# michelbarbeau/gr-uwspr

Hardware: AMD Instinct MI355X
Metric: 2-min WSPR frames decoded/sec (coarse+sync) (higher is better)
Workload: dtype f32

## Files before the change

gr-uwspr_amd/csrc/k4_jig.hip:

```cpp
#include "k4_common.h"

#pragma clang fp contract(off)

namespace uwspr {

constexpr int K4J_WAVES = 2;
#ifndef K4J_OCC
#define K4J_OCC 2
#endif
constexpr int K4J_PT_STRIDE = 18;

__global__ __launch_bounds__(64 * K4J_WAVES, K4J_OCC) void k4_jig(
    const float2 *__restrict__ frames, int fstride, int np, int nframes, const dev_grp *__restrict__ grps,
    int G, float *__restrict__ p_out, const float2 *__restrict__ ptab, int gps) {
  constexpr int NL = 6, PPW = 16;
  constexpr int R = 24;
  constexpr int AH = 21;
  constexpr int Q = (2 * (7 + AH) + 1) / 16;
  constexpr int M = Q + 1;
  constexpr int NSLOT = 16 + Q;
  constexpr int RS = 32 * M + 4;
  static_assert(4 * (NL - 1) < AH && M == 4, "ring reach");
  __shared__ __align__(16) float lds_all[K4J_WAVES][PPW * RS];
  __shared__ __align__(16) float2 ptl_all[K4J_WAVES][8 * K4J_PT_STRIDE];

  const int lane = threadIdx.x & 63;
  const int wv = __builtin_amdgcn_readfirstlane(threadIdx.x >> 6);
  float *lds = lds_all[wv];
  float2 *ptl = ptl_all[wv];

  const long long total = (long long)G * UWSPR_NSYM;
  const unsigned lblock = xcd_swizzle(blockIdx.x, gridDim.x);
  const long long g0 = ((long long)lblock * K4J_WAVES + wv) * PPW;
  if (g0 >= total) return;

  const int gA = (int)(g0 / UWSPR_NSYM);
  const int iA0 = (int)(g0 - (long long)gA * UWSPR_NSYM);
  const int sb = min(PPW, UWSPR_NSYM - iA0);
  const dev_grp A = grps[gA];
  const dev_grp Bg = grps[min(gA + 1, G - 1)];
  const bool okA = A.frame >= 0 && A.frame < nframes;
  const bool okB = (gA + 1 < G) && Bg.frame >= 0 && Bg.frame < nframes;
  const int frA = okA ? A.frame : 0, frB = okB ? Bg.frame : 0;
  const int nvA = okA ? (A.nvalid & 0xff) : 0, nvB = okB ? (Bg.nvalid & 0xff) : 0;
  const int selA = okA ? (A.nvalid >> 16) & 0xff : 0, selB = okB ? (Bg.nvalid >> 16) & 0xff : 0;
  const bool liveB = sb < PPW && okB;
  const bool use_tab = ptab != nullptr && (okA || liveB) && (!okA || selA != 0) && (!liveB || selB != 0);

  const int pr = lane >> 2;
  const int tone = lane & 3;
  const bool mineA = pr < sb;
  const int own_i = mineA ? iA0 + pr : pr - sb;
  if (!okA && !liveB) {
    if (g0 + pr < total) {
      const dev_grp &gy = mineA ? A : Bg;
      for (int l = 0; l < (gy.nvalid & 0xff) && l < NL; l++)
        p_out[((long long)(gy.hyp_base + (int)((gy.hmap >> (4 * l)) & 15u)) * UWSPR_NSYM + own_i) * 4 + tone] = 0.0f;
    }
    return;
  }
  const float2 *tabA = ptab, *tabB = ptab;
  if (use_tab) {
    tabA = ptab + ((size_t)(gA / gps) * kPtabPerSlot + (max(selA, 1) - 1)) * kPtabFloat2;
    tabB = ptab + ((size_t)((gA + 1) / gps) * kPtabPerSlot + (max(selB, 1) - 1)) * kPtabFloat2;
    if (!selA) tabA = tabB;
    if (!selB) tabB = tabA;
  }
  const bool knownA = !okA || (A.nvalid & 0x100) != 0, knownB = !okB || (Bg.nvalid & 0x100) != 0;
  const bool skip_mid = knownA && (knownB || sb >= PPW);
  const bool skip_last = !skip_mid && (!okA || nvA <= 5) && (!liveB || nvB <= 5);
  auto body = [&](auto skip_tag, auto tab_tag) __attribute__((always_inline)) {
  constexpr int SKIPL = decltype(skip_tag)::value;
  constexpr bool TAB = decltype(tab_tag)::value;
  const int l0A = okA ? A.lag[0] : 1 - 256 * iA0;
  const int l0B = okB ? Bg.lag[0] : 1;

  const int own_nb = (mineA ? l0A : l0B) + 256 * own_i;
  const bool interior = __all((own_nb > 0) && (own_nb + 255 + 16 * Q < np)  );

  const int kk = lane & 15;
  const int segq = lane >> 4;
  const float2 *src[4];
#pragma unroll
  for (int j = 0; j < 4; j++) {
    const int pj = 4 * j + segq;
    const bool sA = pj < sb;
    src[j] = frames + (long long)(sA ? frA : frB) * fstride + ((sA ? l0A + 256 * (iA0 + pj) : l0B + 256 * (pj - sb)) + kk);
  }
  float2 stage[4];
  auto load_slot = [&](int sl) {
    if (interior) {
#pragma unroll
      for (int j = 0; j < 4; j++) stage[j] = src[j][16 * sl];
    } else {
#pragma unroll
      for (int j = 0; j < 4; j++) {
        const int pj = 4 * j + segq;
        const bool sA = pj < sb;
        const int n = (sA ? l0A + 256 * (iA0 + pj) : l0B + 256 * (pj - sb)) + kk + 16 * sl;
        const bool inr = (n > 0) && (n < np);
        const float2 v = frames[(long long)(sA ? frA : frB) * fstride + min(max(n, 0), np - 1)];
        stage[j] = inr ? v : make_float2(0.0f, 0.0f);
      }
    }
  };
  const int st_row = segq * RS + 2 * kk;
  auto store_slot = [&](int pos) {
#pragma unroll
    for (int j = 0; j < 4; j++) *reinterpret_cast<float2 *>(&lds[st_row + 4 * j * RS + 32 * pos]) = stage[j];
  };
  float2 tstage[2];
  auto load_tab = [&](int c) {
#pragma unroll
    for (int j = 0; j < 2; j++) {
      const int e = lane + 64 * j, tn = (e >> 4) & 3, st = e & 15;
      tstage[j] = ((e >> 6) ? tabB : tabA)[tn * 256 + 16 * c + st];
    }
  };
  auto store_tab = [&]() {
#pragma unroll
    for (int j = 0; j < 2; j++) {
      const int e = lane + 64 * j;
      ptl[(e >> 4) * K4J_PT_STRIDE + (e & 15)] = tstage[j];
    }
  };

  {
    float2 pro[Q + 1][4];
#pragma unroll
    for (int sl = 0; sl <= Q; sl++) {
      load_slot(sl);
#pragma unroll
      for (int j = 0; j < 4; j++) pro[sl][j] = stage[j];
    }
    if (TAB) load_tab(0);
#pragma unroll
    for (int sl = 0; sl <= Q; sl++) {
#pragma unroll
      for (int j = 0; j < 4; j++) stage[j] = pro[sl][j];
      store_slot(sl);
    }
    if (TAB) store_tab();
  }
  float rc = 1.0f, rs = 0.0f, rcd = 1.0f, rsd = 0.0f;
  if (!TAB) {
    const dev_grp &gy = mineA ? A : Bg;
    const float fp = (gy.m_type == UWSPR_LINEAR)
                         ? (float)((double)gy.f0 + ((double)gy.drift / 2.0) * ((double)(float)own_i - 81.0) / 81.0)
                         : gy.f0 + gy.slmc;
    const float delta = ((float)tone - 1.5f) * 1.46484375f;
    double sn, cs;
    sincos(kTwoPiDt * (double)(fp + delta), &sn, &cs);
    rcd = (float)cs;
    rsd = (float)sn;
  }

  int sa[M];
#pragma unroll
  for (int q = 0; q < M; q++) sa[q] = pr * RS + 32 * q;
  const int trow = ((mineA ? 0 : 4) + tone) * K4J_PT_STRIDE;

  float inp[NL], quad[NL];
#pragma unroll
  for (int l = 0; l < NL; l++) { inp[l] = 0.0f; quad[l] = 0.0f; }

  float4 ring[R];
  wave_lds_fence();
#pragma unroll
  for (int e = 0; e < AH; e++) ring[e] = *reinterpret_cast<const float4 *>(&lds[sa[(2 * e) >> 4] + 2 * ((2 * e) & 15)]);
#pragma unroll
  for (int e = AH; e < R; e++) ring[e] = make_float4(0.0f, 0.0f, 0.0f, 0.0f);

  int wpos = 0;
  auto chunk = [&](auto phase_tag, int ch) __attribute__((always_inline)) {
    constexpr int PH = decltype(phase_tag)::value;
    load_slot(min(ch + Q + 1, NSLOT - 1));
    if (TAB) load_tab(min(ch + 1, 15));
    wave_lds_fence();
    float4 phn = make_float4(0.0f, 0.0f, 0.0f, 0.0f);
    if (TAB) phn = *reinterpret_cast<const float4 *>(&ptl[trow]);
#pragma unroll
    for (int i = 0; i < 8; i++) {
      const int j0 = 8 * PH + i;
      const int o = 2 * i + 2 * AH;
      ring[(j0 + AH) % R] = *reinterpret_cast<const float4 *>(&lds[sa[o >> 4] + 2 * (o & 15)]);
      float4 ph = phn;
      if (TAB) {
        if (i < 7) phn = *reinterpret_cast<const float4 *>(&ptl[trow + 2 * i + 2]);
      } else {
        ph.x = rc; ph.y = rs;
        k4_rot<false>(rc, rs, rcd, rsd);
        ph.z = rc; ph.w = rs;
        k4_rot<false>(rc, rs, rcd, rsd);
      }
      __builtin_amdgcn_sched_barrier(0);
#pragma unroll
      for (int l = 0; l < NL; l++) {
        if (l == SKIPL) continue;
        const float4 v = ring[(j0 + 4 * l) % R];
        k4_mac<false>(inp[l], quad[l], v.x, v.y, ph.x, ph.y);
        k4_mac<false>(inp[l], quad[l], v.z, v.w, ph.z, ph.w);
      }
      asm volatile("" : "+v"(inp[0]), "+v"(inp[1]), "+v"(inp[2]), "+v"(inp[3]), "+v"(inp[4]), "+v"(inp[5]),
                        "+v"(quad[0]), "+v"(quad[1]), "+v"(quad[2]), "+v"(quad[3]), "+v"(quad[4]), "+v"(quad[5])
                   :: "memory");
      __builtin_amdgcn_sched_barrier(0);
    }
    wave_lds_fence();
    store_slot(wpos);
    if (TAB) store_tab();
    wpos = (wpos + 1 == M) ? 0 : wpos + 1;
    const int first = sa[0];
#pragma unroll
    for (int q = 0; q + 1 < M; q++) sa[q] = sa[q + 1];
    sa[M - 1] = first;
  };
  for (int t = 0; t < 5; t++) {
    chunk(std::integral_constant<int, 0>{}, 3 * t);
    chunk(std::integral_constant<int, 1>{}, 3 * t + 1);
    chunk(std::integral_constant<int, 2>{}, 3 * t + 2);
  }
  chunk(std::integral_constant<int, 0>{}, 15);

  if (g0 + pr < total) {
    const int nv = mineA ? nvA : nvB;
    const int hb = mineA ? A.hyp_base : Bg.hyp_base;
    const uint32_t hm = mineA ? A.hmap : Bg.hmap;
#pragma unroll
    for (int l = 0; l < NL; l++) {
      if (l < nv && l != SKIPL) {
        const float pj = ieee_sqrtf(inp[l] * inp[l] + quad[l] * quad[l]);
        p_out[((long long)(hb + (int)((hm >> (4 * l)) & 15u)) * UWSPR_NSYM + own_i) * 4 + tone] = pj;
      }
    }
    const dev_grp &gy = mineA ? A : Bg;
    if (!(mineA ? okA : okB) && (gy.nvalid & 0xff) > 0)
      for (int l = 0; l < (gy.nvalid & 0xff) && l < NL; l++)
        p_out[((long long)(gy.hyp_base + (int)((gy.hmap >> (4 * l)) & 15u)) * UWSPR_NSYM + own_i) * 4 + tone] = 0.0f;
  }
  };
  if (use_tab) {
    if (skip_mid) body(std::integral_constant<int, 2>{}, std::true_type{});
    else if (skip_last) body(std::integral_constant<int, 5>{}, std::true_type{});
    else body(std::integral_constant<int, -1>{}, std::true_type{});
  } else {
    if (skip_mid) body(std::integral_constant<int, 2>{}, std::false_type{});
    else if (skip_last) body(std::integral_constant<int, 5>{}, std::false_type{});
    else body(std::integral_constant<int, -1>{}, std::false_type{});
  }
}

void launch_tonecorr_jig(uwspr_ctx *c, const float *frames, int B, const dev_grp *grps, int G, int64_t nhyps, float4 *p,
                         int gps) {
  if (G <= 0) return;
  prof_scope ps(c, UWSPR_K_TONECORR, nhyps, true);
  const long long total = (long long)G * UWSPR_NSYM;
  const long long waves = (total + 15) / 16;
  const unsigned blocks = (unsigned)((waves + K4J_WAVES - 1) / K4J_WAVES);
  if (gps < 1) gps = 1;
  launch_timed(c, ps, k4_jig, dim3(blocks), dim3(64 * K4J_WAVES), 0, (const float2 *)frames, c->fstride, c->np, B, grps, G,
               (float *)p, c->use_ptab ? (const float2 *)c->d_ptab : nullptr, gps);
}

}
```

gr-uwspr_amd/csrc/k4_tonecorr.hip:

```cpp
#include <string.h>

#include <algorithm>
#include <type_traits>

#include "k4_common.h"

#pragma clang fp contract(off)

namespace uwspr {

constexpr int K4_WAVES = 4;
constexpr int K4_ROWDW = 36;

template <int T, bool FAST = false>
__global__ __launch_bounds__(64 * K4_WAVES) void k4_tonecorr(
    const float2 *__restrict__ frames, int fstride, int np, int nframes, const dev_hyp *__restrict__ hyps,
    int H, float *__restrict__ p_out, const dev_grp *__restrict__ taken, int hyps_per_grp, int skip_pairs) {
  constexpr int PPW = 16 * T;
  constexpr int LPP = 4 / T;
  constexpr int NLD = PPW / 4;
  __shared__ __align__(16) float lds_all[K4_WAVES][PPW * K4_ROWDW];

  const int lane = threadIdx.x & 63;
  const int wv = __builtin_amdgcn_readfirstlane(threadIdx.x >> 6);
  float *lds = lds_all[wv];

  const long long total = (long long)H * UWSPR_NSYM;
  const long long g0 = ((long long)xcd_swizzle(blockIdx.x, gridDim.x) * K4_WAVES + wv) * PPW;
  if (g0 >= total) return;

  const int hA = (int)(g0 / UWSPR_NSYM);
  const int iA0 = (int)(g0 - (long long)hA * UWSPR_NSYM);
  const int sb = min(PPW, UWSPR_NSYM - iA0);
  dev_hyp A = hyps[hA];
  dev_hyp Bh = hyps[min(hA + 1, H - 1)];
  const int hB = min(hA + 1, H - 1);
  const bool takenA = (taken && ((taken[hA / hyps_per_grp].nvalid >> 16) & 0xff) != 0) ||
                      (skip_pairs && k4_drift_pair(hyps[hA & ~1], hyps[hA | 1], nframes));
  const bool takenB = (taken && ((taken[hB / hyps_per_grp].nvalid >> 16) & 0xff) != 0) ||
                      (skip_pairs && k4_drift_pair(hyps[hB & ~1], hyps[hB | 1], nframes));
  const bool okA = A.frame >= 0 && A.frame < nframes && !takenA;
  const bool okB = (hA + 1 < H) && Bh.frame >= 0 && Bh.frame < nframes && !takenB;
  if (!okA) { A.frame = 0; A.lag = 1 - 256 * iA0; }
  if (!okB) { Bh.frame = 0; Bh.lag = 1; }

  const int pr = lane / LPP;
  const int tone0 = (lane % LPP) * T;
  const bool mineA = pr < sb;
  const int own_i = mineA ? iA0 + pr : pr - sb;
  const bool own_ok = mineA ? okA : (okB && (g0 + pr) < total);
  if (!okA && !(okB && sb < PPW)) {
    if (g0 + pr < total && !(mineA ? takenA : takenB)) {
      float *out = p_out + (g0 + pr) * 4 + tone0;
#pragma unroll
      for (int j = 0; j < T; j++) out[j] = 0.0f;
    }
    return;
  }
  const int own_nb = (mineA ? A.lag : Bh.lag) + 256 * own_i;
  const bool interior = __all((own_nb > 0) && (own_nb + 255 < np));

  float cd[T], sd[T];
  {
    const dev_hyp &hy = mineA ? A : Bh;
    float fp;
    if (hy.m_type == UWSPR_LINEAR) {
      fp = (float)((double)hy.f0 +
                   ((double)hy.drift / 2.0) * ((double)(float)own_i - 81.0) / 81.0);
    } else {
      fp = hy.f0 + hy.slmc;
    }
#pragma unroll
    for (int j = 0; j < T; j++) {
      const float delta = ((float)(tone0 + j) - 1.5f) * 1.46484375f;
      const double ang = kTwoPiDt * (double)(fp + delta);
      double sn, cs;
      sincos(ang, &sn, &cs);
      cd[j] = (float)cs;
      sd[j] = (float)sn;
    }
  }

  const int kk = lane & 15;
  const int segq = lane >> 4;
  const float2 *src[NLD];
#pragma unroll
  for (int t = 0; t < NLD; t++) {
    const int seg = 4 * t + segq;
    const bool sA = seg < sb;
    const int fr = sA ? A.frame : Bh.frame;
    const int nb = sA ? A.lag + 256 * (iA0 + seg) : Bh.lag + 256 * (seg - sb);
    src[t] = frames + ((long long)fr * fstride + nb + kk);
  }

  float2 stage[NLD];
  auto load_chunk = [&](int c) {
    if (interior) {
#pragma unroll
      for (int t = 0; t < NLD; t++) stage[t] = src[t][16 * c];
    } else {
#pragma unroll
      for (int t = 0; t < NLD; t++) {
        const int seg = 4 * t + segq;
        const bool sA = seg < sb;
        const long long fb = (long long)(sA ? A.frame : Bh.frame) * fstride;
        const int n = (sA ? A.lag + 256 * (iA0 + seg) : Bh.lag + 256 * (seg - sb)) + 16 * c + kk;
        const bool inr = (n > 0) && (n < np);
        float2 v = frames[fb + min(max(n, 0), np - 1)];
        stage[t] = inr ? v : make_float2(0.0f, 0.0f);
      }
    }
  };

  float c[T], s[T], inp[T], quad[T];
#pragma unroll
  for (int j = 0; j < T; j++) { c[j] = 1.0f; s[j] = 0.0f; inp[j] = 0.0f; quad[j] = 0.0f; }

  load_chunk(0);
  for (int ch = 0; ch < 16; ch++) {
    wave_lds_fence();
#pragma unroll
    for (int t = 0; t < NLD; t++)
      *reinterpret_cast<float2 *>(&lds[(4 * t + segq) * K4_ROWDW + 2 * kk]) = stage[t];
    wave_lds_fence();
    if (ch < 15) load_chunk(ch + 1);
    float4 vnext = *reinterpret_cast<const float4 *>(&lds[pr * K4_ROWDW]);
#pragma unroll
    for (int k = 0; k < 16; k += 2) {
      const float4 v = vnext;
      if (k < 14) vnext = *reinterpret_cast<const float4 *>(&lds[pr * K4_ROWDW + 2 * (k + 2)]);
#pragma unroll
      for (int half = 0; half < 2; half++) {
        const float xx = half ? v.z : v.x, xy = half ? v.w : v.y;
#pragma unroll
        for (int j = 0; j < T; j++) {
          k4_mac<FAST>(inp[j], quad[j], xx, xy, c[j], s[j]);
          k4_rot<FAST>(c[j], s[j], cd[j], sd[j]);
        }
      }
    }
  }

  if (g0 + pr < total && !(mineA ? takenA : takenB)) {
    float *out = p_out + (g0 + pr) * 4 + tone0;
#pragma unroll
    for (int j = 0; j < T; j++) {
      const float pj = ieee_sqrtf(inp[j] * inp[j] + quad[j] * quad[j]);
      out[j] = own_ok ? pj : 0.0f;
    }
  }
}

void launch_tonecorr(uwspr_ctx *c, const float *frames, int B, const dev_hyp *hyps, int H,
                     float4 *p, const dev_grp *taken, int hyps_per_grp, bool skip_pairs) {
  if (H <= 0) return;
  prof_scope ps(c, UWSPR_K_TONECORR, H, true);
  const long long total = (long long)H * UWSPR_NSYM;
  int T = c->opt[UWSPR_OPT_K4_T];
  if (T != 1 && T != 2 && T != 4) T = total >= 1024 * 1024 ? 2 : 1;
  const long long waves = (total + 16 * T - 1) / (16 * T);
  const unsigned blocks = (unsigned)((waves + K4_WAVES - 1) / K4_WAVES);
  const float2 *fr = (const float2 *)frames;
  float *po = (float *)p;
  dim3 blk(64 * K4_WAVES);
  if (hyps_per_grp < 1) hyps_per_grp = 1;
  const int sp = skip_pairs && (H % 2 == 0) ? 1 : 0;
  if (T == 1 && c->fast_now) launch_timed(c, ps, (k4_tonecorr<1, true>), dim3(blocks), blk, 0, fr, c->fstride, c->np, B, hyps, H, po, taken, hyps_per_grp, sp);
  else if (T == 1) launch_timed(c, ps, k4_tonecorr<1>, dim3(blocks), blk, 0, fr, c->fstride, c->np, B, hyps, H, po, taken, hyps_per_grp, sp);
  else if (T == 2) launch_timed(c, ps, k4_tonecorr<2>, dim3(blocks), blk, 0, fr, c->fstride, c->np, B, hyps, H, po, taken, hyps_per_grp, sp);
  else launch_timed(c, ps, k4_tonecorr<4>, dim3(blocks), blk, 0, fr, c->fstride, c->np, B, hyps, H, po, taken, hyps_per_grp, sp);
}

}

namespace uwspr {

constexpr int K4G_WAVES = 2;

constexpr int K4_PT_STRIDE = 18;

template <int NL, int STEP, bool FAST = false>
__global__ __launch_bounds__(64 * K4G_WAVES) void k4_ring(
    const float2 *__restrict__ frames, int fstride, int np, int nframes, const dev_grp *__restrict__ grps,
    int G, float *__restrict__ p_out, const float2 *__restrict__ ptab, int gps) {
  constexpr int PPW = 16;
  constexpr int W = (NL - 1) * STEP;
  constexpr int Q = (15 + W) / 16;
  constexpr int M = Q + 1;
  constexpr int NSLOT = 16 + Q;
  constexpr int RS = 32 * M + 4;
  __shared__ __align__(16) float lds_all[K4G_WAVES][PPW * RS];
  __shared__ __align__(16) float2 ptl_all[K4G_WAVES][8 * K4_PT_STRIDE];

  const int lane = threadIdx.x & 63;
  const int wv = __builtin_amdgcn_readfirstlane(threadIdx.x >> 6);
  float *lds = lds_all[wv];
  float2 *ptl = ptl_all[wv];

  const long long total = (long long)G * UWSPR_NSYM;
  const unsigned lblock = xcd_swizzle(blockIdx.x, gridDim.x);
  const long long g0 = ((long long)lblock * K4G_WAVES + wv) * PPW;
  if (g0 >= total) return;

  const int gA = (int)(g0 / UWSPR_NSYM);
  const int iA0 = (int)(g0 - (long long)gA * UWSPR_NSYM);
  const int sb = min(PPW, UWSPR_NSYM - iA0);
  const dev_grp A = grps[gA];
  const dev_grp Bg = grps[min(gA + 1, G - 1)];
  const bool okA = A.frame >= 0 && A.frame < nframes;
  const bool okB = (gA + 1 < G) && Bg.frame >= 0 && Bg.frame < nframes;
  const int frA = okA ? A.frame : 0, frB = okB ? Bg.frame : 0;
  const int nvA = okA ? (A.nvalid & 0xff) : 0, nvB = okB ? (Bg.nvalid & 0xff) : 0;
  const int selA = okA ? (A.nvalid >> 16) & 0xff : 0, selB = okB ? (Bg.nvalid >> 16) & 0xff : 0;
  const bool liveB = sb < PPW && okB;
  const bool use_tab = ptab != nullptr && (okA || liveB) && (!okA || selA != 0) && (!liveB || selB != 0);
  const float2 *tabA = ptab, *tabB = ptab;
  if (use_tab) {
    if (selA) tabA = ptab + ((size_t)(gA / gps) * kPtabPerSlot + (selA - 1)) * kPtabFloat2;
    if (selB) tabB = ptab + ((size_t)((gA + 1) / gps) * kPtabPerSlot + (selB - 1)) * kPtabFloat2;
    if (!selA) tabA = tabB;
    if (!selB) tabB = tabA;
  }
  const bool knownA = !okA || (A.nvalid & 0x100) != 0, knownB = !okB || (Bg.nvalid & 0x100) != 0;
  const bool skip_mid = (NL == 5 || NL == 6) && knownA && (knownB || sb >= PPW);
#ifndef UWSPR_SKIP_LAST
#define UWSPR_SKIP_LAST 1
#endif
  const bool skip_last = UWSPR_SKIP_LAST && NL == 6 && !skip_mid && (okA || liveB) && (!okA || nvA <= 5) && (!liveB || nvB <= 5);
  const int l0A = okA ? A.lag[0] : 1 - 256 * iA0;
  const int l0B = okB ? Bg.lag[0] : 1;

  const int pr = lane >> 2;
  const int tone = lane & 3;
  const bool mineA = pr < sb;
  const int own_i = mineA ? iA0 + pr : pr - sb;
  if (!okA && !liveB) {
    if (g0 + pr < total) {
      const dev_grp &gy = mineA ? A : Bg;
      for (int l = 0; l < (gy.nvalid & 0xff) && l < NL; l++)
        p_out[((long long)(gy.hyp_base + (int)((gy.hmap >> (4 * l)) & 15u)) * UWSPR_NSYM + own_i) * 4 + tone] = 0.0f;
    }
    return;
  }
  const int own_nb = (mineA ? l0A : l0B) + 256 * own_i;
  const bool interior = __all((own_nb > 0) && (own_nb + 255 + 16 * Q < np)  );

  float cd = 1.0f, sd = 0.0f;
  if (!use_tab) {
    const dev_grp &gy = mineA ? A : Bg;
    float fp;
    if (gy.m_type == UWSPR_LINEAR) {
      fp = (float)((double)gy.f0 +
                   ((double)gy.drift / 2.0) * ((double)(float)own_i - 81.0) / 81.0);
    } else {
      fp = gy.f0 + gy.slmc;
    }
    const float delta = ((float)tone - 1.5f) * 1.46484375f;
    double sn, cs;
    sincos(kTwoPiDt * (double)(fp + delta), &sn, &cs);
    cd = (float)cs;
    sd = (float)sn;
  }

  const int kk = lane & 15;
  const int segq = lane >> 4;
  const float2 *src[4];
  long long fbase[4];
  int nfirst[4];
#pragma unroll
  for (int j = 0; j < 4; j++) {
    const int pj = 4 * j + segq;
    const bool sA = pj < sb;
    fbase[j] = (long long)(sA ? frA : frB) * fstride;
    nfirst[j] = (sA ? l0A + 256 * (iA0 + pj) : l0B + 256 * (pj - sb)) + kk;
    src[j] = frames + fbase[j] + nfirst[j];
  }
  float2 stage[4];
  auto load_slot = [&](int sl) {
    if (interior) {
#pragma unroll
      for (int j = 0; j < 4; j++) stage[j] = src[j][16 * sl];
    } else {
#pragma unroll
      for (int j = 0; j < 4; j++) {
        const int n = nfirst[j] + 16 * sl;
        const bool inr = (n > 0) && (n < np);
        const float2 v = frames[fbase[j] + min(max(n, 0), np - 1)];
        stage[j] = inr ? v : make_float2(0.0f, 0.0f);
      }
    }
  };
  auto store_slot = [&](int pos) {
#pragma unroll
    for (int j = 0; j < 4; j++)
      *reinterpret_cast<float2 *>(&lds[(4 * j + segq) * RS + 2 * kk + 32 * pos]) = stage[j];
  };

  {
    float2 pro[Q + 1][4];
#pragma unroll
    for (int sl = 0; sl <= Q; sl++) {
      load_slot(sl);
#pragma unroll
      for (int j = 0; j < 4; j++) pro[sl][j] = stage[j];
    }
#pragma unroll
    for (int sl = 0; sl <= Q; sl++) {
#pragma unroll
      for (int j = 0; j < 4; j++) stage[j] = pro[sl][j];
      store_slot(sl);
    }
  }

  int sa[M];
#pragma unroll
  for (int q = 0; q < M; q++) sa[q] = pr * RS + 32 * q;

  float c = 1.0f, s = 0.0f;
  float inp[NL], quad[NL];
#pragma unroll
  for (int l = 0; l < NL; l++) { inp[l] = 0.0f; quad[l] = 0.0f; }

  float2 tstage[2];
  auto load_tab = [&](int c) {
#pragma unroll
    for (int j = 0; j < 2; j++) {
      const int e = lane + 64 * j, tn = (e >> 4) & 3, st = e & 15;
      tstage[j] = ((e >> 6) ? tabB : tabA)[tn * 256 + 16 * c + st];
    }
  };
  auto store_tab = [&]() {
#pragma unroll
    for (int j = 0; j < 2; j++) {
      const int e = lane + 64 * j;
      ptl[(e >> 4) * K4_PT_STRIDE + (e & 15)] = tstage[j];
    }
  };
  const int trow = ((mineA ? 0 : 4) + tone) * K4_PT_STRIDE;
  if (use_tab) { load_tab(0); store_tab(); }

  int wpos = 0;
  auto walk = [&](auto skip_tag, auto tab_tag) {
    constexpr int SKIPL = decltype(skip_tag)::value;
    constexpr bool TAB = decltype(tab_tag)::value;
    for (int ch = 0; ch < 16; ch++) {
      load_slot(min(ch + Q + 1, NSLOT - 1));
      if (TAB) load_tab(min(ch + 1, 15));
      wave_lds_fence();
      static_assert(STEP % 2 == 0, "sample pairs must not straddle lags");
      float4 vc[NL], vn[NL];
#pragma unroll
      for (int l = 0; l < NL; l++) {
        if (l == SKIPL) { vc[l] = make_float4(0.0f, 0.0f, 0.0f, 0.0f); vn[l] = vc[l]; continue; }
        vc[l] = *reinterpret_cast<const float4 *>(&lds[sa[(STEP * l) >> 4] + 2 * ((STEP * l) & 15)]);
        vn[l] = vc[l];
      }
#pragma unroll
      for (int k = 0; k < 16; k += 2) {
        if (k < 14) {
#pragma unroll
          for (int l = 0; l < NL; l++) {
            if (l == SKIPL) continue;
            const int o = k + 2 + STEP * l;
            vn[l] = *reinterpret_cast<const float4 *>(&lds[sa[o >> 4] + 2 * (o & 15)]);
          }
        }
        float4 ph = make_float4(0.0f, 0.0f, 0.0f, 0.0f);
        if (TAB) ph = *reinterpret_cast<const float4 *>(&ptl[trow + k]);
#pragma unroll
        for (int half = 0; half < 2; half++) {
          const float pc = TAB ? (half ? ph.z : ph.x) : c, psn = TAB ? (half ? ph.w : ph.y) : s;
#pragma unroll
          for (int l = 0; l < NL; l++) {
            if (l == SKIPL) continue;
            const float xx = half ? vc[l].z : vc[l].x, xy = half ? vc[l].w : vc[l].y;
            k4_mac<FAST>(inp[l], quad[l], xx, xy, pc, psn);
          }
          if (!TAB) k4_rot<FAST>(c, s, cd, sd);
        }
#pragma unroll
        for (int l = 0; l < NL; l++) vc[l] = vn[l];
      }
      wave_lds_fence();
      store_slot(wpos);
      if (TAB) store_tab();
      wpos = (wpos + 1 == M) ? 0 : wpos + 1;
      const int first = sa[0];
#pragma unroll
      for (int q = 0; q + 1 < M; q++) sa[q] = sa[q + 1];
      sa[M - 1] = first;
    }
  };
  using sk_none = std::integral_constant<int, -1>;
  using sk_mid = std::integral_constant<int, 2>;
  using sk_last = std::integral_constant<int, NL == 6 ? NL - 1 : -1>;
  if (use_tab) {
    if (skip_mid) walk(sk_mid{}, std::true_type{});
    else if (skip_last) walk(sk_last{}, std::true_type{});
    else walk(sk_none{}, std::true_type{});
  } else {
    if (skip_mid) walk(sk_mid{}, std::false_type{});
    else if (skip_last) walk(sk_last{}, std::false_type{});
    else walk(sk_none{}, std::false_type{});
  }

  if (g0 + pr < total) {
    const int nv = mineA ? nvA : nvB;
    const int hb = mineA ? A.hyp_base : Bg.hyp_base;
    const uint32_t hm = mineA ? A.hmap : Bg.hmap;
#pragma unroll
    for (int l = 0; l < NL; l++) {
      if (l < nv && !(skip_mid && l == 2)) {
        const float pj = ieee_sqrtf(inp[l] * inp[l] + quad[l] * quad[l]);
        p_out[((long long)(hb + (int)((hm >> (4 * l)) & 15u)) * UWSPR_NSYM + own_i) * 4 + tone] = pj;
      }
    }
    const dev_grp &gy = mineA ? A : Bg;
    if (!(mineA ? okA : okB) && (gy.nvalid & 0xff) > 0)
      for (int l = 0; l < (gy.nvalid & 0xff) && l < NL; l++)
        p_out[((long long)(gy.hyp_base + (int)((gy.hmap >> (4 * l)) & 15u)) * UWSPR_NSYM + own_i) * 4 + tone] = 0.0f;
  }
}

void launch_tonecorr_ring(uwspr_ctx *c, const float *frames, int B, const dev_grp *grps, int G,
                          int NL, int step, int64_t nhyps, float4 *p, int gps) {
  if (G <= 0) return;
  const bool r5 = NL == 5 && step == 16, r6 = NL == 6 && step == 8;
  if (!r5 && !r6) return;
  prof_scope ps(c, UWSPR_K_TONECORR, nhyps, true);
  const long long total = (long long)G * UWSPR_NSYM;
  const long long waves = (total + 15) / 16;
  const unsigned blocks = (unsigned)((waves + K4G_WAVES - 1) / K4G_WAVES);
  const float2 *fr = (const float2 *)frames;
  float *po = (float *)p;
  dim3 blk(64 * K4G_WAVES);
  const float2 *pt = c->use_ptab ? c->d_ptab : nullptr;
  if (gps < 1) gps = 1;
  if (r5 && c->fast_now) launch_timed(c, ps, (k4_ring<5, 16, true>), dim3(blocks), blk, 0, fr, c->fstride, c->np, B, grps, G, po, pt, gps);
  else if (r5) launch_timed(c, ps, (k4_ring<5, 16>), dim3(blocks), blk, 0, fr, c->fstride, c->np, B, grps, G, po, pt, gps);
  else launch_timed(c, ps, (k4_ring<6, 8>), dim3(blocks), blk, 0, fr, c->fstride, c->np, B, grps, G, po, pt, gps);
}


}

namespace uwspr {

#ifndef K4F_CHUNK
#define K4F_CHUNK 32
#endif

constexpr int K4L_ROWS_PER_SLOT = UWSPR_NSYM + 1;

template <int QMASK, bool FAST>
__device__ __forceinline__ void k4_lag0_chunk(const float *__restrict__ smprow, const float4 *__restrict__ tabrow,
                                              int a0, float (&inp)[4], float (&quad)[4]) {
#pragma unroll 1
  for (int k0 = 0; k0 < 32; k0 += 8) {
#pragma unroll
    for (int kk = 0; kk < 8; kk += 2) {
      const int k = k0 + kk;
      const float4 x = *reinterpret_cast<const float4 *>(&smprow[2 * k]);
#pragma unroll
      for (int q = 0; q < 4; q++) {
        if (!((QMASK >> q) & 1)) continue;
        const float4 ph = tabrow[(a0 - 64 * q + k) >> 1];
        k4_mac<FAST>(inp[q], quad[q], x.x, x.y, ph.x, ph.y);
        k4_mac<FAST>(inp[q], quad[q], x.z, x.w, ph.z, ph.w);
      }
    }
  }
}

template <bool FAST = false>
__global__ __launch_bounds__(256, 4) void k4_lag0(
    const float2 *__restrict__ frames, int fstride, int np, int nframes, const dev_grp *__restrict__ grps,
    int nslots, float *__restrict__ p_out, const float2 *__restrict__ ptab) {
  constexpr int ROWS = 64, CH = 32, ROWDW = 2 * CH + 4, SEGS = 256 / CH, NR = ROWS / SEGS, NCHUNK = 14;
  __shared__ __align__(16) float smp[ROWS * ROWDW];
  __shared__ __align__(16) float4 tab[2][4][128];

  const int tid = threadIdx.x;
  const int lane = tid & 63;
  const int tone = __builtin_amdgcn_readfirstlane(tid >> 6);
  const long long total = (long long)nslots * K4L_ROWS_PER_SLOT;
  const long long g0 = (long long)xcd_swizzle(blockIdx.x, gridDim.x) * ROWS;
  if (g0 >= total) return;

  const int slotA = (int)(g0 / K4L_ROWS_PER_SLOT);
  const int rA0 = (int)(g0 - (long long)slotA * K4L_ROWS_PER_SLOT);
  const int sb = min(ROWS, K4L_ROWS_PER_SLOT - rA0);
  const bool hasB = sb < ROWS && slotA + 1 < nslots;
  const int slotB = hasB ? slotA + 1 : slotA;
  const dev_grp A = grps[slotA], Bg = grps[slotB];
  const int selA = (A.nvalid >> 16) & 0xff, selB = (Bg.nvalid >> 16) & 0xff;
  const bool doA = A.frame >= 0 && A.frame < nframes && selA != 0;
  const bool doB = hasB && Bg.frame >= 0 && Bg.frame < nframes && selB != 0;
  if (!doA && !doB) return;

#pragma unroll
  for (int sl = 0; sl < 2; sl++) {
    if (!(sl ? doB : doA)) continue;
    const float4 *src = reinterpret_cast<const float4 *>(
        ptab + ((size_t)(sl ? slotB : slotA) * kPtabPerSlot + ((sl ? selB : selA) - 1)) * kPtabFloat2);
    float4 *dst = &tab[sl][0][0];
    dst[tid] = src[tid];
    dst[tid + 256] = src[tid + 256];
  }

  const int row = lane;
  const bool mineA = row < sb;
  const int own_r = mineA ? rA0 + row : row - sb;
  const bool own_do = mineA ? doA : doB;
  const bool valid = (g0 + row < total) && (mineA || hasB) && own_do;

  const int kk = tid % CH, seg = tid / CH;
  const float2 *fbA = frames + (long long)(doA ? A.frame : 0) * fstride;
  const float2 *fbB = frames + (long long)(doB ? Bg.frame : 0) * fstride;
  const int nA0 = A.lag[0] + 256 * rA0, nB0 = Bg.lag[0];
  const bool interior = doA && (nA0 > 0) && (nA0 + 256 * (sb - 1) + 32 * NCHUNK < np) &&
                        (sb >= ROWS || (doB && (nB0 > 0) && (nB0 + 256 * (ROWS - sb - 1) + 32 * NCHUNK < np)));
  float2 stage[NR];
  int nrow[NR];
  bool rowB[NR];
#pragma unroll
  for (int r = 0; r < NR; r++) {
    const int rw = SEGS * r + seg;
    rowB[r] = rw >= sb;
    nrow[r] = (rowB[r] ? nB0 + 256 * (rw - sb) : nA0 + 256 * rw) + kk;
  }
  auto load_chunk = [&](int c) {
    if (interior) {
#pragma unroll
      for (int r = 0; r < NR; r++) stage[r] = (rowB[r] ? fbB : fbA)[nrow[r] + CH * c];
    } else {
#pragma unroll
      for (int r = 0; r < NR; r++) {
        const int n = nrow[r] + CH * c;
        const bool inr = (n > 0) && (n < np);
        const float2 v = (rowB[r] ? fbB : fbA)[min(max(n, 0), np - 1)];
        stage[r] = inr ? v : make_float2(0.0f, 0.0f);
      }
    }
  };
  auto store_chunk = [&]() {
#pragma unroll
    for (int r = 0; r < NR; r++)
      *reinterpret_cast<float2 *>(&smp[(SEGS * r + seg) * ROWDW + 2 * kk]) = stage[r];
  };

  float inp[4], quad[4];
#pragma unroll
  for (int q = 0; q < 4; q++) { inp[q] = 0.0f; quad[q] = 0.0f; }
  const float *smprow = &smp[row * ROWDW];
  const float4 *tabrow = &tab[mineA ? 0 : 1][tone][0];

  load_chunk(0);
  auto phase = [&](auto mask_tag, int c0) {
    constexpr int QMASK = decltype(mask_tag)::value;
#pragma unroll 1
    for (int c = c0; c < c0 + 2; c++) {
      __syncthreads();
      store_chunk();
      __syncthreads();
      load_chunk(min(c + 1, NCHUNK - 1));
      k4_lag0_chunk<QMASK, FAST>(smprow, tabrow, 32 * c, inp, quad);
    }
  };
  phase(std::integral_constant<int, 0x1>{}, 0);
  phase(std::integral_constant<int, 0x3>{}, 2);
  phase(std::integral_constant<int, 0x7>{}, 4);
  phase(std::integral_constant<int, 0xf>{}, 6);
  phase(std::integral_constant<int, 0xe>{}, 8);
  phase(std::integral_constant<int, 0xc>{}, 10);
  phase(std::integral_constant<int, 0x8>{}, 12);

  if (valid) {
    const int hb = mineA ? A.hyp_base : Bg.hyp_base;
#pragma unroll
    for (int q = 0; q < 4; q++) {
      const float pj = ieee_sqrtf(inp[q] * inp[q] + quad[q] * quad[q]);
      if (own_r < UWSPR_NSYM) p_out[((long long)(hb + q) * UWSPR_NSYM + own_r) * 4 + tone] = pj;
      if (q == 0 && own_r >= 1) p_out[((long long)(hb + 4) * UWSPR_NSYM + own_r - 1) * 4 + tone] = pj;
    }
  }
}

template <int WSETS>
__global__ __launch_bounds__(256 * WSETS, WSETS == 1 ? 3 : 6) void k4_lag0x(
    const float2 *__restrict__ frames, int fstride, int np, int nframes, const dev_grp *__restrict__ grps,
    int nslots, float *__restrict__ p_out, const float2 *__restrict__ ptab) {
  constexpr int NT = 256 * WSETS;
  constexpr int ROWS = 64, CH = 32, ROWDW = 2 * CH + 4, SEGS = NT / CH, NR = ROWS / SEGS, NCHUNK = 14;
  __shared__ __align__(16) float smp[2][ROWS * ROWDW];
  __shared__ __align__(16) float4 tab[2][4][128];

  const int tid = threadIdx.x;
  const int lane = tid & 63;
  const int wv = __builtin_amdgcn_readfirstlane(tid >> 6);
  const int tone = wv & 3;
  const int wset = wv >> 2;
  const long long total = (long long)nslots * K4L_ROWS_PER_SLOT;
  const long long g0 = (long long)xcd_swizzle(blockIdx.x, gridDim.x) * ROWS;
  if (g0 >= total) return;

  const int slotA = (int)(g0 / K4L_ROWS_PER_SLOT);
  const int rA0 = (int)(g0 - (long long)slotA * K4L_ROWS_PER_SLOT);
  const int sb = min(ROWS, K4L_ROWS_PER_SLOT - rA0);
  const bool hasB = sb < ROWS && slotA + 1 < nslots;
  const int slotB = hasB ? slotA + 1 : slotA;
  const dev_grp A = grps[slotA], Bg = grps[slotB];
  const int selA = (A.nvalid >> 16) & 0xff, selB = (Bg.nvalid >> 16) & 0xff;
  const bool doA = A.frame >= 0 && A.frame < nframes && selA != 0;
  const bool doB = hasB && Bg.frame >= 0 && Bg.frame < nframes && selB != 0;
  if (!doA && !doB) return;

#pragma unroll
  for (int sl = 0; sl < 2; sl++) {
    if (!(sl ? doB : doA)) continue;
    const float4 *src = reinterpret_cast<const float4 *>(
        ptab + ((size_t)(sl ? slotB : slotA) * kPtabPerSlot + ((sl ? selB : selA) - 1)) * kPtabFloat2);
    float4 *dst = &tab[sl][0][0];
    for (int e = tid; e < 512; e += NT) dst[e] = src[e];
  }

  const int row = lane;
  const bool mineA = row < sb;
  const int own_r = mineA ? rA0 + row : row - sb;
  const bool own_do = mineA ? doA : doB;
  const bool valid = (g0 + row < total) && (mineA || hasB) && own_do;

  const int kk = tid % CH, seg = tid / CH;
  const float2 *fbA = frames + (long long)(doA ? A.frame : 0) * fstride;
  const float2 *fbB = frames + (long long)(doB ? Bg.frame : 0) * fstride;
  const int nA0 = A.lag[0] + 256 * rA0, nB0 = Bg.lag[0];
  const bool interior = doA && (nA0 > 0) && (nA0 + 256 * (sb - 1) + 32 * NCHUNK < np) &&
                        (sb >= ROWS || (doB && (nB0 > 0) && (nB0 + 256 * (ROWS - sb - 1) + 32 * NCHUNK < np)));
  float2 stage[NR];
  int nrow[NR];
  bool rowB[NR];
#pragma unroll
  for (int r = 0; r < NR; r++) {
    const int rw = SEGS * r + seg;
    rowB[r] = rw >= sb;
    nrow[r] = (rowB[r] ? nB0 + 256 * (rw - sb) : nA0 + 256 * rw) + kk;
  }
  auto load_chunk = [&](int c) {
    if (interior) {
#pragma unroll
      for (int r = 0; r < NR; r++) stage[r] = (rowB[r] ? fbB : fbA)[nrow[r] + CH * c];
    } else {
#pragma unroll
      for (int r = 0; r < NR; r++) {
        const int n = nrow[r] + CH * c;
        const bool inr = (n > 0) && (n < np);
        const float2 v = (rowB[r] ? fbB : fbA)[min(max(n, 0), np - 1)];
        stage[r] = inr ? v : make_float2(0.0f, 0.0f);
      }
    }
  };
  auto store_chunk = [&](int buf) {
#pragma unroll
    for (int r = 0; r < NR; r++)
      *reinterpret_cast<float2 *>(&smp[buf][(SEGS * r + seg) * ROWDW + 2 * kk]) = stage[r];
  };

  float inp[4], quad[4];
#pragma unroll
  for (int q = 0; q < 4; q++) { inp[q] = 0.0f; quad[q] = 0.0f; }
  const float4 *tabrow = &tab[mineA ? 0 : 1][tone][0];

  load_chunk(0);
  store_chunk(0);
  load_chunk(1);
  __syncthreads();
  auto phase = [&](auto mask_tag, int c0) {
    constexpr int QM = decltype(mask_tag)::value;
#pragma unroll 1
    for (int c = c0; c < c0 + 2; c++) {
      if (WSETS == 1) {
        k4_lag0_chunk<QM, false>(&smp[c & 1][row * ROWDW], tabrow, 32 * c, inp, quad);
      } else if (wset == 0) {
        if (QM & 0x5) k4_lag0_chunk<QM & 0x5, false>(&smp[c & 1][row * ROWDW], tabrow, 32 * c, inp, quad);
      } else {
        if (QM & 0xa) k4_lag0_chunk<QM & 0xa, false>(&smp[c & 1][row * ROWDW], tabrow, 32 * c, inp, quad);
      }
      store_chunk((c + 1) & 1);
      load_chunk(min(c + 2, NCHUNK - 1));
      __syncthreads();
    }
  };
  phase(std::integral_constant<int, 0x1>{}, 0);
  phase(std::integral_constant<int, 0x3>{}, 2);
  phase(std::integral_constant<int, 0x7>{}, 4);
  phase(std::integral_constant<int, 0xf>{}, 6);
  phase(std::integral_constant<int, 0xe>{}, 8);
  phase(std::integral_constant<int, 0xc>{}, 10);
  phase(std::integral_constant<int, 0x8>{}, 12);

  if (valid) {
    const int hb = mineA ? A.hyp_base : Bg.hyp_base;
#pragma unroll
    for (int q = 0; q < 4; q++) {
      if (WSETS == 2 && (q & 1) != wset) continue;
      const float pj = ieee_sqrtf(inp[q] * inp[q] + quad[q] * quad[q]);
      if (own_r < UWSPR_NSYM) p_out[((long long)(hb + q) * UWSPR_NSYM + own_r) * 4 + tone] = pj;
      if (q == 0 && own_r >= 1) p_out[((long long)(hb + 4) * UWSPR_NSYM + own_r - 1) * 4 + tone] = pj;
    }
  }
}

void launch_tonecorr_lag0(uwspr_ctx *c, const float *frames, int B, const dev_grp *grps, int nslots,
                          int64_t nhyps, float4 *p) {
  if (nslots <= 0) return;
  prof_scope ps(c, UWSPR_K_TONECORR, nhyps, true);
  const unsigned wgs = (unsigned)(((long long)nslots * K4L_ROWS_PER_SLOT + 63) / 64);
  const int form = c->fast_now ? 0 : (c->opt[UWSPR_OPT_K4_FORMS] >> 1) & 3;
  if (c->fast_now)
    launch_timed(c, ps, k4_lag0<true>, dim3(wgs), dim3(256), 0, (const float2 *)frames, c->fstride, c->np, B, grps,
                 nslots, (float *)p, (const float2 *)c->d_ptab);
  else if (form & 2)
    launch_timed(c, ps, k4_lag0x<2>, dim3(wgs), dim3(512), 0, (const float2 *)frames, c->fstride, c->np, B, grps,
                 nslots, (float *)p, (const float2 *)c->d_ptab);
  else if (form & 1)
    launch_timed(c, ps, k4_lag0x<1>, dim3(wgs), dim3(256), 0, (const float2 *)frames, c->fstride, c->np, B, grps,
                 nslots, (float *)p, (const float2 *)c->d_ptab);
  else
    launch_timed(c, ps, k4_lag0<false>, dim3(wgs), dim3(256), 0, (const float2 *)frames, c->fstride, c->np, B, grps,
                 nslots, (float *)p, (const float2 *)c->d_ptab);
}

#ifdef K4F_STAMPS
constexpr int K4F_STAMP_WAVES = 4096;
__device__ unsigned long long g_k4f_stamps[K4F_STAMP_WAVES * 10];
#define K4F_T(v) const unsigned long long v = __builtin_amdgcn_s_memtime()
#define K4F_ACC(a, t1, t0) a += (t1) - (t0)
#else
#define K4F_T(v) do { } while (0)
#define K4F_ACC(a, t1, t0) do { } while (0)
#endif

template <int NF, int CH, bool FAST = false>
__global__ __launch_bounds__(256) void k4_fpack(
    const float2 *__restrict__ frames, int fstride, int np, int nframes, const dev_hyp *__restrict__ hyps,
    int nslots, float *__restrict__ p_out) {
  constexpr int ROWS = 64;
  constexpr int ROWDW = 2 * CH + 4;
  constexpr int NCH = 256 / CH;
  constexpr int SEGS = 256 / CH;
  constexpr int NR = ROWS / SEGS;
  __shared__ __align__(16) float smp[ROWS * ROWDW];
  __shared__ __align__(16) float4 tab[2][4][CH / 2][NF];

  const int tid = threadIdx.x;
  const int lane = tid & 63;
  const int tone = __builtin_amdgcn_readfirstlane(tid >> 6);
  #ifdef K4F_STAMPS
  const unsigned long long st_c0 = __builtin_amdgcn_s_memtime(), st_r0 = __builtin_amdgcn_s_memrealtime();
  unsigned long long st_bar1 = 0, st_gen = 0, st_bar2 = 0, st_ar = 0;
#endif
  const long long total = (long long)nslots * UWSPR_NSYM;
  const long long g0 = (long long)xcd_swizzle(blockIdx.x, gridDim.x) * ROWS;
  if (g0 >= total) return;
  const unsigned prio_class = k4_prio_class();

  const int slotA = (int)(g0 / UWSPR_NSYM);
  const int iA0 = (int)(g0 - (long long)slotA * UWSPR_NSYM);
  const int sb = min(ROWS, UWSPR_NSYM - iA0);
  const bool hasB = sb < ROWS && slotA + 1 < nslots;
  const int slotB = hasB ? slotA + 1 : slotA;
  const dev_hyp hA = hyps[(size_t)slotA * NF], hB = hyps[(size_t)slotB * NF];
  float fA[NF], fB[NF];
#pragma unroll
  for (int q = 0; q < NF; q++) { fA[q] = hyps[(size_t)slotA * NF + q].f0; fB[q] = hyps[(size_t)slotB * NF + q].f0; }
  const bool liveA = hA.frame >= 0 && hA.frame < nframes;
  const bool liveB = hasB && hB.frame >= 0 && hB.frame < nframes;
  const bool tabA = (hA.m_type != UWSPR_LINEAR) || (hA.drift == 0.0f);
  const bool tabB = (hB.m_type != UWSPR_LINEAR) || (hB.drift == 0.0f);
  const bool knownA = hyps[(size_t)slotA * NF + NF / 2].frame <= -2, knownB = hyps[(size_t)slotB * NF + NF / 2].frame <= -2;
  const bool tabled = (!liveA || tabA) && (!liveB || tabB);
  const bool skip_mid = (liveA || liveB) && (!liveA || knownA) && (!liveB || knownB);

  const int row = lane;
  const bool mineA = row < sb;
  const int own_i = mineA ? iA0 + row : row - sb;
  const int own_slot = mineA ? slotA : slotB;
  const bool own_live = mineA ? liveA : liveB;
  const bool valid = (g0 + row < total) && (mineA || hasB);
  if (!liveA && !liveB) {
    if (valid) {
#pragma unroll
      for (int q = 0; q < NF; q++) p_out[(((long long)own_slot * NF + q) * UWSPR_NSYM + own_i) * 4 + tone] = 0.0f;
    }
    return;
  }
  const dev_hyp &ho = mineA ? hA : hB;
  const float delta = ((float)tone - 1.5f) * 1.46484375f;

  const int kk = tid % CH, seg = tid / CH;
  const float2 *fbA = frames + (long long)(liveA ? hA.frame : 0) * fstride;
  const float2 *fbB = frames + (long long)(liveB ? hB.frame : 0) * fstride;
  const int nA0 = hA.lag + 256 * iA0, nB0 = hB.lag;
  const bool interior = liveA && (nA0 > 0) && (nA0 + 256 * sb < np) &&
                        (sb >= ROWS || (liveB && (nB0 > 0) && (nB0 + 256 * (ROWS - sb) < np)));
  float2 stage[NR];
  int nrow[NR];
  bool rowB[NR];
#pragma unroll
  for (int r = 0; r < NR; r++) {
    const int rw = SEGS * r + seg;
    rowB[r] = rw >= sb;
    nrow[r] = (rowB[r] ? nB0 + 256 * (rw - sb) : nA0 + 256 * rw) + kk;
  }
  auto load_chunk = [&](int c) {
    if (interior) {
#pragma unroll
      for (int r = 0; r < NR; r++) stage[r] = (rowB[r] ? fbB : fbA)[nrow[r] + CH * c];
    } else {
#pragma unroll
      for (int r = 0; r < NR; r++) {
        const int n = nrow[r] + CH * c;
        const bool inr = (n > 0) && (n < np);
        const float2 v = (rowB[r] ? fbB : fbA)[min(max(n, 0), np - 1)];
        stage[r] = inr ? v : make_float2(0.0f, 0.0f);
      }
    }
  };
  auto store_chunk = [&]() {
#pragma unroll
    for (int r = 0; r < NR; r++)
      *reinterpret_cast<float2 *>(&smp[(SEGS * r + seg) * ROWDW + 2 * kk]) = stage[r];
  };

  float inp[NF], quad[NF];
#pragma unroll
  for (int q = 0; q < NF; q++) { inp[q] = 0.0f; quad[q] = 0.0f; }

  if (tabled) {
    float cq = 1.0f, sq = 0.0f, cdq = 1.0f, sdq = 0.0f;
    const int gs = lane >= 4 * NF ? 1 : 0, gl = lane - gs * 4 * NF;
    const int gq = gl % NF, gt = min(gl / NF, 3);
    const bool gen = (tone == 0) && (lane < 8 * NF) && (gs ? liveB : liveA);
    if (gen) {
      float fq = gs ? fB[0] : fA[0];
#pragma unroll
      for (int q = 1; q < NF; q++) fq = (gq == q) ? (gs ? fB[q] : fA[q]) : fq;
      const dev_hyp &hg = gs ? hB : hA;
      const float fp = (hg.m_type == UWSPR_LINEAR)
                           ? (float)((double)fq + ((double)hg.drift / 2.0) * ((double)(float)0 - 81.0) / 81.0)
                           : fq + hg.slmc;
      const float gdelta = ((float)gt - 1.5f) * 1.46484375f;
      double sn, cs;
      sincos(kTwoPiDt * (double)(fp + gdelta), &sn, &cs);
      cdq = (float)cs;
      sdq = (float)sn;
    }
    const float4 *mytab = &tab[mineA ? 0 : 1][tone][0][0];
    load_chunk(0);
    auto walk = [&](auto skip_tag) {
      constexpr bool SKIP = decltype(skip_tag)::value;
      for (int ch = 0; ch < NCH; ch++) {
        K4F_T(t0);
        __syncthreads();
        K4F_T(t1);
        store_chunk();
        if (gen) {
#pragma unroll
          for (int k = 0; k < CH; k++) {
            reinterpret_cast<float2 *>(&tab[gs][gt][k >> 1][gq])[k & 1] = make_float2(cq, sq);
            k4_rot<FAST>(cq, sq, cdq, sdq);
          }
        }
        K4F_T(t2);
        __syncthreads();
        K4F_T(t3);
        k4_rotate_priority((unsigned)ch, prio_class);
        load_chunk(min(ch + 1, NCH - 1));
#pragma unroll
        for (int k = 0; k < CH; k += 2) {
          const float4 x = *reinterpret_cast<const float4 *>(&smp[row * ROWDW + 2 * k]);
#pragma unroll
          for (int q = 0; q < NF; q++) {
            if (SKIP && q == NF / 2) continue;
            const float4 ph = mytab[(k >> 1) * NF + q];
            k4_mac<FAST>(inp[q], quad[q], x.x, x.y, ph.x, ph.y);
            k4_mac<FAST>(inp[q], quad[q], x.z, x.w, ph.z, ph.w);
          }
        }
        K4F_T(t4);
        K4F_ACC(st_bar1, t1, t0); K4F_ACC(st_gen, t2, t1); K4F_ACC(st_bar2, t3, t2); K4F_ACC(st_ar, t4, t3);
      }
    };
    if (skip_mid) walk(std::true_type{}); else walk(std::false_type{});
  } else {
    float c[NF], s[NF], cd[NF], sd[NF];
#pragma unroll
    for (int q = 0; q < NF; q++) {
      const float f0 = mineA ? fA[q] : fB[q];
      const float fp = (ho.m_type == UWSPR_LINEAR)
                           ? (float)((double)f0 + ((double)ho.drift / 2.0) * ((double)(float)own_i - 81.0) / 81.0)
                           : f0 + ho.slmc;
      double sn, cs;
      sincos(kTwoPiDt * (double)(fp + delta), &sn, &cs);
      cd[q] = (float)cs; sd[q] = (float)sn; c[q] = 1.0f; s[q] = 0.0f;
    }
    load_chunk(0);
    for (int ch = 0; ch < NCH; ch++) {
      __syncthreads();
      store_chunk();
      __syncthreads();
      load_chunk(min(ch + 1, NCH - 1));
#pragma unroll
      for (int k = 0; k < CH; k += 2) {
        const float4 x4 = *reinterpret_cast<const float4 *>(&smp[row * ROWDW + 2 * k]);
#pragma unroll
        for (int half = 0; half < 2; half++) {
          const float xx = half ? x4.z : x4.x, xy = half ? x4.w : x4.y;
#pragma unroll
          for (int q = 0; q < NF; q++) {
            k4_mac<FAST>(inp[q], quad[q], xx, xy, c[q], s[q]);
            k4_rot<FAST>(c[q], s[q], cd[q], sd[q]);
          }
        }
      }
    }
  }

#ifdef K4F_STAMPS
  {
    const unsigned gw = xcd_swizzle(blockIdx.x, gridDim.x) * 4 + tone;
    if (lane == 0 && gw < (unsigned)K4F_STAMP_WAVES) {
      unsigned long long *o = &g_k4f_stamps[(size_t)gw * 10];
      o[0] = st_c0; o[1] = __builtin_amdgcn_s_memtime(); o[2] = st_r0; o[3] = __builtin_amdgcn_s_memrealtime();
      o[4] = st_bar1; o[5] = st_gen; o[6] = st_bar2; o[7] = st_ar;
      o[8] = (unsigned long long)__builtin_amdgcn_s_getreg((31 << 11) | 4) | ((unsigned long long)__builtin_amdgcn_s_getreg((31 << 11) | 20) << 32);
      o[9] = tabled ? 1 : 0;
    }
  }
#endif
  if (valid) {
#pragma unroll
    for (int q = 0; q < NF; q++) {
      float *o = &p_out[(((long long)own_slot * NF + q) * UWSPR_NSYM + own_i) * 4 + tone];
      if (!own_live) *o = 0.0f;
      else if (!(skip_mid && q == NF / 2)) *o = ieee_sqrtf(inp[q] * inp[q] + quad[q] * quad[q]);
    }
  }
}

void launch_tonecorr_fstage(uwspr_ctx *c, const float *frames, int B, const dev_hyp *hyps, int nslots,
                            int64_t nhyps, float4 *p) {
  if (nslots <= 0) return;
  prof_scope ps(c, UWSPR_K_TONECORR, nhyps, true);
  const unsigned wgs = (unsigned)(((long long)nslots * UWSPR_NSYM + 63) / 64);
  if (c->fast_now)
    launch_timed(c, ps, (k4_fpack<5, K4F_CHUNK, true>), dim3(wgs), dim3(256), 0,
                 (const float2 *)frames, c->fstride, c->np, B, hyps, nslots, (float *)p);
  else
    launch_timed(c, ps, (k4_fpack<5, K4F_CHUNK>), dim3(wgs), dim3(256), 0,
                 (const float2 *)frames, c->fstride, c->np, B, hyps, nslots, (float *)p);
}

}

#ifdef K4F_STAMPS
extern "C" int uwspr_debug_k4f_stamps(unsigned long long *out, int nwaves) {
  if (nwaves > uwspr::K4F_STAMP_WAVES) nwaves = uwspr::K4F_STAMP_WAVES;
  hipDeviceSynchronize();
  return (int)hipMemcpyFromSymbol(out, HIP_SYMBOL(uwspr::g_k4f_stamps), (size_t)nwaves * 80);
}
#endif
```

gr-uwspr_amd/csrc/k5_fold_schedule.hip:

```cpp
#include "uwspr_internal.h"

#pragma clang fp contract(off)

namespace uwspr {

__device__ __constant__ uint32_t kPr3[6] = UWSPR_PR3_WORDS;
__device__ __forceinline__ bool pr3_rt(int i) { return (kPr3[i >> 5] >> (i & 31)) & 1u; }

__device__ __forceinline__ void k5_wave_fence() {
  __builtin_amdgcn_fence(__ATOMIC_RELEASE, "wavefront");
  __builtin_amdgcn_wave_barrier();
  __builtin_amdgcn_fence(__ATOMIC_ACQUIRE, "wavefront");
}
constexpr int K5L_CH = 9;
__global__ __launch_bounds__(64) void k5_fold(const dev_hyp *__restrict__ hyps,
                                              const float4 *__restrict__ p, int H,
                                              float symfac, float *__restrict__ sync,
                                              uint8_t *__restrict__ symbols,
                                              const float4 *__restrict__ pwin, int per_slot) {
  UWSPR_SET_PRIO(UWSPR_SMALL_PRIO);
  __shared__ __align__(16) float4 tile[64 * K5L_CH];
  __shared__ __align__(16) uint8_t bytes[64 * UWSPR_NSYM];
  __shared__ int rowoff[64];
  __shared__ int rowslot[64];
  const int lane = threadIdx.x;
  const int h0 = blockIdx.x * 64;
  const int nh = min(64, H - h0);
  const int h = h0 + min(lane, nh - 1);
  const int fr = hyps[h].frame;
  const bool known = pwin != nullptr && fr <= -2;
  const bool live = lane < nh && (fr >= 0 || known);
  const bool soft = symbols != nullptr;
  const float4 *base = p + (size_t)h0 * UWSPR_NSYM;
  rowoff[lane] = known ? -1 : min(lane, nh - 1) * UWSPR_NSYM;
  rowslot[lane] = known ? h / per_slot : 0;

  auto stage = [&](int c) {
    k5_wave_fence();
#pragma unroll
    for (int j = 0; j < K5L_CH; j++) {
      const int idx = lane + 64 * j;
      const int hy = idx / K5L_CH, sy = idx - hy * K5L_CH;
      const int ro = rowoff[hy];
      tile[idx] = ro >= 0 ? base[(size_t)ro + c * K5L_CH + sy]
                          : pwin[(size_t)rowslot[hy] * UWSPR_NSYM + c * K5L_CH + sy];
    }
    k5_wave_fence();
  };

  float ss = 0.0f, totp = 0.0f, fsum = 0.0f, f2sum = 0.0f;
  for (int c = 0; c < UWSPR_NSYM / K5L_CH; c++) {
    stage(c);
#pragma unroll
    for (int j = 0; j < K5L_CH; j++) {
      const float4 P = tile[lane * K5L_CH + j];
      const bool bit = pr3_rt(c * K5L_CH + j);
      totp = totp + P.x; totp = totp + P.y; totp = totp + P.z; totp = totp + P.w;
      const float cmet = (P.y + P.w) - (P.x + P.z);
      ss = bit ? ss + cmet : ss - cmet;
      if (soft) {
        const float fs = bit ? P.w - P.y : P.z - P.x;
        fsum = (float)((double)fsum + (double)fs / 162.0);
        f2sum = (float)((double)f2sum + (double)(fs * fs) / 162.0);
      }
    }
  }
  if (lane < nh) sync[h] = live ? ieee_divf(ss, totp) : -1e30f;
  if (!soft) return;

  const float fac = ieee_sqrtf(f2sum - fsum * fsum);
  for (int c = 0; c < UWSPR_NSYM / K5L_CH; c++) {
    stage(c);
#pragma unroll
    for (int j = 0; j < K5L_CH; j++) {
      const float4 P = tile[lane * K5L_CH + j];
      const int i = c * K5L_CH + j;
      const bool bit = pr3_rt(i);
      float v = bit ? P.w - P.y : P.z - P.x;
      v = ieee_divf(symfac * v, fac);
      if (v > 127.0f) v = 127.0f;
      if (v < -128.0f) v = -128.0f;
      v = v + 128.0f;
      bytes[lane * UWSPR_NSYM + i] = (!live || v != v) ? (uint8_t)0 : (uint8_t)(int)v;
    }
  }
  k5_wave_fence();
  uint8_t *out = symbols + (size_t)h0 * UWSPR_NSYM;
  const int nbytes = nh * UWSPR_NSYM;
  for (int o = 4 * lane; o < nbytes; o += 256) {
    if (o + 4 <= nbytes && ((reinterpret_cast<uintptr_t>(out) + o) & 3) == 0) {
      *reinterpret_cast<uint32_t *>(out + o) = *reinterpret_cast<const uint32_t *>(&bytes[o]);
    } else {
      for (int q = 0; q < 4 && o + q < nbytes; q++) out[o + q] = bytes[o + q];
    }
  }
}

constexpr int K5W_WAVES = 4;

struct k5_wave_lds {
  float4 str[2][UWSPR_NSYM];
};
struct k5_wave_lds_soft {
  double q[2][UWSPR_NSYM];
};

template <bool SOFT>
__device__ __forceinline__ float fold_wave(const dev_hyp *__restrict__ hyps,
                                           const float4 *__restrict__ p, int h, float symfac,
                                           uint8_t *__restrict__ symbols, k5_wave_lds &L,
                                           k5_wave_lds_soft *Q, const float4 *__restrict__ prow = nullptr) {
  const int lane = threadIdx.x & 63;
  if (hyps[h].frame < 0 && !prow) {
    if (SOFT)
      for (int i = lane; i < UWSPR_NSYM; i += 64) symbols[(size_t)h * UWSPR_NSYM + i] = 0;
    return -1e30f;
  }
  const float4 *src = prow ? prow : p + (size_t)h * UWSPR_NSYM;
  float fs[3];
#pragma unroll
  for (int r = 0; r < 3; r++) {
    const int i = lane + 64 * r;
    fs[r] = 0.0f;
    if (i < UWSPR_NSYM) {
      const float4 P = src[i];
      const bool bit = pr3_rt(i);
      L.str[0][i] = P;
      const float cmet = (P.y + P.w) - (P.x + P.z);
      L.str[1][i] = make_float4(0.0f, 0.0f, 0.0f, bit ? cmet : -cmet);
      fs[r] = bit ? P.w - P.y : P.z - P.x;
      if (SOFT) {
        Q->q[0][i] = (double)fs[r] / 162.0;
        Q->q[1][i] = (double)(fs[r] * fs[r]) / 162.0;
      }
    }
  }
  k5_wave_fence();
  float acc = 0.0f;
  if (lane < 2) {
    const float4 *st = L.str[lane];
#pragma unroll 9
    for (int i = 0; i < UWSPR_NSYM; i++) {
      const float4 P = st[i];
      acc = acc + P.x; acc = acc + P.y; acc = acc + P.z; acc = acc + P.w;
    }
  } else if (SOFT && lane < 4) {
    const double *q = Q->q[lane - 2];
#pragma unroll 9
    for (int i = 0; i < UWSPR_NSYM; i++) acc = (float)((double)acc + q[i]);
  }
  const float totp = __shfl(acc, 0), ss = __shfl(acc, 1);
  const float sync = ieee_divf(ss, totp);
  if (SOFT) {
    const float fsum = __shfl(acc, 2), f2sum = __shfl(acc, 3);
    const float fac = ieee_sqrtf(f2sum - fsum * fsum);
#pragma unroll
    for (int r = 0; r < 3; r++) {
      const int i = lane + 64 * r;
      if (i < UWSPR_NSYM) {
        float v = ieee_divf(symfac * fs[r], fac);
        if (v > 127.0f) v = 127.0f;
        if (v < -128.0f) v = -128.0f;
        v = v + 128.0f;
        symbols[(size_t)h * UWSPR_NSYM + i] = (v != v) ? (uint8_t)0 : (uint8_t)(int)v;
      }
    }
  }
  k5_wave_fence();
  return sync;
}

template <bool SOFT>
__global__ __launch_bounds__(64 * K5W_WAVES) void k5_fold_wave(
    const dev_hyp *__restrict__ hyps, const float4 *__restrict__ p, int H, float symfac,
    float *__restrict__ sync, uint8_t *__restrict__ symbols, const float4 *__restrict__ pwin, int per_slot) {
  UWSPR_SET_PRIO(UWSPR_SMALL_PRIO);
  __shared__ k5_wave_lds L[K5W_WAVES];
  __shared__ k5_wave_lds_soft Q[SOFT ? K5W_WAVES : 1];
  const int wv = __builtin_amdgcn_readfirstlane(threadIdx.x >> 6);
  const int h = blockIdx.x * K5W_WAVES + wv;
  if (h >= H) return;
  const float4 *prow = (pwin && hyps[h].frame <= -2) ? pwin + (size_t)(h / per_slot) * UWSPR_NSYM : nullptr;
  const float s = fold_wave<SOFT>(hyps, p, h, symfac, symbols, L[wv], SOFT ? &Q[wv] : nullptr, prow);
  if ((threadIdx.x & 63) == 0) sync[h] = s;
}

void launch_fold(uwspr_ctx *c, const dev_hyp *hyps, const float4 *p, int H, float *sync,
                 uint8_t *symbols, const float4 *pwin, int per_slot) {
  if (H <= 0) return;
  prof_scope ps(c, UWSPR_K_FOLD, H);
  const int forced = c->opt[UWSPR_OPT_K5_LANES];
  const bool lanes_form = forced >= 0 ? forced != 0 : H >= 32768;
  if (per_slot < 1) per_slot = 1;
  if (!lanes_form) {
    dim3 g((H + K5W_WAVES - 1) / K5W_WAVES), b(64 * K5W_WAVES);
    if (symbols) hipLaunchKernelGGL(k5_fold_wave<true>, g, b, 0, c->stream, hyps, p, H, 50.0f, sync, symbols, pwin, per_slot);
    else hipLaunchKernelGGL(k5_fold_wave<false>, g, b, 0, c->stream, hyps, p, H, 50.0f, sync, symbols, pwin, per_slot);
  } else {
    hipLaunchKernelGGL(k5_fold, dim3((H + 63) / 64), dim3(64), 0, c->stream, hyps, p, H, 50.0f,
                       sync, symbols, pwin, per_slot);
  }
}

__device__ float slm_drift_t0(double V1, double V2, int p1, int p2, float cf) {
  const double q1 = V1 * 0.0 + (double)p1, q2 = V2 * 0.0 + (double)p2;
  const float sign = (float)(((q1 * V1 + q2 * V2) > 0) * 2 - 1);
  const double num = fabs(V1 * q1 + V2 * q2);
  const double den = sqrt(q1 * q1 + q2 * q2);
  if (den == 0) return 0.0f;
  return (float)((double)(-sign) * num / den * (double)cf / (double)1500.0f);
}

__global__ void k_prep_hyps(const uwspr_hyp *__restrict__ in, dev_hyp *__restrict__ out, int H,
                            float cf) {
  const int h = blockIdx.x * 256 + threadIdx.x;
  if (h >= H) return;
  const uwspr_hyp a = in[h];
  dev_hyp d;
  d.frame = a.frame; d.lag = a.lag; d.f0 = a.f0; d.drift = a.drift; d.m_type = a.m_type;
  d.slmc = (a.m_type == UWSPR_NONLINEAR) ? slm_drift_t0(a.V1, a.V2, a.p1, a.p2, cf) : 0.0f;
  out[h] = d;
}

void launch_prep_hyps(uwspr_ctx *c, const uwspr_hyp *abi, dev_hyp *out, int H) {
  if (H <= 0) return;
  prof_scope ps(c, UWSPR_K_SCHED, H);
  hipLaunchKernelGGL(k_prep_hyps, dim3((H + 255) / 256), dim3(256), 0, c->stream, abi, out, H,
                     (float)c->p.cf);
}


__device__ inline void emit(dev_hyp *h, const cand_state &st, bool on, int lag, float f0,
                            float drift, bool known = false) {
  h->frame = on ? (known ? -2 - st.frame : st.frame) : -1;
  h->lag = lag; h->f0 = f0; h->drift = drift; h->slmc = st.slmc; h->m_type = st.m_type;
}

__device__ inline void emit_group(dev_grp *g, const cand_state &st, bool on, float f0, float drift,
                                  int hyp_base, const int *lags, int n, uint32_t hmap = 0x76543210u) {
  g->frame = on ? st.frame : -1;
  g->m_type = st.m_type; g->f0 = f0; g->drift = drift; g->slmc = st.slmc;
  g->nvalid = n; g->hyp_base = hyp_base; g->hmap = hmap;
  for (int l = 0; l < 8; l++) g->lag[l] = l < n ? lags[l] : lags[0];
}

__device__ inline void emit_centre(uwspr_candidate *ce, int32_t *cframe, const cand_state &st, bool on) {
  ce->freq = st.f1; ce->snr = 0.0f; ce->drift = 0.0f; ce->sync = 0.0f; ce->shift = st.shift1;
  ce->m_nonlinear.V1 = 0.0; ce->m_nonlinear.V2 = 0.0; ce->m_nonlinear.p1 = 0; ce->m_nonlinear.p2 = 0;
  if (st.m_type == UWSPR_LINEAR) { ce->m_type = UWSPR_LINEAR; ce->m_linear.drift = st.drift1; }
  else { ce->m_type = 2; ce->m_linear.drift = st.slmc; }
  *cframe = on ? st.frame : -1;
}

struct best3 { float sync; int shift; float f; int q; };
__device__ inline best3 best_of(const float *sy, const dev_hyp *hy, int n) {
  best3 b{-1e30f, 0, 0.0f, -1};
  for (int q = 0; q < n; q++)
    if (sy[q] > b.sync) { b.sync = sy[q]; b.shift = hy[q].lag; b.f = hy[q].f0; b.q = q; }
  return b;
}

constexpr double kTwoPiDt5 = 2.0 * 3.14159265358979323846 * (double)(float)(1.0 / 375.0);

__device__ __forceinline__ void ptab_build(float2 *__restrict__ tabs, int nq, int qfirst, float fc, float fstep,
                                           int m_type, float drift, float slmc) {
  const int lane = threadIdx.x & 63;
  if (lane >= 4 * nq) return;
  const int qi = lane >> 2, tone = lane & 3, q = qfirst + qi;
  const float f0 = fc + (float)(q - 2) * fstep;
  const float fp = (m_type == UWSPR_LINEAR)
                       ? (float)((double)f0 + ((double)drift / 2.0) * ((double)(float)0 - 81.0) / 81.0)
                       : f0 + slmc;
  const float delta = ((float)tone - 1.5f) * 1.46484375f;
  double sn, cs;
  sincos(kTwoPiDt5 * (double)(fp + delta), &sn, &cs);
  const float cd = (float)cs, sd = (float)sn;
  float c = 1.0f, sv = 0.0f;
  float4 *t = reinterpret_cast<float4 *>(tabs + (size_t)qi * kPtabFloat2 + tone * 256);
  for (int k = 0; k < 128; k += 4) {
    float4 v[4];
#pragma unroll
    for (int j = 0; j < 4; j++) {
      v[j].x = c; v[j].y = sv;
      float nc = c * cd - sv * sd;
      float ns = c * sd + sv * cd;
      c = nc; sv = ns;
      v[j].z = c; v[j].w = sv;
      nc = c * cd - sv * sd;
      ns = c * sd + sv * cd;
      c = nc; sv = ns;
    }
#pragma unroll
    for (int j = 0; j < 4; j++) t[k + j] = v[j];
  }
}

__device__ __forceinline__ int ptab_index(const cand_state &st, int set, float f0, float drift, bool on) {
  if (!on) return -1;
  if (st.m_type == UWSPR_LINEAR && drift != 0.0f) return -1;
  if (!(set == 0 ? st.tabA_ok : st.tabB_ok)) return -1;
  const float fc = set == 0 ? st.tabA_f : st.tabB_f, step = set == 0 ? 0.25f : 0.05f;
  for (int q = 0; q < 5; q++)
    if (__float_as_int(fc + (float)(q - 2) * step) == __float_as_int(f0)) return (set == 0 ? 0 : kPtabSetB) + q;
  return -1;
}
__device__ __forceinline__ int ptab_set(const cand_state &st, int set, float centre, float drift, bool on) {
  if (!on) return -1;
  if (st.m_type == UWSPR_LINEAR && drift != 0.0f) return -1;
  if (!(set == 0 ? st.tabA_ok : st.tabB_ok)) return -1;
  if (__float_as_int(centre) != __float_as_int(set == 0 ? st.tabA_f : st.tabB_f)) return -1;
  return set == 0 ? 0 : kPtabSetB;
}
__device__ __forceinline__ int ptab_select(const cand_state &st, int set, float f0, float drift, bool on) {
  return ptab_index(st, set, f0, drift, on) + 1;
}

__global__ void k_sched_init(const uwspr_candidate *__restrict__ cands,
                             const int32_t *__restrict__ npk, int cand_stride, int B,
                             int per_frame, float cf, cand_state *__restrict__ state,
                             dev_hyp *__restrict__ hyps, dev_grp *__restrict__ grps, float2 *__restrict__ ptab) {
  UWSPR_SET_PRIO(UWSPR_SMALL_PRIO);
  const int slot = blockIdx.x;
  if (slot >= B * per_frame) return;
  const int b = slot / per_frame, j = slot - b * per_frame;
  cand_state st;
  const bool on = j < npk[b] && j < cand_stride;
  if (on) {
    const uwspr_candidate cnd = cands[(size_t)b * cand_stride + j];
    st.frame = b;
    st.m_type = cnd.m_type;
    st.slmc = (cnd.m_type == UWSPR_NONLINEAR)
                  ? slm_drift_t0(cnd.m_nonlinear.V1, cnd.m_nonlinear.V2, cnd.m_nonlinear.p1,
                                 cnd.m_nonlinear.p2, cf)
                  : 0.0f;
    st.f1 = cnd.freq;
    st.drift1 = (cnd.m_type == UWSPR_LINEAR) ? cnd.m_linear.drift : 0.0f;
    st.shift1 = cnd.shift;
    st.sync1 = cnd.sync;
  } else {
    st.frame = -1; st.m_type = 0; st.slmc = 0.0f; st.f1 = 0.0f; st.drift1 = 0.0f;
    st.shift1 = 0; st.sync1 = 0.0f;
  }
  st.worth = 0; st.driftp = 0.0f; st.driftm = 0.0f; st.csync = 0.0f; st.cknown = 0;
  const float f0 = st.f1 + (float)0 * 0.0f;
  st.tabA_f = f0; st.tabB_f = 0.0f; st.tabB_ok = 0;
  st.tabA_ok = (ptab != nullptr && on && (st.m_type != UWSPR_LINEAR || st.drift1 == 0.0f)) ? 1 : 0;
  if (st.tabA_ok) ptab_build(ptab + ((size_t)slot * kPtabPerSlot + 2) * kPtabFloat2, 1, 2, f0, 0.25f, st.m_type, st.drift1, st.slmc);
  if (threadIdx.x != 0) return;
  state[slot] = st;
  dev_hyp *h = hyps + (size_t)slot * 5;
  int lags[5];
  for (int q = 0; q < 5; q++) {
    lags[q] = st.shift1 - 128 + 64 * q;
    emit(&h[q], st, on, lags[q], f0, st.drift1);
  }
  emit_group(&grps[slot], st, on, f0, st.drift1, slot * 5, lags, 5);
  grps[slot].nvalid |= ptab_select(st, 0, f0, st.drift1, on) << 16;
}

template <int STAGE>
__device__ __forceinline__ void sched_step_body(int slot, cand_state *__restrict__ state,
                                                const dev_hyp *__restrict__ hin,
                                                const float *sync_of_slot,
                                                dev_hyp *__restrict__ hout,
                                                dev_grp *__restrict__ grps,
                                                uwspr_candidate *__restrict__ cent,
                                                int32_t *__restrict__ cframe, bool reuse, int team = 0,
                                                int njig = UWSPR_NJIG, int *wsrc = nullptr, bool tabs = false,
                                                bool fast = false) {
  int ws = -1;
  cand_state st = state[slot];
  const bool live = st.frame >= 0;
  constexpr int NIN = STAGE == 1 ? 5 : STAGE == 2 ? 5 : STAGE == 3 ? 2 : STAGE == 4 ? 5 : 5;
  constexpr int NOUT = STAGE == 1 ? 5 : STAGE == 2 ? 2 : STAGE == 3 ? 5 : STAGE == 4 ? 5 : 17;
  const dev_hyp *hi = hin + (size_t)slot * NIN;
  const float *sy = sync_of_slot;
  dev_hyp *ho = hout + (size_t)slot * (STAGE == 5 ? njig : NOUT);

  if (STAGE == 1) {
    if (live) { best3 b = best_of(sy, hi, 5); st.sync1 = b.sync; st.shift1 = b.shift; st.f1 = b.f; ws = b.q; }
    st.cknown = (reuse && live && st.sync1 > -1e30f) ? 1 : 0;
    st.csync = st.sync1;
    for (int q = 0; q < 5; q++)
      emit(&ho[q], st, live, st.shift1, st.f1 + (float)(q - 2) * 0.25f, st.drift1, q == 2 && st.cknown);
    emit_centre(&cent[slot], &cframe[slot], st, live);
  } else if (STAGE == 2) {
    if (live) {
      best3 b = best_of(sy, hi, 5); st.sync1 = b.sync; st.shift1 = b.shift; st.f1 = b.f;
      ws = (b.q == 2 && hi[2].frame <= -2) ? -1 : b.q;
    }
    st.cknown = (reuse && live && st.sync1 > -1e30f) ? 1 : 0;
    st.csync = st.sync1;
    const bool lin = live && st.m_type == UWSPR_LINEAR;
    st.driftp = (float)((double)st.drift1 + 0.5);
    st.driftm = (float)((double)st.drift1 - 0.5);
    const float f0 = st.f1 + (float)0 * 0.0f;
    emit(&ho[0], st, lin, st.shift1, f0, st.driftp);
    emit(&ho[1], st, lin, st.shift1, f0, st.driftm);
    emit_centre(&cent[slot], &cframe[slot], st, lin);
  } else if (STAGE == 3) {
    if (live && st.m_type == UWSPR_LINEAR) {
      float syncp = -1e30f, syncm = -1e30f;
      if (sy[0] > syncp) syncp = sy[0]; else { st.f1 = 0.0f; st.shift1 = 0; st.cknown = 0; }
      if (sy[1] > syncm) syncm = sy[1]; else { st.f1 = 0.0f; st.shift1 = 0; st.cknown = 0; }
      if (syncp > st.sync1) { st.drift1 = st.driftp; st.sync1 = syncp; ws = 0; }
      else if (syncm > st.sync1) { st.drift1 = st.driftm; st.sync1 = syncm; ws = 1; }
    }
    st.worth = (live && st.sync1 > 0.10f) ? 1 : 0;
    st.csync = st.sync1;
    const float f0 = st.f1 + (float)0 * 0.0f;
    int lags[5];
    for (int q = 0; q < 5; q++) {
      lags[q] = st.shift1 - 32 + 16 * q;
      emit(&ho[q], st, st.worth != 0, lags[q], f0, st.drift1, q == 2 && st.cknown);
    }
    emit_group(&grps[slot], st, st.worth != 0, f0, st.drift1, slot * 5, lags, 5);
    if (st.cknown) grps[slot].nvalid |= 0x100;
    st.tabB_f = f0;
    st.tabB_ok = (tabs && st.worth && (st.m_type != UWSPR_LINEAR || st.drift1 == 0.0f)) ? 1 : 0;
    grps[slot].nvalid |= ptab_select(st, 1, f0, st.drift1, st.worth != 0) << 16;
  } else if (STAGE == 4) {
    if (st.worth) {
      best3 b = best_of(sy, hi, 5); st.sync1 = b.sync; st.shift1 = b.shift; st.f1 = b.f;
      ws = (b.q == 2 && hi[2].frame <= -2) ? -1 : b.q;
    }
    st.cknown = (reuse && st.worth && st.sync1 > -1e30f) ? 1 : 0;
    st.csync = st.sync1;
    for (int q = 0; q < 5; q++)
      emit(&ho[q], st, st.worth != 0, st.shift1, st.f1 + (float)(q - 2) * 0.05f, st.drift1,
           q == 2 && st.cknown);
    emit_centre(&cent[slot], &cframe[slot], st, st.worth != 0);
  } else {
    if (st.worth) {
      best3 b = best_of(sy, hi, 5); st.sync1 = b.sync; st.shift1 = b.shift; st.f1 = b.f;
      ws = (b.q == 2 && hi[2].frame <= -2) ? -1 : b.q;
    }
    const bool known0 = reuse && !fast && st.worth && st.sync1 > -1e30f;
    st.cknown = known0 ? 1 : 0;
    if (team < njig) {
      const int idt = team;
      int ii = (idt + 1) / 2;
      if (idt % 2 == 1) ii = -ii;
      ii = 8 * ii;
      emit(&ho[idt], st, st.worth != 0, st.shift1 + ii, st.f1, st.drift1, idt == 0 && known0);
    }
    for (int g = 0; g < 3; g++) {
      if (team != UWSPR_NJIG + g) continue;
      const int n = g < 2 ? 6 : 5;
      int gl[6], idt0 = 99;
      int id[6];
      for (int l = 0; l < n; l++) {
        const int m = 6 * g + l, d = m - 8;
        id[l] = d == 0 ? 0 : (d < 0 ? -2 * d - 1 : 2 * d);
        gl[l] = st.shift1 + 8 * d;
        idt0 = id[l] < idt0 ? id[l] : idt0;
      }
      uint32_t hmap = 0;
      for (int l = 0; l < n; l++) hmap |= (uint32_t)(id[l] - idt0) << (4 * l);
      emit_group(&grps[slot * 3 + g], st, st.worth != 0 && njig >= UWSPR_NJIG, st.f1, st.drift1,
                 slot * UWSPR_NJIG + idt0, gl, n, hmap);
      if (g == 1 && known0) grps[slot * 3 + g].nvalid |= 0x100;
      grps[slot * 3 + g].nvalid |= ptab_select(st, 1, st.f1, st.drift1, st.worth != 0 && njig >= UWSPR_NJIG) << 16;
    }
  }
  if (team == 0) { state[slot] = st; if (wsrc) *wsrc = ws; }
}

__device__ __forceinline__ float wave_sum(float v) {
#pragma unroll
  for (int o = 32; o >= 1; o >>= 1) v += __shfl_xor(v, o);
  return v;
}
__device__ __forceinline__ float fold_wave_fast(const dev_hyp *__restrict__ hyps, const float4 *__restrict__ p, int h) {
  const int lane = threadIdx.x & 63;
  if (hyps[h].frame < 0) return -1e30f;
  float tp = 0.0f, sm = 0.0f;
#pragma unroll
  for (int r = 0; r < 3; r++) {
    const int i = lane + 64 * r;
    if (i < UWSPR_NSYM) {
      const float4 P = p[(size_t)h * UWSPR_NSYM + i];
      tp += (P.x + P.y) + (P.z + P.w);
      const float cmet = (P.y + P.w) - (P.x + P.z);
      sm += pr3_rt(i) ? cmet : -cmet;
    }
  }
  return ieee_divf(wave_sum(sm), wave_sum(tp));
}

template <int STAGE, bool FAST = false>
__global__ void k5_fold_step(cand_state *__restrict__ state, const dev_hyp *__restrict__ hin,
                             const float4 *__restrict__ p, float *__restrict__ sync,
                             dev_hyp *__restrict__ hout, dev_grp *__restrict__ grps,
                             uwspr_candidate *__restrict__ cent, int32_t *__restrict__ cframe, int nslots,
                             int reuse, int njig, float4 *__restrict__ pwin, float2 *__restrict__ ptab) {
  UWSPR_SET_PRIO(UWSPR_SMALL_PRIO);
  constexpr int NIN = STAGE == 3 ? 2 : 5;
  __shared__ k5_wave_lds L[FAST ? 1 : NIN];
  __shared__ float sy[NIN];
  __shared__ int s_wsrc;
  const int slot = blockIdx.x;
  const int wv = __builtin_amdgcn_readfirstlane(threadIdx.x >> 6);
  {
    const int q = wv;
    const int h = slot * NIN + q;
    float s;
    if (hin[h].frame <= -2) s = state[slot].csync;
    else if (FAST) s = fold_wave_fast(hin, p, h);
    else s = fold_wave<false>(hin, p, h, 50.0f, nullptr, L[FAST ? 0 : q], nullptr);
    if ((threadIdx.x & 63) == 0) { sy[q] = s; sync[h] = s; }
  }
  __syncthreads();
  if (STAGE == 5) {
    if (threadIdx.x < UWSPR_NJIG + 3)
      sched_step_body<STAGE>(slot, state, hin, sy, hout, grps, cent, cframe, reuse != 0, (int)threadIdx.x, njig, &s_wsrc, ptab != nullptr, FAST);
  } else if (threadIdx.x == 0) {
    sched_step_body<STAGE>(slot, state, hin, sy, hout, grps, cent, cframe, reuse != 0, 0, njig, &s_wsrc, ptab != nullptr, FAST);
  }
  __syncthreads();
  if (STAGE == 3 && ptab && threadIdx.x < 64) {
    const cand_state st = state[slot];
    if (st.tabB_ok)
      ptab_build(ptab + ((size_t)slot * kPtabPerSlot + kPtabSetB) * kPtabFloat2, 5, 0, st.tabB_f, 0.05f, st.m_type, st.drift1, st.slmc);
  }
  const int ws = s_wsrc;
  if (pwin && ws >= 0)
    for (int e = threadIdx.x; e < UWSPR_NSYM; e += blockDim.x)
      pwin[(size_t)slot * UWSPR_NSYM + e] = p[((size_t)slot * NIN + ws) * UWSPR_NSYM + e];
}

__global__ void k_sched_finish(const cand_state *__restrict__ state,
                               const dev_hyp *__restrict__ h5, const float *__restrict__ sync5,
                               const uint8_t *__restrict__ sym5, uwspr_demod_out *__restrict__ out,
                               int nslots, int njig, const uwspr_candidate *__restrict__ cands,
                               const int32_t *__restrict__ npk, int maxfreqs, int per_frame, int K,
                               uint8_t *__restrict__ slab) {
  UWSPR_SET_PRIO(UWSPR_SMALL_PRIO);
  const int slot = blockIdx.x;
  if (slot >= nslots) return;
  const int tid = threadIdx.x;
  constexpr int K5F_HALFWORDS = (UWSPR_NJIG * UWSPR_NSYM + 2) / 2, K5F_ROUNDS = (K5F_HALFWORDS + 255) / 256;
  uint16_t symv[K5F_ROUNDS];
  {
    const uint16_t *src = reinterpret_cast<const uint16_t *>(sym5 + (size_t)slot * njig * UWSPR_NSYM);
    const int have = njig * UWSPR_NSYM;
#pragma unroll
    for (int j = 0; j < K5F_ROUNDS; j++) {
      const int e = tid + 256 * j;
      symv[j] = (e < K5F_HALFWORDS && 2 * e < have) ? src[e] : (uint16_t)0;
    }
  }
  const cand_state st = state[slot];
  uwspr_demod_out *o = out + slot;
  if (tid == 0) {
    o->f1 = st.f1; o->drift1 = st.drift1; o->sync1 = st.sync1; o->shift1 = st.shift1;
    o->worth_a_try = st.worth;
  }
  const bool on = st.frame >= 0 && st.worth;
  static_assert((UWSPR_NJIG * UWSPR_NSYM) % 2 == 0 && UWSPR_NSYM % 2 == 0, "two-byte accesses below");
  static_assert(offsetof(uwspr_demod_out, symbols) % 4 == 0 && sizeof(uwspr_demod_out) % 4 == 0 &&
                offsetof(uwspr_demod_out, _pad) == offsetof(uwspr_demod_out, symbols) + UWSPR_NJIG * UWSPR_NSYM &&
                sizeof(((uwspr_demod_out *)0)->_pad) == 2, "symbols + pad are written as 32-bit words below");
  __shared__ __align__(4) uint8_t sy_s[UWSPR_NJIG * UWSPR_NSYM + 2];
  const int nby = on ? njig * UWSPR_NSYM : 0;
  {
    uint16_t *dst = reinterpret_cast<uint16_t *>(sy_s);
#pragma unroll
    for (int j = 0; j < K5F_ROUNDS; j++) {
      const int e = tid + 256 * j;
      if (e < K5F_HALFWORDS) dst[e] = 2 * e < nby ? symv[j] : (uint16_t)0;
    }
  }
  __syncthreads();
  if (tid < UWSPR_NJIG) {
    const bool have = on && tid < njig;
    const size_t q = (size_t)slot * njig + tid;
    float rms = 0.0f;
    if (have) {
      float sq = 0.0f;
#pragma unroll 6
      for (int i = 0; i < UWSPR_NSYM; i++) {
        const float y = (float)((double)(float)sy_s[tid * UWSPR_NSYM + i] - 128.0);
        sq += y * y;
      }
      rms = (float)sqrt((double)sq / 162.0);
    }
    o->jig_sync[tid] = have ? sync5[q] : 0.0f;
    o->jig_rms[tid] = rms;
    o->jig_shift[tid] = have ? h5[q].lag : 0;
  }
  {
    uint32_t *dst = reinterpret_cast<uint32_t *>(&o->symbols[0][0]);
    const uint32_t *src = reinterpret_cast<const uint32_t *>(sy_s);
    for (int e = tid; e < (UWSPR_NJIG * UWSPR_NSYM + 2) / 4; e += blockDim.x) dst[e] = src[e];
  }
  if (slab != nullptr && slot % per_frame == 0) {
    const int b = slot / per_frame;
    const int slab_bytes = 16 + K * 48 + 16, words = slab_bytes / 4;
    uint32_t *so = reinterpret_cast<uint32_t *>(slab + (size_t)b * slab_bytes);
    const uint32_t *cw = reinterpret_cast<const uint32_t *>(cands + (size_t)b * maxfreqs);
    const int n = npk[b];
    for (int w = tid; w < words; w += blockDim.x) {
      uint32_t v = 0;
      if (w == 0) v = (uint32_t)n;
      else if (w >= 4 && w < 4 + K * 12) { const int k = (w - 4) / 12; v = (k < n && k < maxfreqs) ? cw[w - 4] : 0u; }
      else if (w >= 4 + K * 12) {
        const int t = w - 4 - K * 12;
        v = t == 0 ? __float_as_uint(st.f1) : t == 1 ? __float_as_uint(st.drift1) : t == 2 ? __float_as_uint(st.sync1) : (uint32_t)st.shift1;
      }
      so[w] = v;
    }
  }
}

__global__ void k_pack_slabs(const uwspr_candidate *__restrict__ cands,
                             const int32_t *__restrict__ npk, int maxfreqs,
                             const uwspr_demod_out *__restrict__ dout, int per_frame, int K,
                             uint8_t *__restrict__ slab, int B) {
  UWSPR_SET_PRIO(UWSPR_SMALL_PRIO);
  const int b = blockIdx.x;
  if (b >= B) return;
  const int slab_bytes = 16 + K * 48 + 16;
  uint32_t *out = reinterpret_cast<uint32_t *>(slab + (size_t)b * slab_bytes);
  const int words = slab_bytes / 4;
  const uint32_t *cw = reinterpret_cast<const uint32_t *>(cands + (size_t)b * maxfreqs);
  const uint32_t *dw = reinterpret_cast<const uint32_t *>(dout + (size_t)b * per_frame);
  const int n = npk[b];
  for (int w = threadIdx.x; w < words; w += blockDim.x) {
    uint32_t v = 0;
    if (w == 0) v = (uint32_t)n;
    else if (w >= 4 && w < 4 + K * 12) { const int k = (w - 4) / 12; v = (k < n && k < maxfreqs) ? cw[w - 4] : 0u; }
    else if (w >= 4 + K * 12) v = dw[w - 4 - K * 12];
    out[w] = v;
  }
}

void launch_pack_slabs(uwspr_ctx *c, const uwspr_candidate *cands, const int32_t *npk,
                       const uwspr_demod_out *dout, int per_frame, int K, uint8_t *slab, int B) {
  prof_scope ps(c, UWSPR_K_SCHED, B);
  hipLaunchKernelGGL(k_pack_slabs, dim3(B), dim3(128), 0, c->stream, cands, npk, c->fc.maxfreqs,
                     dout, per_frame, K, slab, B);
}

void launch_sched_init(uwspr_ctx *c, const uwspr_candidate *cands, const int32_t *npk,
                       int cand_stride, int B, int per_frame) {
  const int nslots = B * per_frame;
  prof_scope ps(c, UWSPR_K_SCHED, nslots);
  hipLaunchKernelGGL(k_sched_init, dim3(nslots), dim3(64), 0, c->stream, cands,
                     npk, cand_stride, B, per_frame, (float)c->p.cf, c->d_state, c->d_hyps, c->d_grps,
                     c->use_ptab ? c->d_ptab : nullptr);
}

void launch_fold_step(uwspr_ctx *c, int stage, int nslots, int njig) {
  prof_scope ps(c, UWSPR_K_FOLD, (int64_t)nslots * (stage == 3 ? 2 : 5));
  dev_hyp *half0 = c->d_hyps, *half1 = c->d_hyps + (size_t)nslots * UWSPR_NJIG;
  dev_hyp *hin = (stage & 1) ? half0 : half1;
  dev_hyp *hout = (stage & 1) ? half1 : half0;
  dim3 g(nslots);
  const int reuse = c->reuse_centre ? 1 : 0;
  auto go = [&](auto kern, int threads) {
    hipLaunchKernelGGL(kern, g, dim3(threads), 0, c->stream, c->d_state, hin, c->d_p, c->d_sync, hout, c->d_grps,
                       c->d_cent, c->d_cent_frame, nslots, reuse, njig, (float4 *)c->d_pwin,
                       c->use_ptab ? c->d_ptab : nullptr);
  };
  if (c->fast_now) {
    switch (stage) {
      case 1: go(k5_fold_step<1, true>, 320); break;
      case 2: go(k5_fold_step<2, true>, 320); break;
      case 3: go(k5_fold_step<3, true>, 128); break;
      case 4: go(k5_fold_step<4, true>, 320); break;
      default: go(k5_fold_step<5, true>, 320); break;
    }
  } else {
    switch (stage) {
      case 1: go(k5_fold_step<1>, 320); break;
      case 2: go(k5_fold_step<2>, 320); break;
      case 3: go(k5_fold_step<3>, 128); break;
      case 4: go(k5_fold_step<4>, 320); break;
      default: go(k5_fold_step<5>, 320); break;
    }
  }
}

__global__ void k_keep_try0(const dev_hyp *__restrict__ h5, const float4 *__restrict__ p, float4 *__restrict__ pwin,
                            int njig, int nslots) {
  UWSPR_SET_PRIO(UWSPR_SMALL_PRIO);
  const int slot = blockIdx.x;
  if (slot >= nslots || h5[(size_t)slot * njig].frame < 0) return;
  for (int e = threadIdx.x; e < UWSPR_NSYM; e += blockDim.x)
    pwin[(size_t)slot * UWSPR_NSYM + e] = p[(size_t)slot * njig * UWSPR_NSYM + e];
}

void launch_keep_try0(uwspr_ctx *c, int nslots, int njig) {
  dev_hyp *h5 = c->d_hyps + (size_t)nslots * UWSPR_NJIG;
  hipLaunchKernelGGL(k_keep_try0, dim3(nslots), dim3(192), 0, c->stream, h5, c->d_p, (float4 *)c->d_pwin, njig, nslots);
}

void launch_sched_finish(uwspr_ctx *c, int nslots, int njig) {
  prof_scope ps(c, UWSPR_K_SCHED, nslots);
  dev_hyp *h5 = c->d_hyps + (size_t)nslots * UWSPR_NJIG;
  uint8_t *slab = c->cands_from_fdr ? c->next_slab : nullptr;
  hipLaunchKernelGGL(k_sched_finish, dim3(nslots), dim3(256), 0, c->stream, c->d_state, h5,
                     c->d_sync, c->d_sym, c->cur_dout, nslots, njig, c->cur_cands, c->cur_npk, c->fc.maxfreqs,
                     c->sched_per_frame, c->next_slab_K, slab);
  if (slab) c->next_slab_done = true;
}

}
```

gr-uwspr_amd/csrc/uwspr_api.hip:

```cpp
#include <errno.h>
#include <math.h>
#include <stdarg.h>
#include <stdio.h>
#include <stdlib.h>
#include <string.h>

#include <algorithm>
#include <vector>

#include "uwspr_internal.h"

namespace uwspr {
int coarse_configure(const fdr_consts &f);
size_t coarse_lds_bytes(const fdr_consts &f);
int coarse_seq_words();
size_t coarse_plan(fdr_consts &f, int pitch_opt, int tile_opt);
uint32_t coarse_seq_entry(const fdr_consts &f, int k, int off);
}

using namespace uwspr;

static int fail(uwspr_ctx *c, int status, const char *fmt, ...) {
  if (c) {
    va_list ap;
    va_start(ap, fmt);
    vsnprintf(c->err, sizeof(c->err), fmt, ap);
    va_end(ap);
  }
  return status;
}

#define HIPCHK(c, call)                                                                  \
  do {                                                                                   \
    hipError_t e_ = (call);                                                              \
    if (e_ != hipSuccess)                                                                \
      return fail((c), UWSPR_ERR_HIP, "%s failed: %s (%s:%d)", #call, hipGetErrorString(e_), \
                  __FILE__, __LINE__);                                                   \
  } while (0)

template <typename T>
static int ensure(uwspr_ctx *c, T **buf, size_t *cap, size_t need_elems) {
  if (need_elems <= *cap && *buf) return UWSPR_OK;
  if (*buf) { HIPCHK(c, hipStreamSynchronize(c->stream)); HIPCHK(c, hipFree(*buf)); *buf = nullptr; *cap = 0; }
  size_t n = std::max<size_t>(need_elems, 1);
  hipError_t e = hipMalloc((void **)buf, n * sizeof(T));
  if (e != hipSuccess) return fail(c, UWSPR_ERR_NOMEM, "hipMalloc(%zu bytes): %s", n * sizeof(T), hipGetErrorString(e));
  *cap = n;
  return UWSPR_OK;
}

prof_scope::prof_scope(uwspr_ctx *cx, int kind, int64_t units, bool ext_) : c(cx), idx(-1), ext(ext_) {
  if (!(c->prof_mask & (1 << kind))) return;
  ev_pair p;
  auto get = [&]() {
    hipEvent_t e;
    if (!c->ev_pool.empty()) { e = c->ev_pool.back(); c->ev_pool.pop_back(); }
    else (void)hipEventCreate(&e);
    return e;
  };
  p.a = get(); p.b = get(); p.kind = kind; p.units = units;
  if (!ext) (void)hipEventRecord(p.a, c->stream);
  c->prof_events.push_back(p);
  idx = (int)c->prof_events.size() - 1;
}
prof_scope::~prof_scope() {
  if (idx >= 0 && !ext) (void)hipEventRecord(c->prof_events[idx].b, c->stream);
}

static float slm_frequency_drift(double V1, double V2, int p1, int p2, float cf, float t) {
  const float cs = 1500.0f;
  const double q1 = V1 * (double)t + (double)p1;
  const double q2 = V2 * (double)t + (double)p2;
  const float sign = (float)(((q1 * V1 + q2 * V2) > 0) * 2 - 1);
  const double num = fabs(V1 * q1 + V2 * q2);
  const double den = sqrt(q1 * q1 + q2 * q2);
  if (den == 0) return 0.0f;
  return (float)((double)(-sign) * num / den * (double)cf / (double)cs);
}

static const struct { const char *name; int dflt, lo, hi; } kOptions[UWSPR_NOPT] = {
    {"sched", 1, 0, 1},
    {"stage_kernels", 1, 0, 1},
    {"reuse", 1, 0, 1},
    {"phasor_tables", 1, 0, 1},
    {"fast_search", 0, 0, 1},
    {"k4_t", 0, 0, 4},
    {"k5_lanes", -1, -1, 1},
    {"k1_rows", 0, 0, 348},
    {"k3_tile", -1, -1, 2},
    {"k3_pitch", 0, 0, 4096},
    {"sched_stamps", 0, 0, 1},
    {"sched_grid", 0, 0, 65536},
    {"dist_force_comm", 0, 0, 1},
    {"frontend", 0, 0, 1},
    {"k4_forms", 1, 0, 255},
};

static void refresh_options(uwspr_ctx *c) {
  c->use_stage_kernels = c->opt[UWSPR_OPT_STAGE_KERNELS] != 0;
  c->reuse_centre = c->opt[UWSPR_OPT_REUSE] != 0;
  c->use_ptab = c->opt[UWSPR_OPT_PHASOR_TABLES] != 0;
  c->fast_search = c->opt[UWSPR_OPT_FAST_SEARCH] != 0;
  c->use_fused = c->opt[UWSPR_OPT_SCHED] != 0 && !c->fast_search;
  c->sched_grid = c->opt[UWSPR_OPT_SCHED_GRID];
}

static int option_index(const char *name) {
  if (!name) return -1;
  for (int i = 0; i < UWSPR_NOPT; i++)
    if (!strcmp(name, kOptions[i].name)) return i;
  return -1;
}

extern "C" int uwspr_set_option(uwspr_ctx *c, const char *name, int value) {
  if (!c) return UWSPR_ERR_ARG;
  const int i = option_index(name);
  if (i < 0) return fail(c, UWSPR_ERR_ARG, "unknown option '%s'", name ? name : "(null)");
  if (i == UWSPR_OPT_K1_ROWS || i == UWSPR_OPT_K3_TILE || i == UWSPR_OPT_K3_PITCH)
    return fail(c, UWSPR_ERR_ARG, "option '%s' shapes the context when it is created: UWSPR_OPTIONS=%s=%d", name, name, value);
  if (value < kOptions[i].lo || value > kOptions[i].hi)
    return fail(c, UWSPR_ERR_ARG, "option '%s' = %d: allowed %d .. %d", name, value, kOptions[i].lo, kOptions[i].hi);
  c->opt[i] = value; c->opt_set[i] = true;
  refresh_options(c);
  return UWSPR_OK;
}

extern "C" int uwspr_get_option(uwspr_ctx *c, const char *name, int *value) {
  if (!c || !value) return UWSPR_ERR_ARG;
  const int i = option_index(name);
  if (i < 0) return fail(c, UWSPR_ERR_ARG, "unknown option '%s'", name ? name : "(null)");
  *value = c->opt[i];
  return UWSPR_OK;
}

static int options_from_environment(uwspr_ctx *c) {
  for (int i = 0; i < UWSPR_NOPT; i++) { c->opt[i] = kOptions[i].dflt; c->opt_set[i] = false; }
  const char *e = getenv("UWSPR_OPTIONS");
  if (e) {
    char buf[512];
    const size_t len = strlen(e);
    if (len >= sizeof(buf)) return fail(c, UWSPR_ERR_ARG, "UWSPR_OPTIONS: %zu characters (at most %zu)", len, sizeof(buf) - 1);
    memcpy(buf, e, len + 1);
    char *tok = buf;
    while (*tok) {
      while (*tok == ',' || *tok == ' ') tok++;
      if (!*tok) break;
      char *end = tok;
      while (*end && *end != ',' && *end != ' ') end++;
      const bool last = *end == 0;
      *end = 0;
      char *eq = strchr(tok, '=');
      if (!eq) return fail(c, UWSPR_ERR_ARG, "UWSPR_OPTIONS: '%s' is not name=value", tok);
      *eq = 0;
      const int i = option_index(tok);
      if (i < 0) return fail(c, UWSPR_ERR_ARG, "UWSPR_OPTIONS: unknown option '%s'", tok);
      char *vend = nullptr;
      errno = 0;
      const long v = strtol(eq + 1, &vend, 10);
      if (vend == eq + 1 || *vend || errno || v < kOptions[i].lo || v > kOptions[i].hi)
        return fail(c, UWSPR_ERR_ARG, "UWSPR_OPTIONS: %s='%s' is not an integer in %d .. %d", tok, eq + 1, kOptions[i].lo, kOptions[i].hi);
      c->opt[i] = (int)v; c->opt_set[i] = true;
      if (last) break;
      tok = end + 1;
    }
  }
  refresh_options(c);
  return UWSPR_OK;
}

extern "C" int uwspr_ctx_create(const uwspr_params *p, int device, uwspr_ctx **out) {
  if (!p || !out) return UWSPR_ERR_ARG;
  *out = nullptr;
  uwspr_ctx *c = new (std::nothrow) uwspr_ctx();
  if (!c) return UWSPR_ERR_NOMEM;
  memset(c->err, 0, sizeof(c->err));
  c->p = *p;
  c->device = device;
  c->own_stream = c->stream = nullptr;
  c->d_window = c->d_twiddle = nullptr; c->d_off = nullptr; c->d_umap = nullptr; c->d_k3_tile = nullptr;
  c->d_fe_taps = nullptr; c->fe_mode = -1; c->fe_J = 0; c->fe_dcols = 0; c->cap_audio = 0; c->d_audio = nullptr;
  c->cap_frames_bytes = 0; c->d_frames = nullptr; c->cap_B = 0;
  c->d_ps = c->d_psavg = c->d_smraw = c->d_smspec = c->d_noise = nullptr;
  c->d_cands = nullptr; c->d_npk = nullptr; c->d_work = nullptr; c->last_B = 0; c->num_cus = 256;
  c->grid_cap = 0; c->cap_grid_bytes = 0; c->d_syncgrid = nullptr;
  c->cap_hyps = 0; c->d_hyps = nullptr; c->cap_grps = 0; c->d_grps = nullptr;
  c->cap_cent = 0; c->d_cent = nullptr; c->d_cent_frame = nullptr; c->cap_abi_hyps = 0; c->d_abi_hyps = nullptr;
  c->cap_p = 0; c->d_p = nullptr; c->cap_sync = 0; c->d_sync = nullptr;
  c->cap_sym = 0; c->d_sym = nullptr; c->cap_state = 0; c->d_state = nullptr;
  c->cap_dout = 0; c->d_dout = nullptr; c->prof_mask = 0;
  c->cur_cands = nullptr; c->cur_npk = nullptr; c->cur_dout = nullptr; c->last_per_frame = 0;
  c->cands_from_fdr = false; c->fast_now = false;
  c->cap_slab = 0; c->d_slab = nullptr;
  c->tx = nullptr;
  c->sub = nullptr;
  c->osd = nullptr;
  c->dist_comm = nullptr; c->dist_rank = 0; c->dist_world = 0;
  c->cap_tmpc = 0; c->d_tmpc = nullptr; c->cap_tmpn = 0; c->d_tmpn = nullptr;
  c->h_pin = nullptr; c->pin_busy[0] = c->pin_busy[1] = false;
  c->d_stream_frames = nullptr; c->cap_stream_frames = 0; c->ring_ev = nullptr;
  c->fstride = p->fl; c->np = p->fl < 45000 ? p->fl : 45000;
  c->cap_ptab = 0; c->d_ptab = nullptr;
  c->ntries = UWSPR_NJIG; c->cap_pwin = 0; c->d_pwin = nullptr; c->cap_need = 0; c->d_need = nullptr;
  c->last_slots = 0; c->last_sched_B = 0; c->last_sched_per_frame = 0; c->last_sched_lazy = false; c->last_sched_out = nullptr;
  c->cap_tabs = 0; c->d_tabs = nullptr; c->d_counter = nullptr; c->d_sched_stamps = nullptr; c->cap_sched_stamps = 0;
  *out = c;
  {
    const int orc = options_from_environment(c);
    if (orc) return orc;
  }

  fdr_consts &f = c->fc;
  memset(&f, 0, sizeof(f));
  const int size = 2 * p->spb;
  const int maxfreq = (int)((float)p->fs / 2.0);
  if (p->halfbandwidth > maxfreq)
    return fail(c, UWSPR_ERR_PARAM, "Half pass bandwidth (%d) must be lower than max freq range (%d)",
                p->halfbandwidth, maxfreq);
  if (p->spb != 256) return fail(c, UWSPR_ERR_UNSUPPORTED, "spb=%d: this build implements the 512-point transform (spb=256)", p->spb);
  if (p->fs <= 0 || p->fl <= 0 || p->maxdrift < 0 || p->maxfreqs < 1 || p->halfbandwidth < 1 || p->cf <= 0)
    return fail(c, UWSPR_ERR_ARG, "non-positive constructor argument");
  f.fl = p->fl; f.size = size; f.m = size / 2; f.maxfreqs = p->maxfreqs; f.maxdrift = p->maxdrift;
  f.df = (float)p->fs / (float)size;
  f.hpbm = (int)ceil((float)(int)(float)p->halfbandwidth / f.df);
  f.n = (int)(floor(((float)p->fl / (float)p->spb) * 2.0) - 3);
  f.finpb = 2 * f.hpbm;
  f.noiseidx = (int)floor(0.3 * (float)f.finpb);
  f.min_snr = (float)pow(10.0, -7.0 / 10.0);
  f.min_snr_floor = (float)(0.1 * (double)f.min_snr);
  f.threshold = (float)p->threshold;
  if (f.n < 2 * (UWSPR_NSYM - 1) + UWSPR_NK0 || (f.n - 1) * (p->spb / 2) + size > p->fl)
    return fail(c, UWSPR_ERR_UNSUPPORTED, "fl=%d too short for 162 symbols + 26 half-symbol offsets", p->fl);
  if (f.finpb > 512 || f.finpb < 3) return fail(c, UWSPR_ERR_RANGE, "pass band of %d bins", f.finpb);

  f.nlin = 2 * p->maxdrift + 1;
  f.cell_hyps = f.nlin + UWSPR_NSLM;
  f.ntot = UWSPR_NIFR * UWSPR_NK0 * f.cell_hyps;
  f.ifr_lo = f.m - f.hpbm + 1 - 2;
  const int ifr_hi = f.m + f.hpbm - 2 + 2;
  f.n_ifr = ifr_hi - f.ifr_lo + 1;
  std::vector<float> slm((size_t)UWSPR_NSLM * 111);
  for (int s = 0; s < UWSPR_NSLM; s++) {
    const double V1 = (double)((s / 5) % 5) - 2.0, V2 = (double)(s / 25) - 2.0;
    const int p2 = 50 + 200 * (s % 5);
    for (int t = 0; t < 111; t++)
      slm[(size_t)s * 111 + t] = slm_frequency_drift(V1, V2, 0, p2, (float)p->cf, (float)t);
  }
  std::vector<int8_t> off((size_t)f.n_ifr * f.cell_hyps * 164, 0);
  int omin = 1 << 30, omax = -(1 << 30);
  for (int r = 0; r < f.n_ifr; r++) {
    const int ifr = f.ifr_lo + r;
    for (int h = 0; h < f.cell_hyps; h++) {
      for (int k = 0; k < UWSPR_NSYM; k++) {
        int ifd;
        if (h < f.nlin) {
          const int drift = h - p->maxdrift;
          ifd = (int)((double)ifr + ((double)(float)k - 81.0) / 81.0 * (double)(float)drift /
                                        (2.0 * (double)f.df));
        } else {
          const int t = k * 111 / 162;
          ifd = (int)((float)ifr + slm[(size_t)(h - f.nlin) * 111 + t] / f.df);
        }
        const int o = ifd - ifr;
        if (o < -128 || o > 127) return fail(c, UWSPR_ERR_RANGE, "search reach %d bins", o);
        omin = std::min(omin, o); omax = std::max(omax, o);
        off[((size_t)r * f.cell_hyps + h) * 164 + k] = (int8_t)o;
      }
    }
  }
  f.off_min = omin; f.off_max = omax; f.nc = UWSPR_NIFR + (omax - omin);
  const int lo = std::min(f.m - f.hpbm - 3, f.ifr_lo + omin - 3);
  const int hi = std::max(f.m + f.hpbm - 1 + 3, ifr_hi + omax + 3);
  if (lo < 0 || hi > size - 1)
    return fail(c, UWSPR_ERR_RANGE,
                "halfbandwidth=%d: pass band + search reach needs columns %d..%d of 0..%d "
                "(the reference reads out of bounds here)", p->halfbandwidth, lo, hi, size - 1);
  f.band_lo = lo; f.band_w = hi - lo + 1;
  f.cand_slots = std::min(p->maxfreqs, std::max(1, (f.finpb - 1) / 2));

  int ndev = 0;
  if (hipGetDeviceCount(&ndev) != hipSuccess || ndev <= 0)
    return fail(c, UWSPR_ERR_NODEVICE, "no HIP device visible; this library has no CPU fallback");
  if (device < 0 || device >= ndev) return fail(c, UWSPR_ERR_ARG, "device %d of %d", device, ndev);
  HIPCHK(c, hipSetDevice(device));
  hipDeviceProp_t prop;
  HIPCHK(c, hipGetDeviceProperties(&prop, device));
  snprintf(c->device_name, sizeof(c->device_name), "%s", prop.gcnArchName);
  c->num_cus = prop.multiProcessorCount > 0 ? prop.multiProcessorCount : 256;
  if (strncmp(prop.gcnArchName, "gfx950", 6) != 0)
    return fail(c, UWSPR_ERR_NODEVICE, "device %d is %s; kernels are built for gfx950 only", device,
                prop.gcnArchName);
  HIPCHK(c, hipStreamCreateWithFlags(&c->own_stream, hipStreamNonBlocking));
  c->stream = c->own_stream;

  std::vector<float> w(size), tw(size);
  for (int i = 0; i < size; i++) w[i] = (float)sin((M_PI / (size - 1)) * i);
  for (int k = 0; k < size / 2; k++) {
    const double ang = 2.0 * M_PI * (double)k / 512.0;
    tw[2 * k] = (float)cos(ang);
    tw[2 * k + 1] = (float)(-sin(ang));
  }
  tw[0] = 1.0f; tw[1] = 0.0f; tw[256] = 0.0f; tw[257] = -1.0f;
  std::vector<std::vector<int>> uniq_of(f.n_ifr);
  std::vector<uint16_t> umap((size_t)f.n_ifr * f.cell_hyps);
  f.umax = 0;
  for (int r = 0; r < f.n_ifr; r++) {
    for (int h = 0; h < f.cell_hyps; h++) {
      const int8_t *sh = &off[((size_t)r * f.cell_hyps + h) * 164];
      int u = -1;
      for (size_t q = 0; q < uniq_of[r].size(); q++)
        if (memcmp(sh, &off[((size_t)r * f.cell_hyps + uniq_of[r][q]) * 164], UWSPR_NSYM) == 0) { u = (int)q; break; }
      if (u < 0) { u = (int)uniq_of[r].size(); uniq_of[r].push_back(h); }
      umap[(size_t)r * f.cell_hyps + h] = (uint16_t)u;
    }
    f.umax = std::max(f.umax, (int)uniq_of[r].size());
  }
  const size_t k3_scratch = coarse_plan(f, c->opt[UWSPR_OPT_K3_PITCH], c->opt[UWSPR_OPT_K3_TILE]);
  const int sw = coarse_seq_words();
  std::vector<uint32_t> offw((size_t)f.n_ifr * f.umax * sw, 0u);
  for (int r = 0; r < f.n_ifr; r++)
    for (int u = 0; u < f.umax; u++) {
      const int h = u < (int)uniq_of[r].size() ? uniq_of[r][u] : uniq_of[r][0];
      for (int k = 0; k < UWSPR_NSYM; k++) {
        const uint32_t e = coarse_seq_entry(f, k, off[((size_t)r * f.cell_hyps + h) * 164 + k]);
        if (e > 0xffffu) return fail(c, UWSPR_ERR_UNSUPPORTED, "coarse tile of %d centre columns", f.nc);
        offw[((size_t)r * f.umax + u) * sw + k / 2] |= e << (16 * (k & 1));
      }
    }
  if (coarse_lds_bytes(f) > 160 * 1024)
    return fail(c, UWSPR_ERR_UNSUPPORTED, "coarse search needs %zu B of LDS (> 160 KiB): reduce maxdrift/cf",
                coarse_lds_bytes(f));
  if (k3_scratch) HIPCHK(c, hipMalloc((void **)&c->d_k3_tile, k3_scratch * sizeof(float) * (size_t)c->num_cus));
  HIPCHK(c, hipMalloc((void **)&c->d_umap, umap.size() * sizeof(uint16_t)));
  HIPCHK(c, hipMemcpy(c->d_umap, umap.data(), umap.size() * sizeof(uint16_t), hipMemcpyHostToDevice));
  HIPCHK(c, hipMalloc((void **)&c->d_window, size * sizeof(float)));
  HIPCHK(c, hipMalloc((void **)&c->d_twiddle, size * sizeof(float)));
  HIPCHK(c, hipMalloc((void **)&c->d_off, offw.size() * sizeof(uint32_t)));
  HIPCHK(c, hipMemcpy(c->d_window, w.data(), size * sizeof(float), hipMemcpyHostToDevice));
  HIPCHK(c, hipMemcpy(c->d_twiddle, tw.data(), size * sizeof(float), hipMemcpyHostToDevice));
  HIPCHK(c, hipMemcpy(c->d_off, offw.data(), offw.size() * sizeof(uint32_t), hipMemcpyHostToDevice));
  if (coarse_configure(f) != 0) return fail(c, UWSPR_ERR_HIP, "cannot reserve %zu B of LDS for the coarse search", coarse_lds_bytes(f));
  return UWSPR_OK;
}

extern "C" void uwspr_ctx_destroy(uwspr_ctx *c) {
  if (!c) return;
  (void)uwspr_dist_finalize(c);
  if (c->own_stream) { (void)hipStreamSynchronize(c->own_stream); }
  tx_release(c);
  sub_release(c);
  osd_release(c);
  void *bufs[] = {c->d_window, c->d_twiddle, c->d_k3_tile, c->d_off, c->d_umap, c->d_fe_taps, c->d_audio, c->d_frames, c->d_ps, c->d_psavg, c->d_smraw,
                  c->d_smspec, c->d_noise, c->d_cands, c->d_npk, c->d_work, c->d_syncgrid, c->d_hyps, c->d_grps, c->d_cent,
                  c->d_abi_hyps, c->d_p, c->d_sync, c->d_sym, c->d_state, c->d_dout, c->d_slab, c->d_tabs, c->d_counter, c->d_sched_stamps, c->d_pwin, c->d_ptab, c->d_need, c->d_stream_frames, c->d_tmpc, c->d_tmpn};
  for (void *b : bufs) if (b) (void)hipFree(b);
  c->ring.close();
  if (c->ring_ev) (void)hipEventDestroy(c->ring_ev);
  if (c->h_pin) { (void)hipHostFree(c->h_pin); (void)hipEventDestroy(c->pin_ev[0]); (void)hipEventDestroy(c->pin_ev[1]); }
  for (auto &e : c->prof_events) { (void)hipEventDestroy(e.a); (void)hipEventDestroy(e.b); }
  for (auto &e : c->ev_pool) (void)hipEventDestroy(e);
  if (c->own_stream) (void)hipStreamDestroy(c->own_stream);
  delete c;
}

extern "C" const char *uwspr_last_error(const uwspr_ctx *c) { return c ? c->err : "null context"; }

extern "C" const char *uwspr_status_string(int s) {
  switch (s) {
    case UWSPR_OK: return "ok";
    case UWSPR_ERR_PARAM: return "half pass bandwidth above fs/2";
    case UWSPR_ERR_RANGE: return "pass band plus search reach outside the spectrum";
    case UWSPR_ERR_UNSUPPORTED: return "unsupported geometry";
    case UWSPR_ERR_HIP: return "HIP runtime error";
    case UWSPR_ERR_NOMEM: return "out of memory";
    case UWSPR_ERR_ARG: return "bad argument";
    case UWSPR_ERR_NODEVICE: return "no gfx950 device (no CPU fallback)";
    default: return "unknown status";
  }
}

extern "C" int uwspr_get_info(const uwspr_ctx *c, uwspr_info *o) {
  if (!c || !o) return UWSPR_ERR_ARG;
  const fdr_consts &f = c->fc;
  memset(o, 0, sizeof(*o));
  o->abi_version = UWSPR_ABI_VERSION;
  o->size = f.size; o->m = f.m; o->hpbm = f.hpbm; o->n = f.n; o->finpb = f.finpb;
  o->noiseidx = f.noiseidx; o->df = f.df; o->min_snr = f.min_snr;
  o->band_lo = f.band_lo; o->band_w = f.band_w; o->cell_hyps = f.cell_hyps;
  o->off_min = f.off_min; o->off_max = f.off_max; o->device = c->device;
  snprintf(o->device_name, sizeof(o->device_name), "%s", c->device_name);
  return UWSPR_OK;
}

static int ready(uwspr_ctx *c) {
  if (!c) return UWSPR_ERR_ARG;
  if (!c->own_stream) return fail(c, UWSPR_ERR_NODEVICE, "context has no device (creation failed: %s)", c->err);
  hipError_t e = hipSetDevice(c->device);
  if (e != hipSuccess) return fail(c, UWSPR_ERR_HIP, "hipSetDevice: %s", hipGetErrorString(e));
  return UWSPR_OK;
}

extern "C" int uwspr_set_stream(uwspr_ctx *c, void *s) {
  int rc = ready(c);
  if (rc) return rc;
  c->stream = s ? (hipStream_t)s : c->own_stream;
  return UWSPR_OK;
}

extern "C" int uwspr_synchronize(uwspr_ctx *c) {
  int rc = ready(c);
  if (rc) return rc;
  HIPCHK(c, hipStreamSynchronize(c->stream));
  return UWSPR_OK;
}

static int upload(uwspr_ctx *c, void *dst, const void *src, size_t bytes) {
  const size_t PIECE = 8u << 20;
  {
    hipPointerAttribute_t at;
    if (hipPointerGetAttributes(&at, src) == hipSuccess && at.type == hipMemoryTypeHost) {
      HIPCHK(c, hipMemcpyAsync(dst, src, bytes, hipMemcpyHostToDevice, c->stream));
      return UWSPR_OK;
    }
    (void)hipGetLastError();
  }
  if (bytes > 4 * PIECE) {
    HIPCHK(c, hipMemcpyAsync(dst, src, bytes, hipMemcpyHostToDevice, c->stream));
    return UWSPR_OK;
  }
  if (!c->h_pin) {
    if (hipHostMalloc((void **)&c->h_pin, 2 * PIECE, hipHostMallocDefault) != hipSuccess) {
      c->h_pin = nullptr;
      (void)hipGetLastError();
      HIPCHK(c, hipMemcpyAsync(dst, src, bytes, hipMemcpyHostToDevice, c->stream));
      return UWSPR_OK;
    }
    HIPCHK(c, hipEventCreateWithFlags(&c->pin_ev[0], hipEventDisableTiming));
    HIPCHK(c, hipEventCreateWithFlags(&c->pin_ev[1], hipEventDisableTiming));
    c->pin_busy[0] = c->pin_busy[1] = false;
  }
  size_t off = 0;
  int k = 0;
  while (off < bytes) {
    const size_t n = bytes - off < PIECE ? bytes - off : PIECE;
    char *half = (char *)c->h_pin + (size_t)(k & 1) * PIECE;
    if (c->pin_busy[k & 1]) HIPCHK(c, hipEventSynchronize(c->pin_ev[k & 1]));
    memcpy(half, (const char *)src + off, n);
    HIPCHK(c, hipMemcpyAsync((char *)dst + off, half, n, hipMemcpyHostToDevice, c->stream));
    HIPCHK(c, hipEventRecord(c->pin_ev[k & 1], c->stream));
    c->pin_busy[k & 1] = true;
    off += n;
    k++;
  }
  return UWSPR_OK;
}

static int frames_on_device(uwspr_ctx *c, const float *frames, int B, int where, const float **dev) {
  if (!frames || B <= 0) return fail(c, UWSPR_ERR_ARG, "frames=%p B=%d", (const void *)frames, B);
  if (where == UWSPR_DEVICE || where == UWSPR_DEVICE_FRAMES) { *dev = frames; return UWSPR_OK; }
  if (where != UWSPR_HOST) return fail(c, UWSPR_ERR_ARG, "where=%d", where);
  const size_t bytes = ((size_t)(B - 1) * c->fstride + c->fc.fl) * 2 * sizeof(float);
  size_t cap = c->cap_frames_bytes / sizeof(float);
  int rc = ensure(c, &c->d_frames, &cap, bytes / sizeof(float));
  c->cap_frames_bytes = cap * sizeof(float);
  if (rc) return rc;
  if ((rc = upload(c, c->d_frames, frames, bytes))) return rc;
  *dev = c->d_frames;
  return UWSPR_OK;
}

int uwspr::api_frames_on_device(uwspr_ctx *c, const float *frames, int B, int where, const float **dev) {
  return frames_on_device(c, frames, B, where, dev);
}

static int copy_out(uwspr_ctx *c, void *dst, const void *src, size_t bytes, int where) {
  if (!dst || bytes == 0) return UWSPR_OK;
  HIPCHK(c, hipMemcpyAsync(dst, src, bytes, where != UWSPR_DEVICE ? hipMemcpyDeviceToHost : hipMemcpyDeviceToDevice, c->stream));
  return UWSPR_OK;
}

extern "C" int uwspr_frontend_batch(uwspr_ctx *c, const float *audio, int B, int nin, int where,
                                    float *frames_out) {
  int rc = ready(c);
  if (rc) return rc;
  const int nout = c->fc.fl;
  if (!audio || !frames_out || B <= 0 || nin <= 0) return fail(c, UWSPR_ERR_ARG, "uwspr_frontend_batch: audio/out/B/nin");
  if (c->p.fs != 375) return fail(c, UWSPR_ERR_UNSUPPORTED, "front-end is 12000 -> 375 S/s (fs=%d)", c->p.fs);
  if (!c->d_fe_taps || c->fe_mode != c->opt[UWSPR_OPT_FRONTEND]) {
    std::vector<float> img;
    int J = 0, dcols = 0;
    if (frontend_tap_image(c->opt[UWSPR_OPT_FRONTEND], img, &J, &dcols)) return fail(c, UWSPR_ERR_ARG, "front-end mode %d", c->opt[UWSPR_OPT_FRONTEND]);
    if (frontend_prepare()) return fail(c, UWSPR_ERR_HIP, "front-end kernel: %zu bytes of LDS refused", (size_t)160 * 1024);
    HIPCHK(c, hipStreamSynchronize(c->stream));
    if (c->d_fe_taps) { HIPCHK(c, hipFree(c->d_fe_taps)); c->d_fe_taps = nullptr; }
    HIPCHK(c, hipMalloc((void **)&c->d_fe_taps, img.size() * sizeof(float)));
    HIPCHK(c, hipMemcpy(c->d_fe_taps, img.data(), img.size() * sizeof(float), hipMemcpyHostToDevice));
    c->fe_mode = c->opt[UWSPR_OPT_FRONTEND]; c->fe_J = J; c->fe_dcols = dcols;
  }
  const float *da = audio;
  float *dout = frames_out;
  if (where == UWSPR_HOST) {
    if ((rc = ensure(c, &c->d_audio, &c->cap_audio, (size_t)B * nin))) return rc;
    size_t cap = c->cap_frames_bytes / sizeof(float);
    rc = ensure(c, &c->d_frames, &cap, (size_t)B * nout * 2);
    c->cap_frames_bytes = cap * sizeof(float);
    if (rc) return rc;
    HIPCHK(c, hipMemcpyAsync(c->d_audio, audio, (size_t)B * nin * sizeof(float), hipMemcpyHostToDevice, c->stream));
    da = c->d_audio; dout = c->d_frames;
  } else if (where != UWSPR_DEVICE) {
    return fail(c, UWSPR_ERR_ARG, "where=%d", where);
  }
  launch_frontend(c, da, B, nin, (float2 *)dout, nout);
  HIPCHK(c, hipGetLastError());
  if (where == UWSPR_HOST) {
    HIPCHK(c, hipMemcpyAsync(frames_out, c->d_frames, (size_t)B * nout * 2 * sizeof(float), hipMemcpyDeviceToHost, c->stream));
    HIPCHK(c, hipStreamSynchronize(c->stream));
  }
  return UWSPR_OK;
}

extern "C" int uwspr_frontend_design(int mode, int stage, double *taps, int cap, int *delay) {
  std::vector<double> g;
  int d = 0;
  const int rc = frontend_design(mode, stage, g, &d);
  if (rc) return rc;
  if (delay) *delay = d;
  const int n = stage == 0 ? (int)g.size() / 2 : (int)g.size();
  if (taps) {
    const int k = (stage == 0 ? 2 : 1) * std::min(n, cap < 0 ? 0 : cap);
    for (int i = 0; i < k; i++) taps[i] = g[i];
  }
  return n;
}

static int ensure_fdr(uwspr_ctx *c, int B) {
  const fdr_consts &f = c->fc;
  if (B <= c->cap_B) return UWSPR_OK;
  size_t cap;
  int rc;
  c->cap_B = 0;
#define GROW(ptr, elems) cap = 0; if (ptr) { HIPCHK(c, hipStreamSynchronize(c->stream)); HIPCHK(c, hipFree(ptr)); ptr = nullptr; } \
  rc = ensure(c, &ptr, &cap, (size_t)(elems)); if (rc) return rc;
  GROW(c->d_ps, (size_t)B * f.n * f.band_w);
  GROW(c->d_psavg, (size_t)B * f.band_w);
  GROW(c->d_smraw, (size_t)B * f.finpb);
  GROW(c->d_smspec, (size_t)B * f.finpb);
  GROW(c->d_noise, (size_t)B);
  GROW(c->d_cands, (size_t)B * f.maxfreqs);
  GROW(c->d_npk, (size_t)B);
  GROW(c->d_work, (size_t)B * f.cand_slots + 1);
#undef GROW
  c->cap_B = B;
  return UWSPR_OK;
}

static int run_fdr(uwspr_ctx *c, const float *dframes, int B, uwspr_candidate *user_cands = nullptr,
                   int32_t *user_npk = nullptr) {
  int rc = ensure_fdr(c, B);
  if (rc) return rc;
  c->cur_cands = user_cands ? user_cands : c->d_cands;
  c->cur_npk = user_npk ? user_npk : c->d_npk;
  if (c->grid_cap > 0) {
    size_t cap = c->cap_grid_bytes / sizeof(float);
    rc = ensure(c, &c->d_syncgrid, &cap, (size_t)B * c->grid_cap * c->fc.ntot);
    c->cap_grid_bytes = cap * sizeof(float);
    if (rc) return rc;
  }
  launch_spectrogram(c, dframes, B);
  launch_spectrum(c, B);
  launch_coarse(c, B);
  HIPCHK(c, hipGetLastError());
  c->last_B = B;
  return UWSPR_OK;
}

extern "C" int uwspr_fdr_batch(uwspr_ctx *c, const float *frames, int B, int where,
                               uwspr_candidate *cands, int32_t *npk) {
  int rc = ready(c);
  if (rc) return rc;
  const float *d;
  if ((rc = frames_on_device(c, frames, B, where, &d))) return rc;
  const bool direct = where == UWSPR_DEVICE && cands && npk;
  if ((rc = run_fdr(c, d, B, direct ? cands : nullptr, direct ? npk : nullptr))) return rc;
  if (!direct) {
    if ((rc = copy_out(c, cands, c->d_cands, (size_t)B * c->fc.maxfreqs * sizeof(uwspr_candidate), where))) return rc;
    if ((rc = copy_out(c, npk, c->d_npk, (size_t)B * sizeof(int32_t), where))) return rc;
  }
  if (where != UWSPR_DEVICE) HIPCHK(c, hipStreamSynchronize(c->stream));
  return UWSPR_OK;
}

extern "C" int uwspr_fdr_read_spectrum(uwspr_ctx *c, int B, float *ps_band, float *psavg, float *smraw,
                                       float *smspec, float *noise) {
  int rc = ready(c);
  if (rc) return rc;
  if (B <= 0 || B > c->last_B) return fail(c, UWSPR_ERR_ARG, "B=%d but the last FDR batch held %d frames", B, c->last_B);
  const fdr_consts &f = c->fc;
  if ((rc = copy_out(c, ps_band, c->d_ps, (size_t)B * f.n * f.band_w * 4, UWSPR_HOST))) return rc;
  if ((rc = copy_out(c, psavg, c->d_psavg, (size_t)B * f.band_w * 4, UWSPR_HOST))) return rc;
  if ((rc = copy_out(c, smraw, c->d_smraw, (size_t)B * f.finpb * 4, UWSPR_HOST))) return rc;
  if ((rc = copy_out(c, smspec, c->d_smspec, (size_t)B * f.finpb * 4, UWSPR_HOST))) return rc;
  if ((rc = copy_out(c, noise, c->d_noise, (size_t)B * 4, UWSPR_HOST))) return rc;
  HIPCHK(c, hipStreamSynchronize(c->stream));
  return UWSPR_OK;
}

extern "C" int uwspr_fdr_keep_syncgrid(uwspr_ctx *c, int ncand_cap) {
  int rc = ready(c);
  if (rc) return rc;
  if (ncand_cap < 0) return fail(c, UWSPR_ERR_ARG, "ncand_cap=%d", ncand_cap);
  c->grid_cap = std::min(ncand_cap, c->fc.cand_slots);
  if (c->grid_cap == 0 && c->d_syncgrid) {
    HIPCHK(c, hipStreamSynchronize(c->stream));
    HIPCHK(c, hipFree(c->d_syncgrid));
    c->d_syncgrid = nullptr; c->cap_grid_bytes = 0;
  }
  return UWSPR_OK;
}

extern "C" int uwspr_fdr_read_syncgrid(uwspr_ctx *c, int B, float *grid) {
  int rc = ready(c);
  if (rc) return rc;
  if (!c->d_syncgrid || c->grid_cap <= 0) return fail(c, UWSPR_ERR_ARG, "sync grid not kept: call uwspr_fdr_keep_syncgrid first");
  if (B <= 0 || B > c->last_B) return fail(c, UWSPR_ERR_ARG, "B=%d but the last FDR batch held %d frames", B, c->last_B);
  if ((rc = copy_out(c, grid, c->d_syncgrid, (size_t)B * c->grid_cap * c->fc.ntot * 4, UWSPR_HOST))) return rc;
  HIPCHK(c, hipStreamSynchronize(c->stream));
  return UWSPR_OK;
}

static int ensure_sweep(uwspr_ctx *c, size_t H, bool soft) {
  int rc;
  if ((rc = ensure(c, &c->d_p, &c->cap_p, H * UWSPR_NSYM))) return rc;
  if ((rc = ensure(c, &c->d_sync, &c->cap_sync, H))) return rc;
  if (soft && (rc = ensure(c, &c->d_sym, &c->cap_sym, H * UWSPR_NSYM))) return rc;
  return UWSPR_OK;
}

extern "C" int uwspr_sync_sweep(uwspr_ctx *c, const float *frames, int B, const uwspr_hyp *hyps, int H,
                                int where, float *sync, uint8_t *symbols) {
  int rc = ready(c);
  if (rc) return rc;
  if (!hyps || H <= 0) return fail(c, UWSPR_ERR_ARG, "hyps=%p H=%d", (const void *)hyps, H);
  if (where == UWSPR_DEVICE_FRAMES) return fail(c, UWSPR_ERR_ARG, "uwspr_sync_sweep: where is UWSPR_HOST or UWSPR_DEVICE");
  const float *d;
  if ((rc = frames_on_device(c, frames, B, where, &d))) return rc;
  if ((rc = ensure(c, &c->d_hyps, &c->cap_hyps, (size_t)H))) return rc;
  const uwspr_hyp *dabi = hyps;
  if (where == UWSPR_HOST) {
    for (int h = 0; h < H; h++)
      if (hyps[h].frame >= B) return fail(c, UWSPR_ERR_ARG, "hyps[%d].frame=%d >= B=%d", h, hyps[h].frame, B);
    if ((rc = ensure(c, &c->d_abi_hyps, &c->cap_abi_hyps, (size_t)H))) return rc;
    HIPCHK(c, hipMemcpyAsync(c->d_abi_hyps, hyps, (size_t)H * sizeof(uwspr_hyp), hipMemcpyHostToDevice, c->stream));
    dabi = c->d_abi_hyps;
  }
  const bool soft = symbols != nullptr;
  if ((rc = ensure_sweep(c, (size_t)H, soft))) return rc;
  launch_prep_hyps(c, dabi, c->d_hyps, H);
  launch_tonecorr(c, d, B, c->d_hyps, H, c->d_p);
  launch_fold(c, c->d_hyps, c->d_p, H, c->d_sync, soft ? c->d_sym : nullptr);
  HIPCHK(c, hipGetLastError());
  if ((rc = copy_out(c, sync, c->d_sync, (size_t)H * 4, where))) return rc;
  if (soft && (rc = copy_out(c, symbols, c->d_sym, (size_t)H * UWSPR_NSYM, where))) return rc;
  if (where == UWSPR_HOST) HIPCHK(c, hipStreamSynchronize(c->stream));
  return UWSPR_OK;
}

extern "C" int uwspr_sync_grid(uwspr_ctx *c, const float *frames, int B, int where,
                               const uwspr_candidate *centres, int nf, const float *df, int ndrift,
                               const float *ddrift, int nlag, const int32_t *dlag, float *sync,
                               uint8_t *symbols) {
  int rc = ready(c);
  if (rc) return rc;
  if (!centres || !df || !ddrift || !dlag || nf < 1 || ndrift < 1 || nlag < 1 || nf > 32 || ndrift > 32 || nlag > 4096)
    return fail(c, UWSPR_ERR_ARG, "uwspr_sync_grid: nf=%d ndrift=%d nlag=%d (nf, ndrift <= 32)", nf, ndrift, nlag);
  if (where == UWSPR_DEVICE_FRAMES) return fail(c, UWSPR_ERR_ARG, "uwspr_sync_grid: where is UWSPR_HOST or UWSPR_DEVICE");
  const float *d;
  if ((rc = frames_on_device(c, frames, B, where, &d))) return rc;
  const long long H = (long long)B * nf * ndrift * nlag;
  if (H > (1LL << 27)) return fail(c, UWSPR_ERR_ARG, "uwspr_sync_grid: %lld hypotheses in one call", H);
  const bool soft = symbols != nullptr;
  if ((rc = ensure(c, &c->d_hyps, &c->cap_hyps, (size_t)H))) return rc;
  if ((rc = ensure_sweep(c, (size_t)H, soft))) return rc;
  size_t need_abi = ((size_t)B * sizeof(uwspr_candidate) + (size_t)nlag * sizeof(int32_t) + sizeof(uwspr_hyp) - 1) / sizeof(uwspr_hyp) + 1;
  if ((rc = ensure(c, &c->d_abi_hyps, &c->cap_abi_hyps, need_abi))) return rc;
  uwspr_candidate *dcent = reinterpret_cast<uwspr_candidate *>(c->d_abi_hyps);
  int32_t *ddl = reinterpret_cast<int32_t *>(dcent + B);
  HIPCHK(c, hipMemcpyAsync(dcent, centres, (size_t)B * sizeof(uwspr_candidate),
                           where == UWSPR_HOST ? hipMemcpyHostToDevice : hipMemcpyDeviceToDevice, c->stream));
  HIPCHK(c, hipMemcpyAsync(ddl, dlag, (size_t)nlag * sizeof(int32_t), hipMemcpyHostToDevice, c->stream));
  if (!launch_tonecorr_grid(c, d, B, dcent, nf, df, ndrift, ddrift, nlag, dlag, ddl, c->d_hyps, c->d_p)) {
    launch_tonecorr(c, d, B, c->d_hyps, (int)H, c->d_p);
  }
  launch_fold(c, c->d_hyps, c->d_p, (int)H, c->d_sync, soft ? c->d_sym : nullptr);
  HIPCHK(c, hipGetLastError());
  if ((rc = copy_out(c, sync, c->d_sync, (size_t)H * 4, where))) return rc;
  if (soft && (rc = copy_out(c, symbols, c->d_sym, (size_t)H * UWSPR_NSYM, where))) return rc;
  if (where == UWSPR_HOST) HIPCHK(c, hipStreamSynchronize(c->stream));
  return UWSPR_OK;
}

extern "C" int uwspr_sync_and_demodulate_batch(uwspr_ctx *c, const float *frames, int B, int where,
                                               const uwspr_sync_call *calls, int ncalls,
                                               uwspr_sync_result *results) {
  int rc = ready(c);
  if (rc) return rc;
  if (!calls || !results || ncalls <= 0) return fail(c, UWSPR_ERR_ARG, "calls/results/ncalls");
  std::vector<uwspr_hyp> hyps;
  std::vector<size_t> first(ncalls + 1, 0);
  bool soft = false;
  for (int q = 0; q < ncalls; q++) {
    const uwspr_sync_call &k = calls[q];
    if (k.mode < 0 || k.mode > 2) return fail(c, UWSPR_ERR_ARG, "calls[%d].mode=%d", q, k.mode);
    if (k.symfac != 50) return fail(c, UWSPR_ERR_UNSUPPORTED, "calls[%d].symfac=%d (the path uses 50)", q, k.symfac);
    if (k.frame < 0 || k.frame >= B) return fail(c, UWSPR_ERR_ARG, "calls[%d].frame=%d", q, k.frame);
    int ifmin = k.ifmin, ifmax = k.ifmax, lagmin = k.lagmin, lagmax = k.lagmax;
    float fstep = k.fstep;
    if (k.mode == 0) { ifmin = 0; ifmax = 0; fstep = 0.0f; }
    if (k.mode == 1) { lagmin = k.shift1; lagmax = k.shift1; }
    if (k.mode == 2) { lagmin = k.shift1; lagmax = k.shift1; ifmin = 0; ifmax = 0; soft = true; }
    if (k.lagstep <= 0) return fail(c, UWSPR_ERR_ARG, "calls[%d].lagstep=%d", q, k.lagstep);
    first[q] = hyps.size();
    for (int ifreq = ifmin; ifreq <= ifmax; ifreq++) {
      const float f0 = k.f1 + (float)ifreq * fstep;
      for (int lag = lagmin; lag <= lagmax; lag += k.lagstep) {
        uwspr_hyp h;
        memset(&h, 0, sizeof(h));
        h.frame = k.frame; h.m_type = k.candidate.m_type; h.f0 = f0; h.lag = lag;
        h.drift = k.drift1;
        if (k.candidate.m_type == UWSPR_NONLINEAR) {
          h.V1 = k.candidate.m_nonlinear.V1; h.V2 = k.candidate.m_nonlinear.V2;
          h.p1 = k.candidate.m_nonlinear.p1; h.p2 = k.candidate.m_nonlinear.p2;
        }
        hyps.push_back(h);
        if (hyps.size() > (size_t)1 << 26) return fail(c, UWSPR_ERR_ARG, "more than 2^26 hypotheses in one batch");
      }
    }
  }
  first[ncalls] = hyps.size();
  const int H = (int)hyps.size();
  std::vector<float> sync(std::max(H, 1));
  std::vector<uint8_t> sym(soft ? (size_t)std::max(H, 1) * UWSPR_NSYM : 0);
  if (H > 0) {
    const float *d;
    if ((rc = frames_on_device(c, frames, B, where, &d))) return rc;
    if ((rc = ensure(c, &c->d_hyps, &c->cap_hyps, (size_t)H))) return rc;
    if ((rc = ensure(c, &c->d_abi_hyps, &c->cap_abi_hyps, (size_t)H))) return rc;
    if ((rc = ensure_sweep(c, (size_t)H, soft))) return rc;
    HIPCHK(c, hipMemcpyAsync(c->d_abi_hyps, hyps.data(), (size_t)H * sizeof(uwspr_hyp), hipMemcpyHostToDevice, c->stream));
    launch_prep_hyps(c, c->d_abi_hyps, c->d_hyps, H);
    launch_tonecorr(c, d, B, c->d_hyps, H, c->d_p);
    launch_fold(c, c->d_hyps, c->d_p, H, c->d_sync, soft ? c->d_sym : nullptr);
    HIPCHK(c, hipGetLastError());
    HIPCHK(c, hipMemcpyAsync(sync.data(), c->d_sync, (size_t)H * 4, hipMemcpyDeviceToHost, c->stream));
    if (soft) HIPCHK(c, hipMemcpyAsync(sym.data(), c->d_sym, (size_t)H * UWSPR_NSYM, hipMemcpyDeviceToHost, c->stream));
    HIPCHK(c, hipStreamSynchronize(c->stream));
  }
  for (int q = 0; q < ncalls; q++) {
    const uwspr_sync_call &k = calls[q];
    uwspr_sync_result &r = results[q];
    memset(&r, 0, sizeof(r));
    float syncmax = -1e30f, fbest = 0.0f;
    int best_shift = 0;
    for (size_t h = first[q]; h < first[q + 1]; h++)
      if (sync[h] > syncmax) { syncmax = sync[h]; best_shift = hyps[h].lag; fbest = hyps[h].f0; }
    r.sync = syncmax;
    if (k.mode <= 1) { r.shift1 = best_shift; r.f1 = fbest; }
    else {
      r.shift1 = k.shift1; r.f1 = k.f1;
      if (first[q + 1] > first[q]) memcpy(r.symbols, &sym[(first[q + 1] - 1) * UWSPR_NSYM], UWSPR_NSYM);
    }
  }
  return UWSPR_OK;
}

static int run_schedule_impl(uwspr_ctx *c, const float *dframes, int B, const uwspr_candidate *dcands,
                             const int32_t *dnpk, int cand_stride, int per_frame, uwspr_demod_out *user_out);

static int run_schedule(uwspr_ctx *c, const float *dframes, int B, const uwspr_candidate *dcands,
                        const int32_t *dnpk, int cand_stride, int per_frame,
                        uwspr_demod_out *user_out = nullptr) {
  c->last_sched_B = 0; c->last_sched_per_frame = 0; c->last_sched_lazy = false; c->last_sched_out = nullptr;
  const int rc = run_schedule_impl(c, dframes, B, dcands, dnpk, cand_stride, per_frame, user_out);
  if (rc) return rc;
  c->last_slots = B * per_frame; c->last_sched_B = B; c->last_sched_per_frame = per_frame;
  c->last_sched_lazy = c->ntries < UWSPR_NJIG;
  c->last_sched_out = c->cur_dout;
  return UWSPR_OK;
}

static int run_schedule_impl(uwspr_ctx *c, const float *dframes, int B, const uwspr_candidate *dcands,
                             const int32_t *dnpk, int cand_stride, int per_frame, uwspr_demod_out *user_out) {
  static const int hpc[6] = {5, 5, 2, 5, 5, UWSPR_NJIG};
  const size_t nslots = (size_t)B * per_frame;
  c->sched_per_frame = per_frame;
  int rc;
  if ((rc = ensure(c, &c->d_state, &c->cap_state, nslots))) return rc;
  const int njig = c->ntries < UWSPR_NJIG ? c->ntries : UWSPR_NJIG;
  if (c->use_fused || njig < UWSPR_NJIG) {
    if (c->sched_grid <= 0) c->sched_grid = c->num_cus;
    if ((rc = ensure(c, &c->d_tabs, &c->cap_tabs, (size_t)c->sched_grid * kSchedTabFloats))) return rc;
    if (!c->d_counter) HIPCHK(c, hipMalloc((void **)&c->d_counter, 64));
  }
  if (c->use_fused) {
    if (c->opt[UWSPR_OPT_SCHED_STAMPS] &&
        (rc = ensure(c, &c->d_sched_stamps, &c->cap_sched_stamps, nslots * 64))) return rc;
    if ((rc = ensure(c, &c->d_dout, &c->cap_dout, nslots))) return rc;
    c->cur_dout = user_out ? user_out : c->d_dout;
    if (c->ntries < UWSPR_NJIG) {
      if ((rc = ensure(c, &c->d_pwin, &c->cap_pwin, nslots * UWSPR_NSYM * 4))) return rc;
    }
    launch_sched_fused(c, dframes, B, dcands, dnpk, cand_stride, per_frame, c->cur_dout,
                       c->ntries < UWSPR_NJIG ? c->ntries : UWSPR_NJIG);
    HIPCHK(c, hipGetLastError());
    return UWSPR_OK;
  }
  if ((rc = ensure(c, &c->d_hyps, &c->cap_hyps, 2 * nslots * UWSPR_NJIG))) return rc;
  if ((rc = ensure(c, &c->d_grps, &c->cap_grps, 3 * nslots))) return rc;
  if ((rc = ensure(c, &c->d_cent, &c->cap_cent, (nslots * 13 + 11) / 12 + 1))) return rc;
  c->d_cent_frame = reinterpret_cast<int32_t *>(c->d_cent + nslots);
  if ((rc = ensure_sweep(c, nslots * UWSPR_NJIG, true))) return rc;
  if ((rc = ensure(c, &c->d_dout, &c->cap_dout, nslots))) return rc;
  c->cur_dout = user_out ? user_out : c->d_dout;
  dev_hyp *half[2] = {c->d_hyps, c->d_hyps + nslots * UWSPR_NJIG};
  if ((rc = ensure(c, &c->d_pwin, &c->cap_pwin, nslots * UWSPR_NSYM * 4))) return rc;
  if ((rc = ensure(c, &c->d_ptab, &c->cap_ptab, nslots * kPtabPerSlot * kPtabFloat2))) return rc;
  launch_sched_init(c, dcands, dnpk, cand_stride, B, per_frame);
  const bool lazy = njig < UWSPR_NJIG;
  const int sk = c->opt[UWSPR_OPT_STAGE_KERNELS];
  for (int s = 0; s < 6; s++) {
    c->fast_now = c->fast_search && s < 5;
    const int H = (int)(nslots * (s == 5 ? njig : hpc[s]));
    const dev_hyp *h = half[s & 1];
    if (sk == 0 || (lazy && s == 5)) launch_tonecorr(c, dframes, B, h, H, c->d_p);
#if !defined(UWSPR_S2_PAIRS) || UWSPR_S2_PAIRS
    else if (s == 2) {
      launch_tonecorr_dpair(c, dframes, B, h, (int)nslots, c->d_p);
      if (!(c->cands_from_fdr && c->p.maxdrift == 0)) launch_tonecorr(c, dframes, B, h, H, c->d_p, nullptr, 1, true);
    }
#else
    else if (s == 2) launch_tonecorr(c, dframes, B, h, H, c->d_p);
#endif
    else if (s == 1 || s == 4) launch_tonecorr_fstage(c, dframes, B, h, (int)nslots, H, c->d_p);
    else if (s == 3) launch_tonecorr_ring(c, dframes, B, c->d_grps, (int)nslots, 5, 16, H, c->d_p, 1);
    else if (s == 5 && (c->opt[UWSPR_OPT_K4_FORMS] & 1))
      launch_tonecorr_jig(c, dframes, B, c->d_grps, (int)(3 * nslots), H, c->d_p, 3);
    else if (s == 5) launch_tonecorr_ring(c, dframes, B, c->d_grps, (int)(3 * nslots), 6, 8, H, c->d_p, 3);
    else if (c->use_ptab) {
      launch_tonecorr_lag0(c, dframes, B, c->d_grps, (int)nslots, H, c->d_p);
      if (!(c->cands_from_fdr && c->p.maxdrift == 0)) launch_tonecorr(c, dframes, B, h, H, c->d_p, c->d_grps, 5);
    }
    else launch_tonecorr(c, dframes, B, h, H, c->d_p);
    if (s < 5) {
      launch_fold_step(c, s + 1, (int)nslots, njig);
      c->fast_now = false;
    } else {
      launch_fold(c, h, c->d_p, H, c->d_sync, c->d_sym, (const float4 *)c->d_pwin, njig);
      launch_sched_finish(c, (int)nslots, njig);
      if (lazy) launch_keep_try0(c, (int)nslots, njig);
    }
  }
  HIPCHK(c, hipGetLastError());
  return UWSPR_OK;
}

extern "C" int uwspr_demod_batch(uwspr_ctx *c, const float *frames, int B, int where,
                                 const uwspr_candidate *cands, const int32_t *npk, int cand_stride,
                                 int max_per_frame, uwspr_demod_out *out) {
  int rc = ready(c);
  if (rc) return rc;
  if (!cands || !npk || cand_stride <= 0 || max_per_frame <= 0 || !out)
    return fail(c, UWSPR_ERR_ARG, "cands/npk/cand_stride/max_per_frame/out");
  const float *d;
  if ((rc = frames_on_device(c, frames, B, where, &d))) return rc;
  const uwspr_candidate *dc = cands;
  const int32_t *dn = npk;
  const bool host_recs = where != UWSPR_DEVICE;
  if (host_recs) {
    if ((rc = ensure(c, &c->d_tmpc, &c->cap_tmpc, (size_t)B * cand_stride))) return rc;
    if ((rc = ensure(c, &c->d_tmpn, &c->cap_tmpn, (size_t)B))) return rc;
    HIPCHK(c, hipMemcpyAsync(c->d_tmpc, cands, (size_t)B * cand_stride * sizeof(uwspr_candidate), hipMemcpyHostToDevice, c->stream));
    HIPCHK(c, hipMemcpyAsync(c->d_tmpn, npk, (size_t)B * sizeof(int32_t), hipMemcpyHostToDevice, c->stream));
    dc = c->d_tmpc; dn = c->d_tmpn;
  }
  c->cands_from_fdr = false;
  rc = run_schedule(c, d, B, dc, dn, cand_stride, max_per_frame);
  if (!rc) rc = copy_out(c, out, c->d_dout, (size_t)B * max_per_frame * sizeof(uwspr_demod_out), host_recs ? UWSPR_HOST : UWSPR_DEVICE);
  if (!rc && !host_recs) c->last_sched_out = out;
  if (host_recs) (void)hipStreamSynchronize(c->stream);
  c->last_per_frame = 0;
  return rc;
}

extern "C" int uwspr_pipeline_batch(uwspr_ctx *c, const float *frames, int B, int where,
                                    int max_per_frame, uwspr_candidate *cands, int32_t *npk,
                                    uwspr_demod_out *out) {
  int rc = ready(c);
  if (rc) return rc;
  if (max_per_frame <= 0) return fail(c, UWSPR_ERR_ARG, "max_per_frame=%d", max_per_frame);
  const float *d;
  if ((rc = frames_on_device(c, frames, B, where, &d))) return rc;
  const bool dev = where == UWSPR_DEVICE;
  if ((rc = run_fdr(c, d, B, dev ? cands : nullptr, (dev && cands) ? npk : nullptr))) return rc;
  c->cands_from_fdr = true;
  if ((rc = run_schedule(c, d, B, c->cur_cands, c->cur_npk, c->fc.maxfreqs, max_per_frame,
                         dev ? out : nullptr))) return rc;
  c->last_per_frame = max_per_frame;
  if (c->next_slab) {
    if (!c->next_slab_done) launch_pack_slabs(c, c->cur_cands, c->cur_npk, c->cur_dout, max_per_frame, c->next_slab_K, c->next_slab, B);
    c->next_slab = nullptr; c->next_slab_done = false;
    HIPCHK(c, hipGetLastError());
  }
  if (c->cur_cands == c->d_cands &&
      (rc = copy_out(c, cands, c->d_cands, (size_t)B * c->fc.maxfreqs * sizeof(uwspr_candidate), where))) return rc;
  if (c->cur_npk == c->d_npk && (rc = copy_out(c, npk, c->d_npk, (size_t)B * sizeof(int32_t), where))) return rc;
  if (c->cur_dout == c->d_dout &&
      (rc = copy_out(c, out, c->d_dout, (size_t)B * max_per_frame * sizeof(uwspr_demod_out), where))) return rc;
  if (where != UWSPR_DEVICE) HIPCHK(c, hipStreamSynchronize(c->stream));
  return UWSPR_OK;
}

__global__ void k_cut_frames(const float2 *__restrict__ src, float2 *__restrict__ dst, int hop, int fl, int f0) {
  const int f = f0 + blockIdx.y;
  for (int i = blockIdx.x * blockDim.x + threadIdx.x; i < fl; i += gridDim.x * blockDim.x)
    dst[(size_t)f * fl + i] = src[(size_t)f * hop + i];
}

extern "C" int uwspr_set_frame_stride(uwspr_ctx *c, int stride) {
  int rc = ready(c);
  if (rc) return rc;
  if (stride < 0) return fail(c, UWSPR_ERR_ARG, "stride=%d", stride);
  c->fstride = stride > 0 ? stride : c->fc.fl;
  return UWSPR_OK;
}

extern "C" int uwspr_stream_open(uwspr_ctx *c, int hop, int max_frames) {
  int rc = ready(c);
  if (rc) return rc;
  if (hop <= 0 || hop > c->fc.fl || max_frames <= 0) return fail(c, UWSPR_ERR_ARG, "hop=%d max_frames=%d", hop, max_frames);
  HIPCHK(c, hipStreamSynchronize(c->stream));
  if (!c->ring.open(c->fc.fl, hop, max_frames))
    return fail(c, UWSPR_ERR_NOMEM, "stream buffers (%d frames, hop %d): %s", max_frames, hop, hipGetErrorString(c->ring.err));
  if (!c->ring_ev) HIPCHK(c, hipEventCreateWithFlags(&c->ring_ev, hipEventDisableTiming));
  return UWSPR_OK;
}

extern "C" int uwspr_stream_push(uwspr_ctx *c, const float *iq, int nsamples, int where, int *nready) {
  int rc = ready(c);
  if (rc) return rc;
  stream_ring &r = c->ring;
  if (!r.is_open()) return fail(c, UWSPR_ERR_ARG, "uwspr_stream_push before uwspr_stream_open");
  if (nsamples < 0 || (nsamples > 0 && !iq)) return fail(c, UWSPR_ERR_ARG, "iq/nsamples");
  if (where != UWSPR_HOST && where != UWSPR_DEVICE && where != UWSPR_HOST_ASYNC) return fail(c, UWSPR_ERR_ARG, "where=%d", where);
  if (r.kind == RING_AUDIO && nsamples > 0) return fail(c, UWSPR_ERR_ARG, "uwspr_stream_push on an audio stream (reset it first)");
  if (r.have + (size_t)nsamples > r.cap)
    return fail(c, UWSPR_ERR_ARG, "stream buffer full (%zu + %d > %zu samples): take frames first", r.have, nsamples, r.cap);
  if (nsamples > 0) {
    r.kind = RING_IQ;
    bool ok;
    if (where == UWSPR_DEVICE) {
      HIPCHK(c, hipEventRecord(c->ring_ev, c->stream));
      ok = r.append(iq, (size_t)nsamples, true, c->ring_ev);
    } else {
      ok = r.append(iq, (size_t)nsamples, false);
      if (ok && where == UWSPR_HOST && r.last_direct) ok = r.wait_uploads();
    }
    if (!ok) return fail(c, UWSPR_ERR_HIP, "stream upload: %s", hipGetErrorString(r.err));
  }
  if (nready) *nready = r.ready();
  return UWSPR_OK;
}

extern "C" int uwspr_stream_push_audio(uwspr_ctx *c, const void *audio, int nsamples, int format, int where, int *nready) {
  int rc = ready(c);
  if (rc) return rc;
  stream_ring &r = c->ring;
  if (!r.is_open()) return fail(c, UWSPR_ERR_ARG, "uwspr_stream_push_audio before uwspr_stream_open");
  if (nsamples < 0 || (nsamples > 0 && !audio)) return fail(c, UWSPR_ERR_ARG, "audio/nsamples");
  if (format != UWSPR_AUDIO_F32 && format != UWSPR_AUDIO_S16) return fail(c, UWSPR_ERR_ARG, "audio format %d", format);
  if (where != UWSPR_HOST && where != UWSPR_DEVICE && where != UWSPR_HOST_ASYNC) return fail(c, UWSPR_ERR_ARG, "where=%d", where);
  if (c->p.fs != 375) return fail(c, UWSPR_ERR_UNSUPPORTED, "front-end is 12000 -> 375 S/s (fs=%d)", c->p.fs);
  const int mode = c->opt[UWSPR_OPT_FRONTEND];
  if (nsamples > 0 && r.kind == RING_IQ) return fail(c, UWSPR_ERR_ARG, "uwspr_stream_push_audio on an (I,Q) stream (reset it first)");
  if (nsamples > 0 && r.kind == RING_AUDIO && mode != r.au.mode)
    return fail(c, UWSPR_ERR_ARG, "option frontend changed to %d while the audio stream runs in mode %d (reset it first)", mode, r.au.mode);
  const long long nout = r.audio_outputs((size_t)nsamples, mode);
  if (r.have + (size_t)nout > r.cap)
    return fail(c, UWSPR_ERR_ARG, "stream buffer full (%zu + %lld > %zu samples): take frames first", r.have, nout, r.cap);
  if (nsamples > 0) {
    if (r.kind != RING_AUDIO && !r.audio_latch(mode, format == UWSPR_AUDIO_S16))
      return fail(c, UWSPR_ERR_HIP, "audio stream set-up: %s", hipGetErrorString(r.err));
    bool ok;
    if (where == UWSPR_DEVICE) {
      HIPCHK(c, hipEventRecord(c->ring_ev, c->stream));
      ok = r.push_audio(audio, (size_t)nsamples, format == UWSPR_AUDIO_S16, true, c->ring_ev);
    } else {
      ok = r.push_audio(audio, (size_t)nsamples, format == UWSPR_AUDIO_S16, false);
      if (ok && where == UWSPR_HOST && r.last_direct) ok = r.wait_uploads();
    }
    if (!ok) return fail(c, UWSPR_ERR_HIP, "audio stream: %s", hipGetErrorString(r.err));
  }
  if (nready) *nready = r.ready();
  return UWSPR_OK;
}

extern "C" int uwspr_stream_wait_uploads(uwspr_ctx *c) {
  int rc = ready(c);
  if (rc) return rc;
  if (c->ring.is_open() && !c->ring.wait_uploads()) return fail(c, UWSPR_ERR_HIP, "stream upload: %s", hipGetErrorString(c->ring.err));
  return UWSPR_OK;
}

static int stream_view(uwspr_ctx *c, int nframes, const float **view, long long *first_pos) {
  stream_ring &r = c->ring;
  if (!r.is_open() || nframes <= 0 || nframes > r.ready())
    return fail(c, UWSPR_ERR_ARG, "uwspr_stream_take(%d): %d frames are complete", nframes, r.is_open() ? r.ready() : 0);
  HIPCHK(c, hipEventRecord(c->ring_ev, c->stream));
  r.reader_done(0, c->ring_ev); r.reader_done(1, c->ring_ev);
  if (!r.view(nframes, c->stream, view, first_pos, nullptr)) return fail(c, UWSPR_ERR_HIP, "stream view: %s", hipGetErrorString(r.err));
  return UWSPR_OK;
}

extern "C" int uwspr_stream_take_view(uwspr_ctx *c, int nframes, const float **frames, int *stride, long long *first_pos) {
  int rc = ready(c);
  if (rc) return rc;
  if (!frames) return fail(c, UWSPR_ERR_ARG, "frames");
  if ((rc = stream_view(c, nframes, frames, first_pos))) return rc;
  if (stride) *stride = c->ring.hop;
  return UWSPR_OK;
}

extern "C" int uwspr_stream_take(uwspr_ctx *c, int nframes, float *dev_dst, const float **frames, long long *first_pos) {
  int rc = ready(c);
  if (rc) return rc;
  const float *src = nullptr;
  if ((rc = stream_view(c, nframes, &src, first_pos))) return rc;
  float *dst = dev_dst;
  if (!dst) {
    if ((rc = ensure(c, &c->d_stream_frames, &c->cap_stream_frames, (size_t)c->ring.maxf * c->fc.fl * 2))) return rc;
    dst = c->d_stream_frames;
  }
  for (int f0 = 0; f0 < nframes; f0 += 32768) {
    const int nf = std::min(32768, nframes - f0);
    hipLaunchKernelGGL(k_cut_frames, dim3(44, nf), dim3(256), 0, c->stream, (const float2 *)src, (float2 *)dst,
                       c->ring.hop, c->fc.fl, f0);
  }
  HIPCHK(c, hipGetLastError());
  if (frames) *frames = dst;
  return UWSPR_OK;
}

extern "C" int uwspr_stream_reset(uwspr_ctx *c, long long pos) {
  int rc = ready(c);
  if (rc) return rc;
  if (c->ring.is_open() && c->ring_ev) {
    HIPCHK(c, hipEventRecord(c->ring_ev, c->stream));
    c->ring.reader_done(0, c->ring_ev); c->ring.reader_done(1, c->ring_ev);
  }
  c->ring.reset(pos);
  return UWSPR_OK;
}

extern "C" int uwspr_device_alloc(size_t bytes, void **ptr) {
  if (!ptr) return UWSPR_ERR_ARG;
  return hipMalloc(ptr, bytes) == hipSuccess ? UWSPR_OK : UWSPR_ERR_NOMEM;
}
extern "C" void uwspr_device_free(void *ptr) { if (ptr) (void)hipFree(ptr); }

extern "C" int uwspr_host_alloc(size_t bytes, void **ptr) {
  if (!ptr) return UWSPR_ERR_ARG;
  return hipHostMalloc(ptr, bytes, hipHostMallocDefault) == hipSuccess ? UWSPR_OK : UWSPR_ERR_NOMEM;
}
extern "C" void uwspr_host_free(void *ptr) { if (ptr) (void)hipHostFree(ptr); }

extern "C" int uwspr_set_tries(uwspr_ctx *c, int ntries) {
  int rc = ready(c);
  if (rc) return rc;
  if (ntries < 1 || ntries > UWSPR_NJIG) return fail(c, UWSPR_ERR_ARG, "ntries=%d (1..%d)", ntries, UWSPR_NJIG);
  c->ntries = ntries;
  return UWSPR_OK;
}

extern "C" int uwspr_demod_resume(uwspr_ctx *c, const float *frames, int B, int where, const uint8_t *need,
                                  int max_per_frame, uwspr_demod_out *out) {
  int rc = ready(c);
  if (rc) return rc;
  if (!need || !out || B <= 0 || max_per_frame <= 0) return fail(c, UWSPR_ERR_ARG, "need/out/B/max_per_frame");
  if (!c->d_pwin || !c->last_sched_lazy || c->last_sched_B != B || c->last_sched_per_frame != max_per_frame)
    return fail(c, UWSPR_ERR_ARG, "uwspr_demod_resume follows a schedule call of the same batch made with uwspr_set_tries(< %d)", UWSPR_NJIG);
  if (where == UWSPR_DEVICE ? (out != c->last_sched_out) : (c->last_sched_out != c->d_dout))
    return fail(c, UWSPR_ERR_ARG, "uwspr_demod_resume: the first pass wrote its records to %s; resume with %s",
                c->last_sched_out == c->d_dout ? "the context (a host-record call)" : "the caller's device buffer",
                c->last_sched_out == c->d_dout ? "where = UWSPR_HOST / UWSPR_DEVICE_FRAMES" : "where = UWSPR_DEVICE and that buffer");
  const float *d;
  if ((rc = frames_on_device(c, frames, B, where, &d))) return rc;
  const size_t nslots = (size_t)B * max_per_frame;
  const uint8_t *dneed = need;
  uwspr_demod_out *dout = out;
  const bool host_io = where != UWSPR_DEVICE;
  if (host_io) {
    if ((rc = ensure(c, &c->d_need, &c->cap_need, nslots))) return rc;
    HIPCHK(c, hipMemcpyAsync(c->d_need, need, nslots, hipMemcpyHostToDevice, c->stream));
    dneed = c->d_need;
    dout = c->d_dout;
  }
  launch_sched_fused(c, d, B, nullptr, nullptr, 0, max_per_frame, dout, UWSPR_NJIG, dneed);
  HIPCHK(c, hipGetLastError());
  if (host_io) {
    HIPCHK(c, hipMemcpyAsync(out, c->d_dout, nslots * sizeof(uwspr_demod_out), hipMemcpyDeviceToHost, c->stream));
    HIPCHK(c, hipStreamSynchronize(c->stream));
  }
  return UWSPR_OK;
}

extern "C" int uwspr_pipeline_slabs(uwspr_ctx *c, int K, void *slabs_device) {
  int rc = ready(c);
  if (rc) return rc;
  if (slabs_device && (K < 1 || K > c->fc.maxfreqs)) return fail(c, UWSPR_ERR_ARG, "uwspr_pipeline_slabs: K=%d", K);
  c->next_slab = (uint8_t *)slabs_device; c->next_slab_K = K; c->next_slab_done = false;
  return UWSPR_OK;
}

extern "C" int uwspr_pack_slabs(uwspr_ctx *c, int B, int K, void *slabs, int where) {
  int rc = ready(c);
  if (rc) return rc;
  if (!slabs || K < 1 || K > c->fc.maxfreqs || B <= 0 || B > c->last_B || c->last_per_frame < 1 || !c->cur_dout)
    return fail(c, UWSPR_ERR_ARG, "uwspr_pack_slabs: needs a preceding uwspr_pipeline_batch of >= %d frames", B);
  const size_t bytes = (size_t)B * (16 + (size_t)K * 48 + 16);
  uint8_t *dst = (uint8_t *)slabs;
  if (where == UWSPR_HOST) {
    size_t cap = c->cap_slab;
    if ((rc = ensure(c, &c->d_slab, &cap, bytes))) return rc;
    c->cap_slab = cap;
    dst = c->d_slab;
  }
  launch_pack_slabs(c, c->cur_cands, c->cur_npk, c->cur_dout, c->last_per_frame, K, dst, B);
  HIPCHK(c, hipGetLastError());
  if (where == UWSPR_HOST) {
    HIPCHK(c, hipMemcpyAsync(slabs, c->d_slab, bytes, hipMemcpyDeviceToHost, c->stream));
    HIPCHK(c, hipStreamSynchronize(c->stream));
  }
  return UWSPR_OK;
}

extern "C" int uwspr_debug_sched_stamps(uwspr_ctx *c, unsigned long long *out, int nslots) {
  if (!c || !out || !c->d_sched_stamps || (size_t)nslots * 64 > c->cap_sched_stamps) return UWSPR_ERR_ARG;
  HIPCHK(c, hipStreamSynchronize(c->stream));
  HIPCHK(c, hipMemcpy(out, c->d_sched_stamps, (size_t)nslots * 64 * sizeof(unsigned long long), hipMemcpyDeviceToHost));
  return UWSPR_OK;
}

extern "C" int uwspr_prof_enable(uwspr_ctx *c, int mask) {
  int rc = ready(c);
  if (rc) return rc;
  c->prof_mask = mask & UWSPR_PROF_ALL;
  return UWSPR_OK;
}

extern "C" int uwspr_prof_intervals(uwspr_ctx *c, int kind, void *epoch_event, double *start_ms,
                                    double *stop_ms, int cap, int *n) {
  int rc = ready(c);
  if (rc) return rc;
  if (!epoch_event || !start_ms || !stop_ms || !n || cap < 0) return UWSPR_ERR_ARG;
  HIPCHK(c, hipStreamSynchronize(c->stream));
  int k = 0;
  for (auto &e : c->prof_events) {
    if (e.kind != kind) continue;
    float a = 0.0f, b = 0.0f;
    if (k < cap && hipEventElapsedTime(&a, (hipEvent_t)epoch_event, e.a) == hipSuccess &&
        hipEventElapsedTime(&b, (hipEvent_t)epoch_event, e.b) == hipSuccess) {
      start_ms[k] = a; stop_ms[k] = b;
      k++;
    }
  }
  *n = k;
  return UWSPR_OK;
}

extern "C" int uwspr_prof_read(uwspr_ctx *c, uwspr_prof *o) {
  int rc = ready(c);
  if (rc) return rc;
  if (!o) return UWSPR_ERR_ARG;
  memset(o, 0, sizeof(*o));
  HIPCHK(c, hipStreamSynchronize(c->stream));
  for (auto &e : c->prof_events) {
    float ms = 0.0f;
    if (hipEventElapsedTime(&ms, e.a, e.b) == hipSuccess) {
      o->ms[e.kind] += ms; o->launches[e.kind] += 1; o->units[e.kind] += e.units;
    }
    c->ev_pool.push_back(e.a); c->ev_pool.push_back(e.b);
  }
  c->prof_events.clear();
  return UWSPR_OK;
}
```

gr-uwspr_amd/csrc/uwspr_internal.h:

```cpp
#pragma once

#include <hip/hip_runtime.h>
#include <hip/hip_ext.h>
#include <stdint.h>
#include <vector>

#include "../../include/uwspr_hip.h"
#include "stream_ring.h"

enum {
  UWSPR_OPT_SCHED = 0,
  UWSPR_OPT_STAGE_KERNELS,
  UWSPR_OPT_REUSE,
  UWSPR_OPT_PHASOR_TABLES,
  UWSPR_OPT_FAST_SEARCH,
  UWSPR_OPT_K4_T,
  UWSPR_OPT_K5_LANES,
  UWSPR_OPT_K1_ROWS,
  UWSPR_OPT_K3_TILE,
  UWSPR_OPT_K3_PITCH,
  UWSPR_OPT_SCHED_STAMPS,
  UWSPR_OPT_SCHED_GRID,
  UWSPR_OPT_DIST_FORCE_COMM,
  UWSPR_OPT_FRONTEND,
  UWSPR_OPT_K4_FORMS,
  UWSPR_NOPT
};

namespace uwspr {

#define UWSPR_PR3_WORDS                                                        \
  { 0x07a47103u, 0x58b340a4u, 0x56349558u, 0xe2cdc904u, 0x63580ca0u, 0x00000000u }
__host__ __device__ constexpr uint32_t pr3_word(int w) {
  constexpr uint32_t t[6] = UWSPR_PR3_WORDS;
  return t[w];
}
__host__ __device__ constexpr int pr3_bit(int k) { return (pr3_word(k >> 5) >> (k & 31)) & 1; }

__device__ __forceinline__ float ieee_sqrtf(float x) { return __builtin_sqrtf(x); }
__device__ __forceinline__ float ieee_divf(float x, float y) { return x / y; }

__device__ __forceinline__ unsigned xcd_swizzle(unsigned bid, unsigned nwg) {
#ifdef UWSPR_NO_XCD_SWIZZLE
  return bid;
#else
  const unsigned q = nwg >> 3, r = nwg & 7u, x = bid & 7u;
  return (x < r ? x * (q + 1) : r * (q + 1) + (x - r) * q) + (bid >> 3);
#endif
}

#ifndef UWSPR_SMALL_PRIO
#define UWSPR_SMALL_PRIO 3
#endif
#define UWSPR_SET_PRIO(level) do { if ((level) > 0) __builtin_amdgcn_s_setprio(level); } while (0)

struct dev_hyp {
  int32_t frame;
  int32_t lag;
  float f0;
  float drift;
  float slmc;
  int32_t m_type;
};

struct dev_grp {
  int32_t frame;
  int32_t m_type;
  float f0, drift, slmc;
  int32_t nvalid;
  int32_t hyp_base;
  int32_t lag[8];
  uint32_t hmap;
};
static_assert(sizeof(dev_grp) == 64, "dev_grp is one 64-byte record");

struct cand_state {
  int32_t frame;
  int32_t m_type;
  float slmc;
  float f1, drift1, sync1;
  int32_t shift1;
  int32_t worth;
  float driftp, driftm;
  float csync;
  int32_t cknown;
  float tabA_f, tabB_f;
  int32_t tabA_ok, tabB_ok;
};
constexpr int kPtabPerSlot = 10;
constexpr int kPtabSetB = 5;
constexpr int kPtabFloat2 = 4 * 256;

struct fdr_consts {
  int fl, n, size, m, hpbm, finpb, noiseidx, maxfreqs, maxdrift;
  int band_lo, band_w;
  int cell_hyps, nlin, ntot;
  int off_min, off_max, nc;
  int tp;
  int k3_mode;
  int ifr_lo, n_ifr;
  int umax;
  int cand_slots;
  float df, min_snr, min_snr_floor, threshold;
};

struct ev_pair { hipEvent_t a, b; int kind; int64_t units; };
struct tx_state;
void tx_release(uwspr_ctx *c);
struct sub_state;
void sub_release(uwspr_ctx *c);
struct osd_state;
void osd_release(uwspr_ctx *c);

}

struct uwspr_ctx {
  uwspr_params p;
  uwspr::fdr_consts fc;
  int device;
  int num_cus;
  char device_name[64];
  hipStream_t own_stream, stream;
  char err[512];

  float *d_window;
  float *d_twiddle;
  float *d_k3_tile;
  uint32_t *d_off;
  uint16_t *d_umap;
  float *d_fe_taps;
  int fe_mode, fe_J, fe_dcols;
  size_t cap_audio; float *d_audio;

  size_t cap_frames_bytes; float *d_frames;
  int cap_B;
  float *d_ps;
  float *d_psavg;
  float *d_smraw;
  float *d_smspec;
  float *d_noise;
  uwspr_candidate *d_cands;
  int32_t *d_npk;
  int32_t *d_work;
  int last_B;
  int grid_cap; size_t cap_grid_bytes; float *d_syncgrid;

  size_t cap_hyps; uwspr::dev_hyp *d_hyps;
  size_t cap_grps; uwspr::dev_grp *d_grps;
  size_t cap_cent; uwspr_candidate *d_cent; int32_t *d_cent_frame;
  size_t cap_abi_hyps; uwspr_hyp *d_abi_hyps;
  size_t cap_p; float4 *d_p;
  size_t cap_sync; float *d_sync;
  size_t cap_sym; uint8_t *d_sym;
  size_t cap_state; uwspr::cand_state *d_state;
  size_t cap_dout; uwspr_demod_out *d_dout;
  uwspr_candidate *cur_cands; int32_t *cur_npk; uwspr_demod_out *cur_dout;
  int last_per_frame;
  int opt[UWSPR_NOPT];
  bool opt_set[UWSPR_NOPT];
  bool use_fused;
  bool use_stage_kernels;
  bool reuse_centre;
  bool use_ptab;
  bool fast_search, fast_now;
  bool cands_from_fdr;
  uint8_t *next_slab = nullptr; int next_slab_K = 0; bool next_slab_done = false;
  int sched_per_frame = 1;
  int sched_grid;
  size_t cap_tabs; float *d_tabs;
  int *d_counter;
  size_t cap_tmpc; uwspr_candidate *d_tmpc; size_t cap_tmpn; int32_t *d_tmpn;
  void *h_pin; hipEvent_t pin_ev[2]; bool pin_busy[2];
  uwspr::stream_ring ring; float *d_stream_frames; size_t cap_stream_frames;
  hipEvent_t ring_ev;
  int fstride, np;
  int ntries;
  size_t cap_ptab; float2 *d_ptab;
  size_t cap_pwin; float *d_pwin;
  size_t cap_need; uint8_t *d_need;
  int last_slots, last_sched_B, last_sched_per_frame;
  bool last_sched_lazy; uwspr_demod_out *last_sched_out;
  unsigned long long *d_sched_stamps; size_t cap_sched_stamps;
  size_t cap_slab; uint8_t *d_slab;
  void *dist_comm; int dist_rank, dist_world;
  uwspr::tx_state *tx;
  uwspr::sub_state *sub;
  uwspr::osd_state *osd;

  int prof_mask;
  std::vector<uwspr::ev_pair> prof_events;
  std::vector<hipEvent_t> ev_pool;
};

namespace uwspr {

int api_frames_on_device(uwspr_ctx *c, const float *frames, int B, int where, const float **dev);
int subtract_check(uwspr_ctx *c, const uwspr_sub_item *items, int nitems, int nframes);
int subtract_run(uwspr_ctx *c, const float *src, size_t stride, int nslots, const int *slot_frame, const uwspr_sub_item *items,
                 int nitems, int refine, float *dst);

int osd_run(uwspr_ctx *c, const uint8_t *base, const unsigned long long *off, int n, int order, uwspr_osd_result *res,
            uwspr_osd_result **res_out);

int frontend_design(int mode, int stage, std::vector<double> &out, int *delay);
int frontend_tap_image(int mode, std::vector<float> &img, int *J, int *dcols);
std::vector<float> lowpass_hamming(double fs, double cutoff, double tw);
int frontend_prepare();
void launch_frontend(uwspr_ctx *c, const float *audio, int B, int nin, float2 *out, int nout);
void launch_spectrogram(uwspr_ctx *c, const float *frames, int B);
void launch_spectrum(uwspr_ctx *c, int B);
void launch_coarse(uwspr_ctx *c, int B);
void launch_prep_hyps(uwspr_ctx *c, const uwspr_hyp *abi, dev_hyp *out, int H);
void launch_tonecorr(uwspr_ctx *c, const float *frames, int B, const dev_hyp *hyps, int H,
                     float4 *p, const dev_grp *taken = nullptr, int hyps_per_grp = 1, bool skip_pairs = false);
void launch_tonecorr_dpair(uwspr_ctx *c, const float *frames, int B, const dev_hyp *hyps, int nslots, float4 *p);
void launch_tonecorr_lag0(uwspr_ctx *c, const float *frames, int B, const dev_grp *grps, int nslots,
                          int64_t nhyps, float4 *p);
void launch_tonecorr_fstage(uwspr_ctx *c, const float *frames, int B, const dev_hyp *hyps, int nslots,
                            int64_t nhyps, float4 *p);
void launch_tonecorr_ring(uwspr_ctx *c, const float *frames, int B, const dev_grp *grps, int G,
                          int NL, int step, int64_t nhyps, float4 *p, int groups_per_slot = 1);
void launch_tonecorr_jig(uwspr_ctx *c, const float *frames, int B, const dev_grp *grps, int G, int64_t nhyps, float4 *p,
                         int groups_per_slot);
bool launch_tonecorr_grid(uwspr_ctx *c, const float *frames, int B, const uwspr_candidate *centres,
                          int nf, const float *df, int ndrift, const float *ddrift, int nlag,
                          const int *dlag_host, const int *dlag_dev, dev_hyp *hyps, float4 *p);
void launch_fold(uwspr_ctx *c, const dev_hyp *hyps, const float4 *p, int H, float *sync,
                 uint8_t *symbols, const float4 *pwin = nullptr, int per_slot = 1);
void launch_keep_try0(uwspr_ctx *c, int nslots, int njig);
void launch_sched_init(uwspr_ctx *c, const uwspr_candidate *cands, const int32_t *npk,
                       int cand_stride, int B, int per_frame);
void launch_fold_step(uwspr_ctx *c, int stage, int ncand, int njig = UWSPR_NJIG);
void launch_pack_slabs(uwspr_ctx *c, const uwspr_candidate *cands, const int32_t *npk,
                       const uwspr_demod_out *dout, int per_frame, int K, uint8_t *slab, int B);
void launch_sched_finish(uwspr_ctx *c, int ncand, int njig = UWSPR_NJIG);
void launch_sched_fused(uwspr_ctx *c, const float *frames, int B, const uwspr_candidate *cands,
                        const int32_t *npk, int cand_stride, int per_frame, uwspr_demod_out *out,
                        int njig, const uint8_t *resume = nullptr);
constexpr int kSchedTabFloats = 2 * 5 * 4 * 512;

struct prof_scope {
  uwspr_ctx *c; int idx; bool ext;
  prof_scope(uwspr_ctx *c, int kind, int64_t units, bool ext = false);
  ~prof_scope();
};

template <typename K, typename... A>
inline void launch_timed(uwspr_ctx *c, prof_scope &ps, K kernel, dim3 grid, dim3 block, size_t shmem,
                         A... args) {
  if (ps.idx >= 0 && ps.ext)
    hipExtLaunchKernelGGL(kernel, grid, block, (uint32_t)shmem, c->stream, c->prof_events[ps.idx].a,
                          c->prof_events[ps.idx].b, 0, args...);
  else
    hipLaunchKernelGGL(kernel, grid, block, shmem, c->stream, args...);
}

}
```

Measured before the change: 741,300.

## Share per-context tone tables across slots via offset indirection

```diff
diff --git a/gr-uwspr_amd/csrc/k4_jig.hip b/gr-uwspr_amd/csrc/k4_jig.hip
--- a/gr-uwspr_amd/csrc/k4_jig.hip
+++ b/gr-uwspr_amd/csrc/k4_jig.hip
@@ -12,7 +12,7 @@
 
 __global__ __launch_bounds__(64 * K4J_WAVES, K4J_OCC) void k4_jig(
     const float2 *__restrict__ frames, int fstride, int np, int nframes, const dev_grp *__restrict__ grps,
-    int G, float *__restrict__ p_out, const float2 *__restrict__ ptab, int gps) {
+    int G, float *__restrict__ p_out, const float2 *__restrict__ ptab, const int32_t *__restrict__ ptofs, int gps) {
   constexpr int NL = 6, PPW = 16;
   constexpr int R = 24;
   constexpr int AH = 21;
@@ -61,8 +61,8 @@
   }
   const float2 *tabA = ptab, *tabB = ptab;
   if (use_tab) {
-    tabA = ptab + ((size_t)(gA / gps) * kPtabPerSlot + (max(selA, 1) - 1)) * kPtabFloat2;
-    tabB = ptab + ((size_t)((gA + 1) / gps) * kPtabPerSlot + (max(selB, 1) - 1)) * kPtabFloat2;
+    if (selA) tabA = ptab + (size_t)ptofs[(gA / gps) * kPtabPerSlot + (selA - 1)] * kPtabFloat2;
+    if (selB) tabB = ptab + (size_t)ptofs[((gA + 1) / gps) * kPtabPerSlot + (selB - 1)] * kPtabFloat2;
     if (!selA) tabA = tabB;
     if (!selB) tabB = tabA;
   }
@@ -259,7 +259,7 @@
   const unsigned blocks = (unsigned)((waves + K4J_WAVES - 1) / K4J_WAVES);
   if (gps < 1) gps = 1;
   launch_timed(c, ps, k4_jig, dim3(blocks), dim3(64 * K4J_WAVES), 0, (const float2 *)frames, c->fstride, c->np, B, grps, G,
-               (float *)p, c->use_ptab ? (const float2 *)c->d_ptab : nullptr, gps);
+               (float *)p, c->use_ptab ? (const float2 *)c->d_ptab : nullptr, c->d_ptofs, gps);
 }
 
 }
diff --git a/gr-uwspr_amd/csrc/k4_tonecorr.hip b/gr-uwspr_amd/csrc/k4_tonecorr.hip
--- a/gr-uwspr_amd/csrc/k4_tonecorr.hip
+++ b/gr-uwspr_amd/csrc/k4_tonecorr.hip
@@ -182,7 +182,7 @@
 template <int NL, int STEP, bool FAST = false>
 __global__ __launch_bounds__(64 * K4G_WAVES) void k4_ring(
     const float2 *__restrict__ frames, int fstride, int np, int nframes, const dev_grp *__restrict__ grps,
-    int G, float *__restrict__ p_out, const float2 *__restrict__ ptab, int gps) {
+    int G, float *__restrict__ p_out, const float2 *__restrict__ ptab, const int32_t *__restrict__ ptofs, int gps) {
   constexpr int PPW = 16;
   constexpr int W = (NL - 1) * STEP;
   constexpr int Q = (15 + W) / 16;
@@ -216,8 +216,8 @@
   const bool use_tab = ptab != nullptr && (okA || liveB) && (!okA || selA != 0) && (!liveB || selB != 0);
   const float2 *tabA = ptab, *tabB = ptab;
   if (use_tab) {
-    if (selA) tabA = ptab + ((size_t)(gA / gps) * kPtabPerSlot + (selA - 1)) * kPtabFloat2;
-    if (selB) tabB = ptab + ((size_t)((gA + 1) / gps) * kPtabPerSlot + (selB - 1)) * kPtabFloat2;
+    if (selA) tabA = ptab + (size_t)ptofs[(gA / gps) * kPtabPerSlot + (selA - 1)] * kPtabFloat2;
+    if (selB) tabB = ptab + (size_t)ptofs[((gA + 1) / gps) * kPtabPerSlot + (selB - 1)] * kPtabFloat2;
     if (!selA) tabA = tabB;
     if (!selB) tabB = tabA;
   }
@@ -436,9 +436,9 @@
   dim3 blk(64 * K4G_WAVES);
   const float2 *pt = c->use_ptab ? c->d_ptab : nullptr;
   if (gps < 1) gps = 1;
-  if (r5 && c->fast_now) launch_timed(c, ps, (k4_ring<5, 16, true>), dim3(blocks), blk, 0, fr, c->fstride, c->np, B, grps, G, po, pt, gps);
-  else if (r5) launch_timed(c, ps, (k4_ring<5, 16>), dim3(blocks), blk, 0, fr, c->fstride, c->np, B, grps, G, po, pt, gps);
-  else launch_timed(c, ps, (k4_ring<6, 8>), dim3(blocks), blk, 0, fr, c->fstride, c->np, B, grps, G, po, pt, gps);
+  if (r5 && c->fast_now) launch_timed(c, ps, (k4_ring<5, 16, true>), dim3(blocks), blk, 0, fr, c->fstride, c->np, B, grps, G, po, pt, c->d_ptofs, gps);
+  else if (r5) launch_timed(c, ps, (k4_ring<5, 16>), dim3(blocks), blk, 0, fr, c->fstride, c->np, B, grps, G, po, pt, c->d_ptofs, gps);
+  else launch_timed(c, ps, (k4_ring<6, 8>), dim3(blocks), blk, 0, fr, c->fstride, c->np, B, grps, G, po, pt, c->d_ptofs, gps);
 }
 
 
@@ -475,7 +475,7 @@
 template <bool FAST = false>
 __global__ __launch_bounds__(256, 4) void k4_lag0(
     const float2 *__restrict__ frames, int fstride, int np, int nframes, const dev_grp *__restrict__ grps,
-    int nslots, float *__restrict__ p_out, const float2 *__restrict__ ptab) {
+    int nslots, float *__restrict__ p_out, const float2 *__restrict__ ptab, const int32_t *__restrict__ ptofs) {
   constexpr int ROWS = 64, CH = 32, ROWDW = 2 * CH + 4, SEGS = 256 / CH, NR = ROWS / SEGS, NCHUNK = 14;
   __shared__ __align__(16) float smp[ROWS * ROWDW];
   __shared__ __align__(16) float4 tab[2][4][128];
@@ -502,7 +502,7 @@
   for (int sl = 0; sl < 2; sl++) {
     if (!(sl ? doB : doA)) continue;
     const float4 *src = reinterpret_cast<const float4 *>(
-        ptab + ((size_t)(sl ? slotB : slotA) * kPtabPerSlot + ((sl ? selB : selA) - 1)) * kPtabFloat2);
+        ptab + (size_t)ptofs[(sl ? slotB : slotA) * kPtabPerSlot + ((sl ? selB : selA) - 1)] * kPtabFloat2);
     float4 *dst = &tab[sl][0][0];
     dst[tid] = src[tid];
     dst[tid + 256] = src[tid + 256];
@@ -589,7 +589,7 @@
 template <int WSETS>
 __global__ __launch_bounds__(256 * WSETS, WSETS == 1 ? 3 : 6) void k4_lag0x(
     const float2 *__restrict__ frames, int fstride, int np, int nframes, const dev_grp *__restrict__ grps,
-    int nslots, float *__restrict__ p_out, const float2 *__restrict__ ptab) {
+    int nslots, float *__restrict__ p_out, const float2 *__restrict__ ptab, const int32_t *__restrict__ ptofs) {
   constexpr int NT = 256 * WSETS;
   constexpr int ROWS = 64, CH = 32, ROWDW = 2 * CH + 4, SEGS = NT / CH, NR = ROWS / SEGS, NCHUNK = 14;
   __shared__ __align__(16) float smp[2][ROWS * ROWDW];
@@ -619,7 +619,7 @@
   for (int sl = 0; sl < 2; sl++) {
     if (!(sl ? doB : doA)) continue;
     const float4 *src = reinterpret_cast<const float4 *>(
-        ptab + ((size_t)(sl ? slotB : slotA) * kPtabPerSlot + ((sl ? selB : selA) - 1)) * kPtabFloat2);
+        ptab + (size_t)ptofs[(sl ? slotB : slotA) * kPtabPerSlot + ((sl ? selB : selA) - 1)] * kPtabFloat2);
     float4 *dst = &tab[sl][0][0];
     for (int e = tid; e < 512; e += NT) dst[e] = src[e];
   }
@@ -718,16 +718,16 @@
   const int form = c->fast_now ? 0 : (c->opt[UWSPR_OPT_K4_FORMS] >> 1) & 3;
   if (c->fast_now)
     launch_timed(c, ps, k4_lag0<true>, dim3(wgs), dim3(256), 0, (const float2 *)frames, c->fstride, c->np, B, grps,
-                 nslots, (float *)p, (const float2 *)c->d_ptab);
+                 nslots, (float *)p, (const float2 *)c->d_ptab, c->d_ptofs);
   else if (form & 2)
     launch_timed(c, ps, k4_lag0x<2>, dim3(wgs), dim3(512), 0, (const float2 *)frames, c->fstride, c->np, B, grps,
-                 nslots, (float *)p, (const float2 *)c->d_ptab);
+                 nslots, (float *)p, (const float2 *)c->d_ptab, c->d_ptofs);
   else if (form & 1)
     launch_timed(c, ps, k4_lag0x<1>, dim3(wgs), dim3(256), 0, (const float2 *)frames, c->fstride, c->np, B, grps,
-                 nslots, (float *)p, (const float2 *)c->d_ptab);
+                 nslots, (float *)p, (const float2 *)c->d_ptab, c->d_ptofs);
   else
     launch_timed(c, ps, k4_lag0<false>, dim3(wgs), dim3(256), 0, (const float2 *)frames, c->fstride, c->np, B, grps,
-                 nslots, (float *)p, (const float2 *)c->d_ptab);
+                 nslots, (float *)p, (const float2 *)c->d_ptab, c->d_ptofs);
 }
 
 #ifdef K4F_STAMPS
diff --git a/gr-uwspr_amd/csrc/k5_fold_schedule.hip b/gr-uwspr_amd/csrc/k5_fold_schedule.hip
--- a/gr-uwspr_amd/csrc/k5_fold_schedule.hip
+++ b/gr-uwspr_amd/csrc/k5_fold_schedule.hip
@@ -1,4 +1,5 @@
 #include "uwspr_internal.h"
+#include "sched_setup.h"
 
 #pragma clang fp contract(off)
 
@@ -202,15 +203,6 @@
   }
 }
 
-__device__ float slm_drift_t0(double V1, double V2, int p1, int p2, float cf) {
-  const double q1 = V1 * 0.0 + (double)p1, q2 = V2 * 0.0 + (double)p2;
-  const float sign = (float)(((q1 * V1 + q2 * V2) > 0) * 2 - 1);
-  const double num = fabs(V1 * q1 + V2 * q2);
-  const double den = sqrt(q1 * q1 + q2 * q2);
-  if (den == 0) return 0.0f;
-  return (float)((double)(-sign) * num / den * (double)cf / (double)1500.0f);
-}
-
 __global__ void k_prep_hyps(const uwspr_hyp *__restrict__ in, dev_hyp *__restrict__ out, int H,
                             float cf) {
   const int h = blockIdx.x * 256 + threadIdx.x;
@@ -229,20 +221,6 @@
                      (float)c->p.cf);
 }
 
-
-__device__ inline void emit(dev_hyp *h, const cand_state &st, bool on, int lag, float f0,
-                            float drift, bool known = false) {
-  h->frame = on ? (known ? -2 - st.frame : st.frame) : -1;
-  h->lag = lag; h->f0 = f0; h->drift = drift; h->slmc = st.slmc; h->m_type = st.m_type;
-}
-
-__device__ inline void emit_group(dev_grp *g, const cand_state &st, bool on, float f0, float drift,
-                                  int hyp_base, const int *lags, int n, uint32_t hmap = 0x76543210u) {
-  g->frame = on ? st.frame : -1;
-  g->m_type = st.m_type; g->f0 = f0; g->drift = drift; g->slmc = st.slmc;
-  g->nvalid = n; g->hyp_base = hyp_base; g->hmap = hmap;
-  for (int l = 0; l < 8; l++) g->lag[l] = l < n ? lags[l] : lags[0];
-}
 
 __device__ inline void emit_centre(uwspr_candidate *ce, int32_t *cframe, const cand_state &st, bool on) {
   ce->freq = st.f1; ce->snr = 0.0f; ce->drift = 0.0f; ce->sync = 0.0f; ce->shift = st.shift1;
@@ -295,15 +273,6 @@
   }
 }
 
-__device__ __forceinline__ int ptab_index(const cand_state &st, int set, float f0, float drift, bool on) {
-  if (!on) return -1;
-  if (st.m_type == UWSPR_LINEAR && drift != 0.0f) return -1;
-  if (!(set == 0 ? st.tabA_ok : st.tabB_ok)) return -1;
-  const float fc = set == 0 ? st.tabA_f : st.tabB_f, step = set == 0 ? 0.25f : 0.05f;
-  for (int q = 0; q < 5; q++)
-    if (__float_as_int(fc + (float)(q - 2) * step) == __float_as_int(f0)) return (set == 0 ? 0 : kPtabSetB) + q;
-  return -1;
-}
 __device__ __forceinline__ int ptab_set(const cand_state &st, int set, float centre, float drift, bool on) {
   if (!on) return -1;
   if (st.m_type == UWSPR_LINEAR && drift != 0.0f) return -1;
@@ -311,51 +280,21 @@
   if (__float_as_int(centre) != __float_as_int(set == 0 ? st.tabA_f : st.tabB_f)) return -1;
   return set == 0 ? 0 : kPtabSetB;
 }
-__device__ __forceinline__ int ptab_select(const cand_state &st, int set, float f0, float drift, bool on) {
-  return ptab_index(st, set, f0, drift, on) + 1;
-}
-
 __global__ void k_sched_init(const uwspr_candidate *__restrict__ cands,
-                             const int32_t *__restrict__ npk, int cand_stride, int B,
-                             int per_frame, float cf, cand_state *__restrict__ state,
-                             dev_hyp *__restrict__ hyps, dev_grp *__restrict__ grps, float2 *__restrict__ ptab) {
+                             const int32_t *__restrict__ npk, int cand_stride, int B, sched_tgt T,
+                             float2 *__restrict__ ptab) {
   UWSPR_SET_PRIO(UWSPR_SMALL_PRIO);
   const int slot = blockIdx.x;
-  if (slot >= B * per_frame) return;
-  const int b = slot / per_frame, j = slot - b * per_frame;
-  cand_state st;
+  if (slot >= B * T.per_frame) return;
+  const int b = slot / T.per_frame, j = slot - b * T.per_frame;
   const bool on = j < npk[b] && j < cand_stride;
-  if (on) {
-    const uwspr_candidate cnd = cands[(size_t)b * cand_stride + j];
-    st.frame = b;
-    st.m_type = cnd.m_type;
-    st.slmc = (cnd.m_type == UWSPR_NONLINEAR)
-                  ? slm_drift_t0(cnd.m_nonlinear.V1, cnd.m_nonlinear.V2, cnd.m_nonlinear.p1,
-                                 cnd.m_nonlinear.p2, cf)
-                  : 0.0f;
-    st.f1 = cnd.freq;
-    st.drift1 = (cnd.m_type == UWSPR_LINEAR) ? cnd.m_linear.drift : 0.0f;
-    st.shift1 = cnd.shift;
-    st.sync1 = cnd.sync;
-  } else {
-    st.frame = -1; st.m_type = 0; st.slmc = 0.0f; st.f1 = 0.0f; st.drift1 = 0.0f;
-    st.shift1 = 0; st.sync1 = 0.0f;
-  }
-  st.worth = 0; st.driftp = 0.0f; st.driftm = 0.0f; st.csync = 0.0f; st.cknown = 0;
-  const float f0 = st.f1 + (float)0 * 0.0f;
-  st.tabA_f = f0; st.tabB_f = 0.0f; st.tabB_ok = 0;
-  st.tabA_ok = (ptab != nullptr && on && (st.m_type != UWSPR_LINEAR || st.drift1 == 0.0f)) ? 1 : 0;
-  if (st.tabA_ok) ptab_build(ptab + ((size_t)slot * kPtabPerSlot + 2) * kPtabFloat2, 1, 2, f0, 0.25f, st.m_type, st.drift1, st.slmc);
+  uwspr_candidate cnd = {};
+  if (on) cnd = cands[(size_t)b * cand_stride + j];
+  int tabA_at; bool build;
+  const cand_state st = sched_setup_state(T, slot, b, on, cnd, &tabA_at, &build);
+  if (build) ptab_build(ptab + (size_t)tabA_at * kPtabFloat2, 1, 2, st.tabA_f, 0.25f, st.m_type, st.drift1, st.slmc);
   if (threadIdx.x != 0) return;
-  state[slot] = st;
-  dev_hyp *h = hyps + (size_t)slot * 5;
-  int lags[5];
-  for (int q = 0; q < 5; q++) {
-    lags[q] = st.shift1 - 128 + 64 * q;
-    emit(&h[q], st, on, lags[q], f0, st.drift1);
-  }
-  emit_group(&grps[slot], st, on, f0, st.drift1, slot * 5, lags, 5);
-  grps[slot].nvalid |= ptab_select(st, 0, f0, st.drift1, on) << 16;
+  sched_setup_write(T, slot, st, tabA_at);
 }
 
 template <int STAGE>
@@ -493,7 +432,7 @@
                              const float4 *__restrict__ p, float *__restrict__ sync,
                              dev_hyp *__restrict__ hout, dev_grp *__restrict__ grps,
                              uwspr_candidate *__restrict__ cent, int32_t *__restrict__ cframe, int nslots,
-                             int reuse, int njig, float4 *__restrict__ pwin, float2 *__restrict__ ptab) {
+                             int reuse, int njig, float4 *__restrict__ pwin, float2 *__restrict__ ptab, ptab_ctx pc) {
   UWSPR_SET_PRIO(UWSPR_SMALL_PRIO);
   constexpr int NIN = STAGE == 3 ? 2 : 5;
   __shared__ k5_wave_lds L[FAST ? 1 : NIN];
@@ -520,8 +459,19 @@
   __syncthreads();
   if (STAGE == 3 && ptab && threadIdx.x < 64) {
     const cand_state st = state[slot];
-    if (st.tabB_ok)
-      ptab_build(ptab + ((size_t)slot * kPtabPerSlot + kPtabSetB) * kPtabFloat2, 5, 0, st.tabB_f, 0.05f, st.m_type, st.drift1, st.slmc);
+    if (st.tabB_ok) {
+      int tabB_at = -1;
+      if (pc.keys != nullptr && st.m_type == UWSPR_LINEAR && st.drift1 == 0.0f) {
+        const int bin = ptab_find_A(pc.keys, pc.band_lo, pc.band_w, pc.m, pc.df, st.tabA_f);
+        const int k = ptab_find_B(pc.keys, pc.band_w, bin, st.tabB_f);
+        if (k >= 0) tabB_at = ptab_ctx_tabB(pc.band_w, bin, k);
+      }
+      if (tabB_at < 0) {
+        tabB_at = ptab_slot_tab(pc.nctx, slot, kPtabSetB);
+        ptab_build(ptab + (size_t)tabB_at * kPtabFloat2, 5, 0, st.tabB_f, 0.05f, st.m_type, st.drift1, st.slmc);
+      }
+      if (threadIdx.x < 5) pc.ofs[slot * kPtabPerSlot + kPtabSetB + threadIdx.x] = tabB_at + (int)threadIdx.x;
+    }
   }
   const int ws = s_wsrc;
   if (pwin && ws >= 0)
@@ -642,13 +592,50 @@
                      dout, per_frame, K, slab, B);
 }
 
+static sched_tgt sched_tgt_of(const uwspr_ctx *c) {
+  sched_tgt T;
+  T.state = c->d_state; T.hyps = c->d_hyps; T.grps = c->d_grps;
+  T.per_frame = c->sched_per_frame; T.use_ptab = (c->use_ptab && c->d_ptab) ? 1 : 0; T.cf = (float)c->p.cf;
+  T.pc = ptab_ctx_of(c);
+  return T;
+}
+
 void launch_sched_init(uwspr_ctx *c, const uwspr_candidate *cands, const int32_t *npk,
                        int cand_stride, int B, int per_frame) {
   const int nslots = B * per_frame;
   prof_scope ps(c, UWSPR_K_SCHED, nslots);
+  c->sched_per_frame = per_frame;
   hipLaunchKernelGGL(k_sched_init, dim3(nslots), dim3(64), 0, c->stream, cands,
-                     npk, cand_stride, B, per_frame, (float)c->p.cf, c->d_state, c->d_hyps, c->d_grps,
-                     c->use_ptab ? c->d_ptab : nullptr);
+                     npk, cand_stride, B, sched_tgt_of(c), c->use_ptab ? c->d_ptab : nullptr);
+}
+
+__global__ __launch_bounds__(64) void k_ptab_ctx_build(float2 *__restrict__ ptab, uint32_t *__restrict__ keys, int band_lo,
+                                                       int band_w, int m, float df) {
+  const int bin = blockIdx.x, part = blockIdx.y;
+  if (bin >= band_w) return;
+  const float fA = ptab_freq_A(band_lo, m, df, bin);
+  if (part == 0) {
+    ptab_build(ptab + (size_t)ptab_ctx_tabA(bin) * kPtabFloat2, 1, 2, fA, 0.25f, UWSPR_LINEAR, 0.0f, 0.0f);
+    if (threadIdx.x == 0) keys[bin] = ptab_bits(fA);
+  } else {
+    const int k = part - 1;
+    const float fB = ptab_freq_B(fA, k);
+    ptab_build(ptab + (size_t)ptab_ctx_tabB(band_w, bin, k) * kPtabFloat2, 5, 0, fB, 0.05f, UWSPR_LINEAR, 0.0f, 0.0f);
+    if (threadIdx.x == 0) keys[band_w + 5 * bin + k] = ptab_bits(fB);
+  }
+}
+
+void launch_ptab_ctx_build(uwspr_ctx *c) {
+  hipLaunchKernelGGL(k_ptab_ctx_build, dim3(c->fc.band_w, 6), dim3(64), 0, c->stream, c->d_ptab, c->d_ptkeys,
+                     c->fc.band_lo, c->fc.band_w, c->fc.m, c->fc.df);
+}
+
+ptab_ctx ptab_ctx_of(const uwspr_ctx *c) {
+  ptab_ctx pc;
+  pc.keys = (c->use_ptab && c->opt[UWSPR_OPT_CTX_TABS] != 0 && c->ptab_nctx > 0) ? c->d_ptkeys : nullptr;
+  pc.ofs = c->d_ptofs;
+  pc.band_lo = c->fc.band_lo; pc.band_w = c->fc.band_w; pc.m = c->fc.m; pc.nctx = c->ptab_nctx; pc.df = c->fc.df;
+  return pc;
 }
 
 void launch_fold_step(uwspr_ctx *c, int stage, int nslots, int njig) {
@@ -661,7 +648,7 @@
   auto go = [&](auto kern, int threads) {
     hipLaunchKernelGGL(kern, g, dim3(threads), 0, c->stream, c->d_state, hin, c->d_p, c->d_sync, hout, c->d_grps,
                        c->d_cent, c->d_cent_frame, nslots, reuse, njig, (float4 *)c->d_pwin,
-                       c->use_ptab ? c->d_ptab : nullptr);
+                       c->use_ptab ? c->d_ptab : nullptr, ptab_ctx_of(c));
   };
   if (c->fast_now) {
     switch (stage) {
diff --git a/gr-uwspr_amd/csrc/ptab_ctx.h b/gr-uwspr_amd/csrc/ptab_ctx.h
--- /dev/null
+++ b/gr-uwspr_amd/csrc/ptab_ctx.h
@@ -0,0 +1,66 @@
+#pragma once
+#include <stdint.h>
+#include <string.h>
+
+#if defined(__HIPCC__) || defined(__CUDACC__)
+#define UWSPR_PT_HD __host__ __device__
+#else
+#define UWSPR_PT_HD
+#endif
+
+namespace uwspr {
+
+constexpr int kPtabCtxPerBin = 26;
+
+struct ptab_ctx {
+  const uint32_t *keys;
+  int32_t *ofs;
+  int band_lo, band_w, m;
+  int nctx;
+  float df;
+};
+
+UWSPR_PT_HD inline uint32_t ptab_bits(float f) {
+  uint32_t u;
+  memcpy(&u, &f, sizeof(u));
+  return u;
+}
+UWSPR_PT_HD inline int ptab_ctx_count(int band_w) { return band_w * kPtabCtxPerBin; }
+UWSPR_PT_HD inline int ptab_ctx_tabA(int bin) { return bin; }
+UWSPR_PT_HD inline int ptab_ctx_tabB(int band_w, int bin, int k) { return band_w + (5 * bin + k) * 5; }
+UWSPR_PT_HD inline int ptab_slot_tab(int nctx, int slot, int t) { return nctx + 10 * slot + t; }
+UWSPR_PT_HD inline size_t ptab_ofs_offset(int nctx, size_t nslots, size_t tab_bytes) { return ((size_t)nctx + 10 * nslots) * tab_bytes; }
+UWSPR_PT_HD inline size_t ptab_keys_offset(int nctx, size_t nslots, size_t tab_bytes) {
+  return ptab_ofs_offset(nctx, nslots, tab_bytes) + 10 * nslots * sizeof(int32_t);
+}
+UWSPR_PT_HD inline size_t ptab_alloc_bytes(int nctx, int band_w, size_t nslots, size_t tab_bytes) {
+  return ptab_keys_offset(nctx, nslots, tab_bytes) + (size_t)band_w * 6 * sizeof(uint32_t);
+}
+
+UWSPR_PT_HD inline float ptab_freq_A(int band_lo, int m, float df, int bin) {
+  const float freq = (float)(band_lo + bin - m) * df;
+  return freq + (float)0 * 0.0f;
+}
+UWSPR_PT_HD inline float ptab_freq_B(float fA, int k) {
+  const float f1 = fA + (float)(k - 2) * 0.25f;
+  return f1 + (float)0 * 0.0f;
+}
+
+UWSPR_PT_HD inline int ptab_find_A(const uint32_t *keys, int band_lo, int band_w, int m, float df, float f) {
+  if (!(f > -1.0e6f && f < 1.0e6f)) return -1;
+  const float r = f / df;
+  const int i0 = (int)(r < 0.0f ? r - 0.5f : r + 0.5f) + m - band_lo;
+  const uint32_t want = ptab_bits(f);
+  for (int i = i0 - 1; i <= i0 + 1; i++)
+    if (i >= 0 && i < band_w && keys[i] == want) return i;
+  return -1;
+}
+UWSPR_PT_HD inline int ptab_find_B(const uint32_t *keys, int band_w, int bin, float f) {
+  if (bin < 0 || bin >= band_w) return -1;
+  const uint32_t want = ptab_bits(f);
+  for (int k = 0; k < 5; k++)
+    if (keys[band_w + 5 * bin + k] == want) return k;
+  return -1;
+}
+
+}
diff --git a/gr-uwspr_amd/csrc/sched_setup.h b/gr-uwspr_amd/csrc/sched_setup.h
--- /dev/null
+++ b/gr-uwspr_amd/csrc/sched_setup.h
@@ -0,0 +1,98 @@
+#pragma once
+#include "uwspr_internal.h"
+
+namespace uwspr {
+
+__device__ inline float slm_drift_t0(double V1, double V2, int p1, int p2, float cf) {
+  const double q1 = V1 * 0.0 + (double)p1, q2 = V2 * 0.0 + (double)p2;
+  const float sign = (float)(((q1 * V1 + q2 * V2) > 0) * 2 - 1);
+  const double num = fabs(V1 * q1 + V2 * q2);
+  const double den = sqrt(q1 * q1 + q2 * q2);
+  if (den == 0) return 0.0f;
+  return (float)((double)(-sign) * num / den * (double)cf / (double)1500.0f);
+}
+
+__device__ inline void emit(dev_hyp *h, const cand_state &st, bool on, int lag, float f0,
+                            float drift, bool known = false) {
+  h->frame = on ? (known ? -2 - st.frame : st.frame) : -1;
+  h->lag = lag; h->f0 = f0; h->drift = drift; h->slmc = st.slmc; h->m_type = st.m_type;
+}
+
+__device__ inline void emit_group(dev_grp *g, const cand_state &st, bool on, float f0, float drift,
+                                  int hyp_base, const int *lags, int n, uint32_t hmap = 0x76543210u) {
+  g->frame = on ? st.frame : -1;
+  g->m_type = st.m_type; g->f0 = f0; g->drift = drift; g->slmc = st.slmc;
+  g->nvalid = n; g->hyp_base = hyp_base; g->hmap = hmap;
+  for (int l = 0; l < 8; l++) g->lag[l] = l < n ? lags[l] : lags[0];
+}
+
+__device__ __forceinline__ int ptab_index(const cand_state &st, int set, float f0, float drift, bool on) {
+  if (!on) return -1;
+  if (st.m_type == UWSPR_LINEAR && drift != 0.0f) return -1;
+  if (!(set == 0 ? st.tabA_ok : st.tabB_ok)) return -1;
+  const float fc = set == 0 ? st.tabA_f : st.tabB_f, step = set == 0 ? 0.25f : 0.05f;
+  for (int q = 0; q < 5; q++)
+    if (__float_as_int(fc + (float)(q - 2) * step) == __float_as_int(f0)) return (set == 0 ? 0 : kPtabSetB) + q;
+  return -1;
+}
+__device__ __forceinline__ int ptab_select(const cand_state &st, int set, float f0, float drift, bool on) {
+  return ptab_index(st, set, f0, drift, on) + 1;
+}
+
+struct sched_tgt {
+  cand_state *state; dev_hyp *hyps; dev_grp *grps;
+  int per_frame, use_ptab;
+  float cf;
+  ptab_ctx pc;
+};
+
+__device__ inline cand_state sched_setup_state(const sched_tgt &T, int slot, int frame, bool on, const uwspr_candidate &cnd,
+                                               int *tabA_at, bool *build) {
+  cand_state st;
+  if (on) {
+    st.frame = frame;
+    st.m_type = cnd.m_type;
+    st.slmc = (cnd.m_type == UWSPR_NONLINEAR)
+                  ? slm_drift_t0(cnd.m_nonlinear.V1, cnd.m_nonlinear.V2, cnd.m_nonlinear.p1,
+                                 cnd.m_nonlinear.p2, T.cf)
+                  : 0.0f;
+    st.f1 = cnd.freq;
+    st.drift1 = (cnd.m_type == UWSPR_LINEAR) ? cnd.m_linear.drift : 0.0f;
+    st.shift1 = cnd.shift;
+    st.sync1 = cnd.sync;
+  } else {
+    st.frame = -1; st.m_type = 0; st.slmc = 0.0f; st.f1 = 0.0f; st.drift1 = 0.0f;
+    st.shift1 = 0; st.sync1 = 0.0f;
+  }
+  st.worth = 0; st.driftp = 0.0f; st.driftm = 0.0f; st.csync = 0.0f; st.cknown = 0;
+  const float f0 = st.f1 + (float)0 * 0.0f;
+  st.tabA_f = f0; st.tabB_f = 0.0f; st.tabB_ok = 0;
+  st.tabA_ok = (T.use_ptab && on && (st.m_type != UWSPR_LINEAR || st.drift1 == 0.0f)) ? 1 : 0;
+  *tabA_at = ptab_slot_tab(T.pc.nctx, slot, 2);
+  *build = false;
+  if (st.tabA_ok) {
+    const int bin = (T.pc.keys != nullptr && st.m_type == UWSPR_LINEAR && st.drift1 == 0.0f)
+                        ? ptab_find_A(T.pc.keys, T.pc.band_lo, T.pc.band_w, T.pc.m, T.pc.df, f0) : -1;
+    if (bin >= 0) *tabA_at = ptab_ctx_tabA(bin);
+    else *build = true;
+  }
+  return st;
+}
+
+__device__ inline void sched_setup_write(const sched_tgt &T, int slot, const cand_state &st, int tabA_at) {
+  const bool on = st.frame >= 0;
+  const float f0 = st.tabA_f;
+  for (int t = 0; t < kPtabPerSlot; t++)
+    T.pc.ofs[slot * kPtabPerSlot + t] = t == 2 ? tabA_at : ptab_slot_tab(T.pc.nctx, slot, t);
+  T.state[slot] = st;
+  dev_hyp *h = T.hyps + (size_t)slot * 5;
+  int lags[5];
+  for (int q = 0; q < 5; q++) {
+    lags[q] = st.shift1 - 128 + 64 * q;
+    emit(&h[q], st, on, lags[q], f0, st.drift1);
+  }
+  emit_group(&T.grps[slot], st, on, f0, st.drift1, slot * 5, lags, 5);
+  T.grps[slot].nvalid |= ptab_select(st, 0, f0, st.drift1, on) << 16;
+}
+
+}
diff --git a/gr-uwspr_amd/csrc/uwspr_api.hip b/gr-uwspr_amd/csrc/uwspr_api.hip
--- a/gr-uwspr_amd/csrc/uwspr_api.hip
+++ b/gr-uwspr_amd/csrc/uwspr_api.hip
@@ -94,6 +94,7 @@
     {"dist_force_comm", 0, 0, 1},
     {"frontend", 0, 0, 1},
     {"k4_forms", 1, 0, 255},
+    {"ctx_tabs", 1, 0, 1},
 };
 
 static void refresh_options(uwspr_ctx *c) {
@@ -199,7 +200,7 @@
   c->h_pin = nullptr; c->pin_busy[0] = c->pin_busy[1] = false;
   c->d_stream_frames = nullptr; c->cap_stream_frames = 0; c->ring_ev = nullptr;
   c->fstride = p->fl; c->np = p->fl < 45000 ? p->fl : 45000;
-  c->cap_ptab = 0; c->d_ptab = nullptr;
+  c->cap_ptab = 0; c->d_ptab = nullptr; c->d_ptofs = nullptr; c->d_ptkeys = nullptr; c->ptab_nctx = 0;
   c->ntries = UWSPR_NJIG; c->cap_pwin = 0; c->d_pwin = nullptr; c->cap_need = 0; c->d_need = nullptr;
   c->last_slots = 0; c->last_sched_B = 0; c->last_sched_per_frame = 0; c->last_sched_lazy = false; c->last_sched_out = nullptr;
   c->cap_tabs = 0; c->d_tabs = nullptr; c->d_counter = nullptr; c->d_sched_stamps = nullptr; c->cap_sched_stamps = 0;
@@ -787,6 +788,28 @@
   return UWSPR_OK;
 }
 
+static int ensure_ptab(uwspr_ctx *c, size_t nslots) {
+  const bool want_ctx = c->use_ptab && c->opt[UWSPR_OPT_CTX_TABS] != 0;
+  const int nctx = (want_ctx || c->ptab_nctx > 0) ? ptab_ctx_count(c->fc.band_w) : 0;
+  if (c->d_ptab && nslots <= c->cap_ptab && nctx == c->ptab_nctx) return UWSPR_OK;
+  const size_t tab_bytes = (size_t)kPtabFloat2 * sizeof(float2);
+  const size_t slots = std::max(nslots, c->cap_ptab);
+  if (c->d_ptab) { HIPCHK(c, hipStreamSynchronize(c->stream)); HIPCHK(c, hipFree(c->d_ptab)); c->d_ptab = nullptr; c->cap_ptab = 0; c->ptab_nctx = 0; }
+  const size_t bytes = ptab_alloc_bytes(nctx, c->fc.band_w, slots, tab_bytes);
+  hipError_t e = hipMalloc((void **)&c->d_ptab, bytes);
+  if (e != hipSuccess) { c->d_ptab = nullptr; return fail(c, UWSPR_ERR_NOMEM, "hipMalloc(%zu bytes): %s", bytes, hipGetErrorString(e)); }
+  char *base = reinterpret_cast<char *>(c->d_ptab);
+  c->d_ptofs = reinterpret_cast<int32_t *>(base + ptab_ofs_offset(nctx, slots, tab_bytes));
+  c->d_ptkeys = reinterpret_cast<uint32_t *>(base + ptab_keys_offset(nctx, slots, tab_bytes));
+  c->cap_ptab = slots; c->ptab_nctx = nctx;
+  if (nctx > 0) {
+    launch_ptab_ctx_build(c);
+    HIPCHK(c, hipGetLastError());
+    HIPCHK(c, hipStreamSynchronize(c->stream));
+  }
+  return UWSPR_OK;
+}
+
 static int run_schedule_impl(uwspr_ctx *c, const float *dframes, int B, const uwspr_candidate *dcands,
                              const int32_t *dnpk, int cand_stride, int per_frame, uwspr_demod_out *user_out) {
   static const int hpc[6] = {5, 5, 2, 5, 5, UWSPR_NJIG};
@@ -822,7 +845,7 @@
   c->cur_dout = user_out ? user_out : c->d_dout;
   dev_hyp *half[2] = {c->d_hyps, c->d_hyps + nslots * UWSPR_NJIG};
   if ((rc = ensure(c, &c->d_pwin, &c->cap_pwin, nslots * UWSPR_NSYM * 4))) return rc;
-  if ((rc = ensure(c, &c->d_ptab, &c->cap_ptab, nslots * kPtabPerSlot * kPtabFloat2))) return rc;
+  if ((rc = ensure_ptab(c, nslots))) return rc;
   launch_sched_init(c, dcands, dnpk, cand_stride, B, per_frame);
   const bool lazy = njig < UWSPR_NJIG;
   const int sk = c->opt[UWSPR_OPT_STAGE_KERNELS];
@@ -1175,6 +1198,34 @@
   return UWSPR_OK;
 }
 
+extern "C" int uwspr_debug_ptab(uwspr_ctx *c, int what, int first, int n, void *out) {
+  int rc = ready(c);
+  if (rc) return rc;
+  if (!out || first < 0 || n < 0) return fail(c, UWSPR_ERR_ARG, "uwspr_debug_ptab(%d, %d, %d)", what, first, n);
+  HIPCHK(c, hipStreamSynchronize(c->stream));
+  const size_t slots = c->d_ptab ? c->cap_ptab : 0;
+  if (what == 0) {
+    int32_t *o = (int32_t *)out;
+    o[0] = c->ptab_nctx; o[1] = c->fc.band_w; o[2] = c->fc.band_lo; o[3] = (int32_t)slots;
+    return UWSPR_OK;
+  }
+  if (!c->d_ptab) return fail(c, UWSPR_ERR_ARG, "uwspr_debug_ptab: no staged schedule has run");
+  if (what == 1) {
+    if (c->ptab_nctx == 0) return fail(c, UWSPR_ERR_ARG, "uwspr_debug_ptab: the context has no tables of its own");
+    HIPCHK(c, hipMemcpy(out, c->d_ptkeys, (size_t)c->fc.band_w * 6 * sizeof(uint32_t), hipMemcpyDeviceToHost));
+  } else if (what == 2) {
+    if ((size_t)first + n > slots) return fail(c, UWSPR_ERR_ARG, "uwspr_debug_ptab: slots %d + %d of %zu", first, n, slots);
+    HIPCHK(c, hipMemcpy(out, c->d_ptofs + (size_t)first * kPtabPerSlot, (size_t)n * kPtabPerSlot * sizeof(int32_t), hipMemcpyDeviceToHost));
+  } else if (what == 3) {
+    const size_t ntab = (size_t)c->ptab_nctx + slots * kPtabPerSlot;
+    if ((size_t)first + n > ntab) return fail(c, UWSPR_ERR_ARG, "uwspr_debug_ptab: tables %d + %d of %zu", first, n, ntab);
+    HIPCHK(c, hipMemcpy(out, c->d_ptab + (size_t)first * kPtabFloat2, (size_t)n * kPtabFloat2 * sizeof(float2), hipMemcpyDeviceToHost));
+  } else {
+    return fail(c, UWSPR_ERR_ARG, "uwspr_debug_ptab: what = %d", what);
+  }
+  return UWSPR_OK;
+}
+
 extern "C" int uwspr_prof_read(uwspr_ctx *c, uwspr_prof *o) {
   int rc = ready(c);
   if (rc) return rc;
diff --git a/gr-uwspr_amd/csrc/uwspr_internal.h b/gr-uwspr_amd/csrc/uwspr_internal.h
--- a/gr-uwspr_amd/csrc/uwspr_internal.h
+++ b/gr-uwspr_amd/csrc/uwspr_internal.h
@@ -7,6 +7,7 @@
 
 #include "../../include/uwspr_hip.h"
 #include "stream_ring.h"
+#include "ptab_ctx.h"
 
 enum {
   UWSPR_OPT_SCHED = 0,
@@ -24,6 +25,7 @@
   UWSPR_OPT_DIST_FORCE_COMM,
   UWSPR_OPT_FRONTEND,
   UWSPR_OPT_K4_FORMS,
+  UWSPR_OPT_CTX_TABS,
   UWSPR_NOPT
 };
 
@@ -175,7 +177,7 @@
   hipEvent_t ring_ev;
   int fstride, np;
   int ntries;
-  size_t cap_ptab; float2 *d_ptab;
+  size_t cap_ptab; float2 *d_ptab; int32_t *d_ptofs; uint32_t *d_ptkeys; int ptab_nctx;
   size_t cap_pwin; float *d_pwin;
   size_t cap_need; uint8_t *d_need;
   int last_slots, last_sched_B, last_sched_per_frame;
@@ -228,6 +230,8 @@
 void launch_fold(uwspr_ctx *c, const dev_hyp *hyps, const float4 *p, int H, float *sync,
                  uint8_t *symbols, const float4 *pwin = nullptr, int per_slot = 1);
 void launch_keep_try0(uwspr_ctx *c, int nslots, int njig);
+void launch_ptab_ctx_build(uwspr_ctx *c);
+ptab_ctx ptab_ctx_of(const uwspr_ctx *c);
 void launch_sched_init(uwspr_ctx *c, const uwspr_candidate *cands, const int32_t *npk,
                        int cand_stride, int B, int per_frame);
 void launch_fold_step(uwspr_ctx *c, int stage, int ncand, int njig = UWSPR_NJIG);
```

Result: no change. 739,600 (-0.2%).
